# hamptus/mlx-swift-qwen3-tts

Measured on NVIDIA B200. Metric: audio-sec generated per sec (RTFx), higher is better.
Workload: dtype u4 g64 weights dequantised at load to f16 operands x f32 accumulate, f32 residual stream

## Files before the change

mlx-swift-qwen3-tts_b200/csrc/api.cu:

```cuda
#include <algorithm>
#include <atomic>
#include <deque>
#include <chrono>
#include <map>
#include <thread>

#include "audio_encoder.h"
#include "speaker_encoder.h"
#include "codec.h"
#include "codec_kernels.h"
#include "engine.h"
#include "gemm_tc.h"
#include "tc_ptx.cuh"

using namespace q3;

struct q3tts_handle : q3::Handle {};

namespace q3 {
void init_talker_kernels();
Handle::~Handle() {
  for (Handle* l : lanes) {
    cudaStreamSynchronize(l->stream);
    delete static_cast<q3tts_handle*>(l);
// ... 323 lines not shown

int64_t plan_decode(int mode, const int32_t* frames, int n, float* out, int64_t capacity, int up, std::vector<DecodeJob>& jobs) {
  if (n <= 0) return 0;
  const int64_t total = std::min<int64_t>((int64_t)n * up, capacity);
  if (mode == Q3TTS_DECODE_WHOLE) {
    jobs.push_back({frames, n, out, 0, total});
    return total;
  }
  const int chunk = mode == Q3TTS_DECODE_FILE ? 16 : (mode == Q3TTS_DECODE_BATCHAPI ? 24 : 18), left = 8;
  for (int pos = 0; pos < n; pos += chunk) {
    const int end = std::min(pos + chunk, n);
    const int ctx = pos == 0 ? 0 : std::min(left, pos);
    const int64_t o0 = (int64_t)pos * up;
    if (o0 >= total) break;
    jobs.push_back({frames + (size_t)(pos - ctx) * 16, end - pos + ctx, out + o0, (int64_t)ctx * up, std::min<int64_t>((int64_t)(end - pos) * up, total - o0)});
  }
  return total;
}

}

extern "C" {

int32_t q3tts_abi_version(void) { return Q3TTS_ABI_VERSION; }

void q3tts_default_options(q3tts_options* o) {
  if (!o) return;
  memset(o, 0, sizeof *o);
  o->struct_size = (int32_t)sizeof *o;
  o->device = 0;
  o->max_batch = 1;
  o->kv_capacity = 512;
  o->max_frames = 2400;
  o->use_cuda_graph = 1;
  o->load_codec = 1;
  o->load_talker = 1;
  o->codec_max_frames = 2400;
  o->codec_max_batch = 8;
}

void q3tts_default_request(q3tts_request* r) {
  if (!r) return;
  memset(r, 0, sizeof *r);
  r->struct_size = (int32_t)sizeof *r;
  r->speaker_id = -1;
  r->temperature = 0.9f;
  r->top_k = 0;
  r->top_p = 1.0f;
  r->repetition_penalty = 1.05f;
  r->max_tokens = 1200;
}

q3tts_status q3tts_create(const char* model_dir, const q3tts_options* opts, q3tts_handle** out) {
  if (!out) return Q3TTS_ERR_INVALID_ARG;
  *out = nullptr;
  q3tts_handle* h = nullptr;
  try {
    Q3_CHECK(model_dir != nullptr, Q3TTS_ERR_INVALID_ARG, "model_dir is NULL");
    q3tts_options o;
    q3tts_default_options(&o);
    if (opts) {
      const size_t n = std::min<size_t>(sizeof o, opts->struct_size > 0 ? (size_t)opts->struct_size : sizeof o);
      memcpy(&o, opts, n);
    }
    require_device(o.device);
    h = new q3tts_handle();
    h->opt.device = o.device;
    h->opt.max_batch = o.max_batch > 0 ? o.max_batch : 1;
    h->opt.kv_capacity = o.kv_capacity > 0 ? std::max(o.kv_capacity, 208) : 512;
    h->opt.max_frames = o.max_frames > 0 ? o.max_frames : 2400;
    h->opt.use_cuda_graph = o.use_cuda_graph;
    h->opt.load_codec = o.load_codec;
    h->opt.load_talker = o.load_talker;
    h->opt.codec_max_frames = o.codec_max_frames > 0 ? o.codec_max_frames : 2400;
    h->opt.codec_max_batch = o.codec_max_batch > 0 ? o.codec_max_batch : 8;
    Q3_CHECK(o.packed_gemm >= 0 && o.packed_gemm <= 2, Q3TTS_ERR_INVALID_ARG, "options.packed_gemm must be 0, 1 or 2");
    h->opt.packed_gemm = o.packed_gemm;
    h->opt.runtime_quantization = o.runtime_quantization != 0;
    h->opt.lanes = std::max(1, std::min(o.lanes, 8));
    if (o.cuda_stream) {
      h->stream = (cudaStream_t)o.cuda_stream;
    } else {
      Q3_CUDA(cudaStreamCreateWithFlags(&h->stream, cudaStreamNonBlocking));
      h->own_stream = true;
    }
    h->opt.stream = h->stream;
    Q3_CUDA(cudaEventCreate(&h->ev_start));
    Q3_CUDA(cudaEventCreate(&h->ev_stop));
    const std::string dir(model_dir);
    h->model_dir = dir;
    if (h->opt.load_talker) {
      Json root = parse_json_file(dir + "/config.json");
      h->cfg = parse_talker_config(root);
      h->talker.reset(new TalkerEngine(dir, h->cfg, h->opt, h->stream, &h->counter));
      h->has_talker = true;
      if (SpeakerEncoderDev::present(dir)) {
        try {
          h->speaker_encoder.reset(new SpeakerEncoderDev(dir, h->stream, &h->counter));
        } catch (const Error& e) {
          g_create_error = std::string("speaker encoder not loaded: ") + e.what();
          cudaGetLastError();
        }
      }
    }
    if (h->opt.load_codec) {
      h->codec.reset(new CodecDecoder(dir + "/speech_tokenizer", h->stream, &h->counter, h->opt.codec_max_frames));
      h->codec->set_use_graph(h->opt.use_cuda_graph != 0);
      if (AudioEncoder::present(dir + "/speech_tokenizer")) {
        try {
          h->audio_encoder.reset(new AudioEncoder(dir + "/speech_tokenizer", h->stream, &h->counter));
        } catch (const Error& e) {
          g_create_error = std::string("audio encoder not loaded: ") + e.what();
          cudaGetLastError();
        }
      }
    }
    Q3_CUDA(cudaStreamSynchronize(h->stream));
    *out = h;
    return Q3TTS_OK;
  } catch (const Error& e) {
    g_create_error = e.what();
    cudaGetLastError();
    delete h;
    return e.status;
  } catch (const std::exception& e) {
    g_create_error = e.what();
    delete h;
    return Q3TTS_ERR_CUDA;
  }
}

q3tts_status q3tts_clone(q3tts_handle* parent, q3tts_handle** out) {
  if (!out) return Q3TTS_ERR_INVALID_ARG;
  *out = nullptr;
  if (!parent) return Q3TTS_ERR_INVALID_ARG;
  q3tts_handle* h = nullptr;
  try {
    std::lock_guard<std::mutex> lk(parent->mu);
    Q3_CHECK(!parent->poisoned, Q3TTS_ERR_CUDA, "the parent handle is poisoned");
    Q3_CUDA(cudaSetDevice(parent->opt.device));
    h = new q3tts_handle();
    h->opt = parent->opt;
    h->opt.lanes = 1;
    h->model_dir = parent->model_dir;
    Q3_CUDA(cudaStreamCreateWithFlags(&h->stream, cudaStreamNonBlocking));
    h->own_stream = true;
    h->opt.stream = h->stream;
    Q3_CUDA(cudaEventCreate(&h->ev_start));
    Q3_CUDA(cudaEventCreate(&h->ev_stop));
    if (parent->talker) {
      h->cfg = parent->cfg;
      h->talker.reset(new TalkerEngine(h->model_dir, h->cfg, h->opt, h->stream, &h->counter, parent->talker->shared()));
      h->has_talker = true;
    }
    if (parent->codec) {
      h->codec.reset(new CodecDecoder(h->model_dir + "/speech_tokenizer", h->stream, &h->counter, h->opt.codec_max_frames));
      h->codec->set_use_graph(h->opt.use_cuda_graph != 0);
    }
    Q3_CUDA(cudaStreamSynchronize(h->stream));
    *out = h;
    return Q3TTS_OK;
  } catch (const Error& e) {
    g_create_error = e.what();
    cudaGetLastError();
    delete h;
    return e.status;
  } catch (const std::exception& e) {
    g_create_error = e.what();
    delete h;
    return Q3TTS_ERR_CUDA;
  }
}

void q3tts_destroy(q3tts_handle* h) {
  if (!h) return;
  cudaSetDevice(h->opt.device);
  cudaStreamSynchronize(h->stream);
  delete h;
}

const char* q3tts_last_error(const q3tts_handle* h) { return h ? h->last_error.c_str() : g_create_error.c_str(); }

q3tts_status q3tts_get_info(const q3tts_handle* hc, q3tts_info* out) {
  if (!hc || !out) return Q3TTS_ERR_INVALID_ARG;
  memset(out, 0, sizeof *out);
  const TalkerConfig& c = hc->cfg;
  if (hc->talker) {
    out->hidden_size = c.hidden_size; out->num_layers = c.num_hidden_layers; out->num_heads = c.num_attention_heads;
    out->num_kv_heads = c.num_key_value_heads; out->head_dim = c.head_dim; out->intermediate_size = c.intermediate_size;
    out->vocab_size = c.vocab_size; out->text_vocab_size = c.text_vocab_size; out->text_hidden_size = c.text_hidden_size;
    out->cp_hidden_size = c.cp.hidden_size; out->cp_num_layers = c.cp.num_hidden_layers; out->cp_vocab_size = c.cp.vocab_size;
    out->num_code_groups = c.cp.num_code_groups;
    out->quant_bits = hc->talker->quant_bits(); out->quant_group_size = hc->talker->quant_group();
    out->weight_dtype = hc->talker->weight_dtype();
    out->num_speakers = (int32_t)c.spk_id.size();
    out->model_type = c.tts_model_type == "voice_design" ? 1 : (c.tts_model_type == "custom_voice" ? 2 : 0);
    out->codec_eos_id = c.codec_eos_token_id; out->codec_pad_id = c.codec_pad_id;
    out->max_batch = hc->talker->max_batch(); out->kv_capacity = hc->talker->kv_capacity(); out->max_frames = hc->talker->max_frames();
    out->device_bytes += (int64_t)hc->talker->device_bytes();
  }
  if (hc->codec) {
    out->has_codec = 1;
    out->codec_num_quantizers = hc->codec->config().num_quantizers;
    out->codec_total_upsample = hc->codec->total_upsample();
    out->device_bytes += (int64_t)hc->codec->device_bytes();
  }
  if (hc->speaker_encoder) {
    out->has_speaker_encoder = 1;
    out->speaker_embedding_dim = hc->speaker_encoder->embedding_dim();
    out->device_bytes += (int64_t)hc->speaker_encoder->device_bytes();
  }
  if (hc->audio_encoder) {
    out->has_audio_encoder = 1;
    out->audio_encoder_hidden = hc->audio_encoder->config().hidden_size;
    out->device_bytes += (int64_t)hc->audio_encoder->device_bytes();
  }
  return Q3TTS_OK;
}

q3tts_status q3tts_speaker_name(const q3tts_handle* h, int32_t index, char* name_out, int32_t capacity, int32_t* id_out) {
  if (!h || index < 0 || index >= (int32_t)h->cfg.spk_id.size()) return Q3TTS_ERR_INVALID_ARG;
  std::vector<std::pair<std::string, int>> s = h->cfg.spk_id;
  std::sort(s.begin(), s.end());
  if (name_out && capacity > 0) {
    strncpy(name_out, s[index].first.c_str(), capacity - 1);
    name_out[capacity - 1] = 0;
  }
  if (id_out) *id_out = s[index].second;
  return Q3TTS_OK;
}

int32_t q3tts_speaker_id(const q3tts_handle* h, const char* name) {
  if (!h || !name) return -1;
  for (auto& kv : h->cfg.spk_id)
    if (kv.first == name) return kv.second;
  return -1;
}

q3tts_status q3tts_clear_cache(q3tts_handle* h) {
  if (h) {
    std::lock_guard<std::mutex> lk(h->lanes_mu);
    for (q3::Handle* l : h->lanes) q3tts_clear_cache(static_cast<q3tts_handle*>(l));
  }
  return guarded(h, [&] {
    Q3_CUDA(cudaStreamSynchronize(h->stream));
    if (h->talker) h->talker->drop_graphs();
  });
}

namespace {
__global__ void debug_mbar_trap_kernel() {
  __shared__ uint64_t bar;
  if (threadIdx.x == 0) {
    q3::tcptx::mbar_init(&bar, 1);
    asm volatile("fence.mbarrier_init.release.cluster;" ::: "memory");
  }
  __syncthreads();
  if (threadIdx.x == 0) q3::tcptx::mbar_wait(&bar, 0);
}
}

q3tts_status q3tts_debug_trap(q3tts_handle* h) {
  return guarded(h, [&] {
    debug_mbar_trap_kernel<<<1, 32, 0, h->stream>>>();
    Q3_CUDA(cudaGetLastError());
    Q3_CUDA(cudaStreamSynchronize(h->stream));
  });
}

q3tts_status q3tts_get_timing(const q3tts_handle* h, q3tts_timing* out) {
  if (!h || !out) return Q3TTS_ERR_INVALID_ARG;
  *out = h->timing;
  return Q3TTS_OK;
}

q3tts_status q3tts_generate_codes(q3tts_handle* h, const q3tts_request* req, int32_t* codes_out, int32_t capacity_frames,
                                  int32_t* frames_out) {
  return guarded(h, [&] {
    Q3_CHECK(req && frames_out, Q3TTS_ERR_INVALID_ARG, "NULL argument");
    Q3_CHECK(h->talker != nullptr, Q3TTS_ERR_MODEL_NOT_LOADED, "Model is not loaded");
    require_no_open_stream(h);
    *frames_out = 0;
    CallTimer tm(h);
    std::vector<int32_t> raw;
    int n_raw = 0;
    run_single(h, *req, raw, n_raw);
    *frames_out = filter_frames(*req, raw, n_raw, codes_out, capacity_frames);
    h->timing.d2h_bytes += (int64_t)n_raw * 64;
    h->timing.h2d_bytes += (int64_t)req->n_text_ids * 4;
    tm.finish();
  });
}

static bool use_lanes(q3tts_handle* h, const q3tts_request* reqs, int32_t n) {
  if (!h || !reqs || h->opt.lanes <= 1 || n <= h->opt.max_batch || h->poisoned) return false;
  for (int i = 0; i < n; ++i)
    if (reqs[i].code0_logits_out || reqs[i].cp_logits_out) return false;
  return true;
}

}
template <typename F>
static q3tts_status over_lanes(q3tts_handle* h, int32_t n, F&& run) {
  const int B = h->opt.max_batch;
  const int blocks = (n + B - 1) / B;
  const int L = std::min(h->opt.lanes, blocks);
// ... 843 lines not shown
```

mlx-swift-qwen3-tts_b200/csrc/engine.h:

```cpp
#pragma once
#include <map>
#include <memory>
#include <mutex>
#include <string>
#include <vector>

#include "frame_kernel.h"
#include "kernels.h"

namespace q3 {

class CodecDecoder;
class AudioEncoder;
class SpeakerEncoderDev;

struct EngineOptions {
  int device = 0;
  cudaStream_t stream = nullptr;
  int max_batch = 1, kv_capacity = 512, max_frames = 2400, use_cuda_graph = 1;
  int load_codec = 1, load_talker = 1, codec_max_frames = 2400, codec_max_batch = 8;
  int lanes = 1;
  int max_trailing = 1024;
  int packed_gemm = 0;
  int runtime_quantization = 0;
};

struct Admission {
  bool too_short = false;
  int prefill_len = 0;
};

struct TalkerShared {
  DeviceArena arena;
  TalkerWeights w;
  int weight_dtype = Q3TTS_BF16, eff_bits = 0, eff_group = 64;
  std::mutex mu;
};

class TalkerEngine {
 public:
  TalkerEngine(const std::string& model_dir, const TalkerConfig& cfg, const EngineOptions& opt, cudaStream_t stream,
               LaunchCounter* counter, std::shared_ptr<TalkerShared> shared = nullptr);
  ~TalkerEngine();

  Admission admit(int slot, const q3tts_request& req);
  struct AdmitItem { int slot; const q3tts_request* req; };
  void admit_batch(const std::vector<AdmitItem>& items, std::vector<Admission>& out);
  int max_prefill_rows() const { return max_rows_; }
  int step_slots(int hi) const {
    if (!handle_tc_) return hi;
    int b = hi <= 32 ? 32 : (hi <= 64 ? 64 : (hi + 127) / 128 * 128);
    return b < opt_.max_batch ? b : opt_.max_batch;
  }
  void run_frames(int n_slots, int n);
  void fetch_states(int n_slots, std::vector<SlotState>& out);
  void fetch_frames(int slot, int first, int count, int32_t* dst);
  void fetch_logits(int frames, float* code0_out, float* cp_out);
  int dump_slot() const { return dump_enabled_ ? dump_slot_ : -1; }
  void release(int slot);
  void drop_graphs();

  const TalkerConfig& config() const { return cfg_; }
  const TalkerWeights& weights() const { return w_; }
  int max_batch() const { return opt_.max_batch; }
  int kv_capacity() const { return opt_.kv_capacity; }
  int max_frames() const { return opt_.max_frames; }
  int weight_dtype() const { return shared_->weight_dtype; }
  int quant_bits() const { return shared_->eff_bits; }
  int quant_group() const { return shared_->eff_group; }
  size_t device_bytes() const { return arena_.total() + (owns_weights_ ? shared_->arena.total() : 0); }
  const std::shared_ptr<TalkerShared>& shared() const { return shared_; }
  size_t weight_bytes_per_frame() const { return w_.talker_step_bytes + 15 * w_.cp_pass_bytes; }
  int64_t graph_replays = 0, graph_nodes_replayed = 0, mega_launches = 0;
  bool megakernel_enabled() const { return mega_.ok; }
  double last_prefill_ms = 0;

  double profile_linears(int which, int m, int iters, int64_t& launches, int64_t& bytes_per_iter);
  int sample_probe(const float* logits, int vocab, float temperature, int top_k, float top_p, float rep_penalty,
                   const int32_t* token_set, int n_set, uint64_t seed, uint64_t counter);

 private:
  void forward_stack(const StackWeights& S, float* x, int m, const int* row_slot, const int* row_pos, const int* win_start,
                     const float* inv_freq, void* kbase, void* vbase, int kv_f16, size_t slot_stride, size_t layer_stride, int capacity,
                     bool one_row_per_slot, bool decode_step, bool x16_ready);
  void issue_frame(int n_slots);
  void build_tc_weights();
  void build_mega_plan();
  TcLinear make_tc(const Linear& L, bool interleave_halves, const float* fold = nullptr);
  bool use_tc(int) const { return handle_tc_; }
  bool use_tc_step(int) const { return handle_tc_; }
  bool use_mega(int n_slots) const { return mega_.ok && !handle_tc_ && opt_.max_batch <= mega_.max_slots && n_slots <= mega_.max_slots; }
  void linear_tc(const TcLinear& L, const void* x16, int m, float* out32, int ld32, void* out16, int ld16, const float* res, int act, int swiglu, bool row_count_invariant = false);
  LaunchCtx ctx() { return LaunchCtx{stream_, counter_, chain_on_ ? &chain_ : nullptr}; }

  TalkerConfig cfg_;
  EngineOptions opt_;
  cudaStream_t stream_;
  LaunchCounter* counter_;
  DeviceArena arena_;
  std::shared_ptr<TalkerShared> shared_;
  bool owns_weights_ = false;
  TalkerWeights& w_;

  int max_rows_ = 0, max_tp_rows_ = 0, set_words_ = 0;
  int tc_min_rows_ = 16, tc_min_rows_step_ = 3;
  bool step_tc_ = false;
  bool handle_tc_ = false;
  bool packed_gemm_ = false;
  void attach_packed(struct TcGemm& g, const TcLinear& L) const;
  static constexpr int kChainCounters = 1024;
  ChainState chain_;
  bool chain_on_ = false, chain_enabled_ = false;
  float* d_rs_ = nullptr;
  static constexpr float kX16Div = 16.0f;
  void *d_h16_ = nullptr, *d_attn16_ = nullptr, *d_act16_ = nullptr, *d_tpe16_ = nullptr, *d_tph16_ = nullptr;
  void *kcache_ = nullptr, *vcache_ = nullptr;
  int kv_f16_ = 0;
  float *cp_k_ = nullptr, *cp_v_ = nullptr;
  size_t kv_slot_stride_ = 0, kv_layer_stride_ = 0, cpkv_slot_stride_ = 0, cpkv_layer_stride_ = 0;
  static constexpr int kCpCapacity = 32;
  SlotState* d_state_ = nullptr;
  int *d_step_slot_ = nullptr, *d_step_pos_ = nullptr, *d_win_ = nullptr;
  int *d_cp_slot2_ = nullptr, *d_cp_pos2_ = nullptr, *d_iota_ = nullptr, *d_cp_pos_ = nullptr;
  int *d_pf_slot_ = nullptr, *d_pf_pos_ = nullptr, *d_pf_win_ = nullptr;
  float *d_x_ = nullptr, *d_qkv_ = nullptr, *d_attn_ = nullptr, *d_act_ = nullptr;
  float *d_hlast_ = nullptr, *d_logits0_ = nullptr, *d_cplogits_ = nullptr, *d_cpin_ = nullptr, *d_cpx_ = nullptr, *d_xstep_ = nullptr;
  int *d_cur_codes_ = nullptr, *d_frames_ = nullptr, *d_forced_ = nullptr;
  unsigned* d_sets_ = nullptr;
  float *d_trailing_ = nullptr, *d_tts_ = nullptr;
  float *d_tpe_ = nullptr, *d_tph_ = nullptr, *d_tp_ = nullptr, *d_spk_ = nullptr;
  int *d_ids_ = nullptr, *d_desc_ = nullptr;
  Embedding* d_cp_emb_ = nullptr;
  float *d_inv_freq_ = nullptr, *d_cp_inv_freq_ = nullptr;
  float *d_dump0_ = nullptr, *d_dumpcp_ = nullptr;
  int dump_cap_ = 0, dump_slot_ = 0;
  bool dump_enabled_ = false;
  float* d_probe_logits_ = nullptr;
  unsigned* d_probe_set_ = nullptr;
  int* d_probe_out_ = nullptr;
  int* h_stage_ = nullptr;
  size_t h_stage_ints_ = 0;
  SlotState* h_state_ = nullptr;
  cudaEvent_t ev_a_ = nullptr, ev_b_ = nullptr;

  struct Graph {
    cudaGraphExec_t exec = nullptr;
    int64_t nodes = 0;
  };
  std::map<long long, Graph> graphs_;
  MegaPlan mega_;
};

struct Handle {
  std::mutex mu;
  std::string model_dir;
  std::string last_error;
  bool poisoned = false;
  EngineOptions opt;
  cudaStream_t stream = nullptr;
  bool own_stream = false;
  LaunchCounter counter;
  TalkerConfig cfg;
  bool has_talker = false;
  std::unique_ptr<TalkerEngine> talker;
  std::unique_ptr<CodecDecoder> codec;
  std::unique_ptr<AudioEncoder> audio_encoder;
  std::unique_ptr<SpeakerEncoderDev> speaker_encoder;
  q3tts_timing timing{};
  cudaEvent_t ev_start = nullptr, ev_stop = nullptr;
  float* h_pcm = nullptr;
  size_t h_pcm_floats = 0;
  int32_t* h_codes = nullptr;
  size_t h_codes_ints = 0;
  int32_t* d_codes = nullptr;
  size_t d_codes_ints = 0;
  float* d_pcm = nullptr;
  size_t d_pcm_floats = 0;
  void* open_stream = nullptr;
  std::mutex lanes_mu;
  std::vector<Handle*> lanes;
  ~Handle();
};

}
```

mlx-swift-qwen3-tts_b200/csrc/gemm_skinny.cu:

```cuda
#include <cuda.h>

#include <algorithm>

#include "skinny_common.cuh"

namespace q3 {

namespace {

using namespace skinny;

template <int ACT, bool SWIGLU>
__global__ void __launch_bounds__(kThreads, 1)
tc_skinny_kernel(const __grid_constant__ CUtensorMap tmW, const __grid_constant__ CUtensorMap tmX, const SkParams p) {
  extern __shared__ uint8_t smem_raw[];
  uint8_t* smem = reinterpret_cast<uint8_t*>((reinterpret_cast<uintptr_t>(smem_raw) + 1023) & ~(uintptr_t)1023);
  const int x_bytes = p.m_pad * kBlockK * 2;
  uint8_t* sW = smem;
  uint8_t* sX = smem + (size_t)p.stages * kWBytes;
  float* red = reinterpret_cast<float*>(sX + (size_t)p.stages * x_bytes);
  uint64_t* full = reinterpret_cast<uint64_t*>(red + (size_t)kRowsW * p.m_pad);
  uint64_t* empty = full + p.stages;
  uint64_t* tmem_full = empty + p.stages;
  uint64_t* red_full = tmem_full + 1;
// ... 31 lines not shown
  __syncthreads();
  tc_fence_after();
  const uint32_t tmem_base = *tmem_slot;
  if (threadIdx.x == 0) SK_STAMP(2);
  if (p.split > 1) cluster_arrive_release();

  if (warp == 0) {
    {
      const bool lead = elect_one();
      const int pre = nkb < p.stages ? nkb : p.stages;
      if (lead) {
        for (int i = 0; i < pre; ++i) {
          mbar_expect_tx(&full[i], (uint32_t)(kWBytes + x_bytes));
          tma_load_2d(sW + (size_t)i * kWBytes, &tmW, &full[i], (kb0 + i) * kBlockK, n0);
        }
        for (int i = pre; i < nkb; ++i) tma_prefetch_2d(&tmW, (kb0 + i) * kBlockK, n0);
      }
      if (p.sig.in) {
        if (lead) sk_wait_dependency_tma(p);
        __syncwarp();
      } else {
        pdl_wait();
      }
      int s = 0;
      uint32_t ph = 0;
      for (int i = 0; i < nkb; ++i) {
        if (i >= pre) mbar_wait(&empty[s], ph ^ 1u);
        if (lead) {
          if (i >= pre) {
            mbar_expect_tx(&full[s], (uint32_t)(kWBytes + x_bytes));
            tma_load_2d(sW + (size_t)s * kWBytes, &tmW, &full[s], (kb0 + i) * kBlockK, n0);
          }
          tma_load_2d(sX + (size_t)s * x_bytes, &tmX, &full[s], (kb0 + i) * kBlockK, 0);
        }
        if (++s == p.stages) { s = 0; ph ^= 1u; }
      }
    }
    __syncwarp();
  } else if (warp == 1) {
    {
      const bool lead = elect_one();
      const uint32_t idesc = (1u << 4) | ((uint32_t)(p.m_pad >> 3) << 17) | ((uint32_t)(kRowsW >> 4) << 24);
      int s = 0;
      uint32_t ph = 0;
      for (int i = 0; i < nkb; ++i) {
        mbar_wait(&full[s], ph);
        tc_fence_after();
        if (lead && i == 0) SK_STAMP(3);
        const uint64_t ad = umma_desc(smem_u32(sW + (size_t)s * kWBytes));
        const uint64_t bd = umma_desc(smem_u32(sX + (size_t)s * x_bytes));
        if (lead) {
#pragma unroll
          for (int k = 0; k < kBlockK / 16; ++k)
            umma_f16(tmem_base, ad + (uint64_t)(2 * k), bd + (uint64_t)(2 * k), idesc, (i | k) != 0 ? 1u : 0u);
          umma_commit(&empty[s]);
        }
        if (++s == p.stages) { s = 0; ph ^= 1u; }
      }
      if (lead) umma_commit(tmem_full);
    }
    __syncwarp();
  } else {
    sk_wait_dependency_warp(p);
    if (p.rms_x) sk_row_factors(p, rowscale_s, rank);
    if (p.split > 1) cluster_wait_acquire();
    mbar_wait(tmem_full, 0);
    tc_fence_after();
    if (threadIdx.x == 64) SK_STAMP(4);
    sk_reduce_epilogue<ACT, SWIGLU>(p, reinterpret_cast<float*>(smem), red, red_full, ack, rowscale_s, tmem_base, rank, n0);
  }
  if (p.split > 1 && warp < 2) cluster_wait_acquire();
  tc_fence_before();
  __syncthreads();
  if (threadIdx.x == 0 && p.trace) {
    SK_STAMP(8);
    p.trace[((size_t)blockIdx.y * gridDim.x + blockIdx.x) * 16 + 9] = sk_globaltimer();
  }
  if (warp == 1) {
    tc_fence_after();
    asm volatile("tcgen05.dealloc.cta_group::1.sync.aligned.b32 %0, %1;" ::"r"(tmem_base), "r"(p.tmem_cols) : "memory");
  }
}

int env_int(const char* name, int dflt) {
  const char* e = getenv(name);
  return e ? atoi(e) : dflt;
}

struct SkPlan {
  int m_pad, split, stages, num_kb, tiles;
  size_t smem;
};

SkPlan plan(const TcGemm& g) {
  static const int max_split = std::max(1, std::min(16, env_int("Q3TTS_SK_MAX_SPLIT", 8)));
  static const int cta_target = env_int("Q3TTS_SK_CTAS", 200);
  static const int smem_kb = env_int("Q3TTS_SK_SMEM_KB", 108);
  SkPlan s{};
  const int M = g.Bt * g.T;
  s.m_pad = M <= 32 ? 32 : (M <= 64 ? 64 : 128);
  s.tiles = (g.N + kRowsW - 1) / kRowsW;
  s.num_kb = (g.cin + kBlockK - 1) / kBlockK;
  s.split = 1;
  while (s.split * 2 <= max_split && s.tiles * s.split * 2 <= cta_target && s.split * 2 <= s.num_kb && s.m_pad / (s.split * 2) >= 4) s.split *= 2;
  const int stage_bytes = kWBytes + s.m_pad * kBlockK * 2;
  const int red_bytes = kRowsW * s.m_pad * 4;
  const int nkb_max = (s.num_kb + s.split - 1) / s.split;
  s.stages = std::max(2, (smem_kb * 1024 - red_bytes) / stage_bytes);
  s.stages = std::max(1, std::min(s.stages, nkb_max));
  while (s.stages * stage_bytes < red_bytes) ++s.stages;
  s.smem = (size_t)s.stages * stage_bytes + red_bytes + 1024 + (2 * s.stages + 4) * 8 + 16 + 128 * 4;
  return s;
}

}

bool tc_skinny_enabled() {
  static const bool on = env_int("Q3TTS_SKINNY", 1) != 0;
  return on;
}

bool tc_skinny_supported(const TcGemm& g) {
  const bool on = tc_skinny_enabled();
  const long long M = (long long)g.Bt * g.T;
  return on && g.allow_skinny && !g.res16 && !g.outr16 && g.ntap == 1 && M >= 1 && M <= 128 && !g.snake_ea && !g.pcm && !(g.swiglu && g.act != TC_ACT_NONE) && tc_gemm_supported(g);
}

using SkKernel = void (*)(const CUtensorMap, const CUtensorMap, const SkParams);
static SkKernel pick_kernel(int act, int swiglu) {
  if (swiglu) return tc_skinny_kernel<TC_ACT_NONE, true>;
  if (act == TC_ACT_GELU) return tc_skinny_kernel<TC_ACT_GELU, false>;
  if (act == TC_ACT_SILU) return tc_skinny_kernel<TC_ACT_SILU, false>;
  return tc_skinny_kernel<TC_ACT_NONE, false>;
}

void init_tc_skinny() {
  tc_resolve_encode();
  for (SkKernel k : {pick_kernel(0, 1), pick_kernel(TC_ACT_GELU, 0), pick_kernel(TC_ACT_SILU, 0), pick_kernel(0, 0)})
    Q3_CUDA(cudaFuncSetAttribute(k, cudaFuncAttributeMaxDynamicSharedMemorySize, 220 * 1024));
  for (SkKernel k : {pick_kernel(0, 1), pick_kernel(TC_ACT_GELU, 0), pick_kernel(TC_ACT_SILU, 0), pick_kernel(0, 0)})
    Q3_CUDA(cudaFuncSetAttribute(k, cudaFuncAttributeNonPortableClusterSizeAllowed, 1));
  init_tc_skinny_q();
}

unsigned long long* g_sk_trace = nullptr;

void tc_skinny_set_trace(unsigned long long* dev_buf) { g_sk_trace = dev_buf; }
unsigned long long* tc_skinny_trace_buf() { return g_sk_trace; }
void tc_skinny_grid(const TcGemm& g, int* tiles, int* split, int* stages) {
  const SkPlan s = plan(g);
  *tiles = s.tiles; *split = s.split; *stages = s.stages;
}

void launch_tc_skinny(const LaunchCtx& c, const TcGemm& g) {
  if (tc_skinny_q_supported(g)) return launch_tc_skinny_q(c, g);
  Q3_CHECK(tc_skinny_supported(g), Q3TTS_ERR_INVALID_ARG, "tc_skinny: unsupported shape (rows %d, cin %d, N %d)", g.Bt * g.T, g.cin, g.N);
  tc_resolve_encode();
  const SkPlan s = plan(g);
  SkParams p{};
  p.M = g.Bt * g.T; p.N = g.N; p.K = g.cin;
  p.m_pad = s.m_pad; p.split = s.split; p.mc = s.m_pad / s.split; p.stages = s.stages; p.num_kb = s.num_kb;
  p.mc_shift = 0;
  while ((1 << p.mc_shift) < p.mc) ++p.mc_shift;
  p.split_shift = 0;
  while ((1 << p.split_shift) < p.split) ++p.split_shift;
  p.tmem_cols = std::max(32, s.m_pad);
  p.bias = g.bias; p.res = g.res; p.ld_res = g.ld_res; p.scale = g.scale; p.act = g.act; p.swiglu = g.swiglu;
  p.out32 = g.out32; p.ld32 = g.ld32; p.out16 = g.out16; p.ld16 = g.ld16;
  p.out16_scale = g.out16_scale;
  p.rms_x = g.rms_in ? g.a : nullptr;
  p.rms_a = 1.0f / (g.in_scale * g.in_scale * (float)g.cin); p.rms_eps = g.rms_eps; p.rms_mult = 1.0f / g.in_scale;
  Q3_CHECK(!g.row_scale, Q3TTS_ERR_INVALID_ARG, "tc_skinny: pass rms_in instead of precomputed row factors");
  p.trace = g_sk_trace;
  p.sig = c.chain_link((unsigned)(s.tiles * s.split));

  const uint64_t wdims[2] = {(uint64_t)g.cin, (uint64_t)g.N};
  const uint64_t wstr[1] = {(uint64_t)g.cin * 2};
  const uint32_t wbox[2] = {(uint32_t)kBlockK, (uint32_t)kRowsW};
  const CUtensorMap mw = tc_make_map(g.w, 2, wdims, wstr, wbox);
  const uint64_t xdims[2] = {(uint64_t)g.cin, (uint64_t)p.M};
  const uint64_t xstr[1] = {(uint64_t)g.cin * 2};
  const uint32_t xbox[2] = {(uint32_t)kBlockK, (uint32_t)s.m_pad};
  const CUtensorMap mx = tc_make_map(g.a, 2, xdims, xstr, xbox);

  Q3_CHECK(s.smem <= 220 * 1024, Q3TTS_ERR_CAPACITY, "tc_skinny: shared memory request %zu too large", s.smem);
  cudaLaunchConfig_t cfg{};
  cfg.gridDim = dim3((unsigned)s.tiles, (unsigned)s.split);
  cfg.blockDim = dim3(kThreads);
  cfg.dynamicSmemBytes = s.smem;
  cfg.stream = c.stream;
  cudaLaunchAttribute attr[2];
  int na = 0;
  if (s.split > 1) {
    attr[na].id = cudaLaunchAttributeClusterDimension;
    attr[na].val.clusterDim.x = 1; attr[na].val.clusterDim.y = (unsigned)s.split; attr[na].val.clusterDim.z = 1;
    ++na;
  }
  if (pdl_enabled()) {
    attr[na].id = cudaLaunchAttributeProgrammaticStreamSerialization;
    attr[na].val.programmaticStreamSerializationAllowed = 1;
    ++na;
  }
  cfg.attrs = attr;
  cfg.numAttrs = na;
  Q3_CUDA(cudaLaunchKernelEx(&cfg, pick_kernel(g.act, g.swiglu), mw, mx, p));
  c.tick_chained();
}

}
```

mlx-swift-qwen3-tts_b200/csrc/skinny_common.cuh:

```cuda
#pragma once
#include <cuda.h>

#include "gemm_tc.h"
#include "tc_ptx.cuh"

namespace q3 {
namespace skinny {

using namespace tcptx;

constexpr int kRowsW = 128;
constexpr int kBlockK = 64;
constexpr int kWBytes = kRowsW * kBlockK * 2;
constexpr int kThreads = 192;

struct SkParams {
  int M, N, K;
  int m_pad, mc, mc_shift, split, stages, num_kb, tmem_cols;
  const float* bias;
  const float* res;
  int ld_res;
  const float* scale;
  int act, swiglu;
  float* out32;
  int ld32;
  __half* out16;
  int ld16;
  float out16_scale;
  const __half* rms_x;
  float rms_a, rms_eps, rms_mult;
  unsigned long long* trace;
  ChainSig sig;
  const void* q_scales;
  const void* q_biases;
  const float* q_fold;
  int q_group, q_sdt;
  int q_pstages;
  int q_xstages, q_xown;
  int q_half_rows;
  int split_shift;
  int q_dbg;
};

__device__ __forceinline__ unsigned long long sk_globaltimer() {
  unsigned long long t;
  asm volatile("mov.u64 %0, %%globaltimer;" : "=l"(t));
  return t;
}
#define SK_STAMP_EPI(slot) do { if (!(p.q_dbg & 1)) SK_STAMP(slot); } while (0)
#define SK_STAMP(slot)                                                                                        \
  do {                                                                                                        \
    if (p.trace) p.trace[((size_t)blockIdx.y * gridDim.x + blockIdx.x) * 16 + (slot)] = (unsigned long long)clock64(); \
  } while (0)

__device__ __forceinline__ float sk_gelu_erf(float v) { return 0.5f * v * (1.0f + erff(v * 0.70710678118654752440f)); }
__device__ __forceinline__ float sk_silu(float v) { return v / (1.0f + expf(-v)); }
__device__ __forceinline__ float sk_silu_fast(float v) { return __fdividef(v, 1.0f + __expf(-v)); }

__device__ __forceinline__ float4 lds_f4(uint32_t saddr) {
  float4 v;
  asm volatile("ld.shared.v4.f32 {%0, %1, %2, %3}, [%4];" : "=f"(v.x), "=f"(v.y), "=f"(v.z), "=f"(v.w) : "r"(saddr));
  return v;
}

template <int NC>
__device__ __forceinline__ void sk_load_res(const SkParams& p, float (&r)[NC], int valid, int m0, int ob) {
  if (p.res) {
    const float* rp = p.res + (size_t)m0 * p.ld_res + ob;
#pragma unroll
    for (int e = 0; e < NC; ++e, rp += p.ld_res) r[e] = e < valid ? *rp : 0.f;
  }
}
template <int NC, int ACT, bool SWIGLU>
__device__ __forceinline__ void sk_finish(const SkParams& p, float (&acc)[NC], const float (&r)[NC], int valid, int m0, int ob, float bias,
                                          float scale, const float* rowscale) {
#pragma unroll
  for (int e = 0; e < NC; ++e) {
    float v = acc[e];
    if (rowscale) v *= rowscale[e];
    v += bias;
    if (ACT == TC_ACT_GELU) v = sk_gelu_erf(v);
    else if (ACT == TC_ACT_SILU) v = sk_silu(v);
    if (SWIGLU) {
      const float up = __shfl_xor_sync(0xffffffffu, v, 1);
      v = sk_silu_fast(v) * up;
    }
    if (p.res) v = r[e] + scale * v;
    acc[e] = v;
  }
  if (p.out32) {
    float* op = p.out32 + (size_t)m0 * p.ld32 + ob;
#pragma unroll
    for (int e = 0; e < NC; ++e, op += p.ld32)
      if (e < valid) *op = acc[e];
  }
  if (p.out16) {
    __half* hp = p.out16 + (size_t)m0 * p.ld16 + ob;
#pragma unroll
    for (int e = 0; e < NC; ++e, hp += p.ld16)
      if (e < valid) *hp = __float2half_rn(acc[e] * p.out16_scale);
  }
}

template <int ACT, bool SWIGLU>
__device__ __forceinline__ void sk_reduce_epilogue(const SkParams& p, float* stage_out, float* red, uint64_t* red_full, uint64_t* ack, const float* rowscale_s,
                                                   uint32_t tmem_base, uint32_t rank, int n0) {
  const int warp = threadIdx.x >> 5, lane = threadIdx.x & 31;
  const int q = warp & 3;
  const int row = q * 32 + lane;
  const int n = n0 + row;
  const bool n_ok = n < p.N;
  const uint32_t taddr = tmem_base + ((uint32_t)(q * 32) << 16);
  const float bias = (p.bias && n_ok) ? p.bias[n] : 0.f;
  const int so = SWIGLU ? (n >> 1) : n;
  const float scale = (p.scale && n_ok) ? p.scale[so] : 1.f;
  for (int c0 = 0; c0 < p.m_pad; c0 += 32) {
    uint32_t raw[32];
    tmem_ld32(taddr + (uint32_t)c0, raw);
#pragma unroll
    for (int j = 0; j < 32; j += 4) {
      const int col = c0 + j;
      const int dst = col >> p.mc_shift;
      const int off = col & (p.mc - 1);
      *reinterpret_cast<float4*>(stage_out + (size_t)dst * kRowsW * p.mc + ((size_t)(off >> 2) * kRowsW + row) * 4) =
          make_float4(__uint_as_float(raw[j]), __uint_as_float(raw[j + 1]), __uint_as_float(raw[j + 2]), __uint_as_float(raw[j + 3]));
    }
  }
  asm volatile("fence.proxy.async.shared::cta;" ::: "memory");
  asm volatile("bar.sync 1, 128;" ::: "memory");
  const uint32_t slice_bytes = (uint32_t)(kRowsW * p.mc * 4);
  if (threadIdx.x == 64 && p.split > 1) {
    mbar_expect_tx(red_full, slice_bytes * (uint32_t)(p.split - 1));
    for (int i = 1; i < p.split; ++i) {
      const uint32_t d = (rank + (uint32_t)i) & (uint32_t)(p.split - 1);
      bulk_copy_to_rank(map_to_rank(smem_u32(red + (size_t)rank * kRowsW * p.mc), d), smem_u32(stage_out + (size_t)d * kRowsW * p.mc), slice_bytes,
                        map_to_rank(smem_u32(red_full), d));
    }
  }
  if (threadIdx.x == 64) SK_STAMP(5);
  const int m_base = (int)rank * p.mc;
  const bool lane_out = n_ok && (!SWIGLU || (n & 1) == 0);
  float r16[16];
  {
    int valid0 = p.M - m_base;
    valid0 = valid0 < 16 ? valid0 : 16;
    valid0 = valid0 < p.mc ? valid0 : p.mc;
    sk_load_res<16>(p, r16, lane_out ? valid0 : 0, m_base, so);
  }
  if (p.split > 1) mbar_wait(red_full, 0);
  if (threadIdx.x == 96) SK_STAMP_EPI(10);
  if (threadIdx.x == 64) {
    SK_STAMP(6);
    for (int i = 1; i < p.split; ++i) mbar_arrive_remote_relaxed(map_to_rank(smem_u32(ack), (rank + (uint32_t)i) & (uint32_t)(p.split - 1)));
  }
  const uint32_t own_s = smem_u32(stage_out), red_s = smem_u32(red);
  for (int cb = 0; cb < p.mc; cb += 16) {
    const int nc = p.mc - cb < 16 ? p.mc - cb : 16;
    float a16[16];
#pragma unroll
    for (int j = 0; j < 16; ++j) a16[j] = 0.f;
    for (int s = 0; s < p.split; ++s) {
      const uint32_t base = (s == (int)rank ? own_s : red_s) + (uint32_t)s * slice_bytes + (uint32_t)row * 16u;
#pragma unroll
      for (int c = 0; c < 16; c += 4) {
        if (c < nc) {
          const float4 v = lds_f4(base + (uint32_t)((cb + c) >> 2) * (uint32_t)(kRowsW * 16));
          a16[c] += v.x; a16[c + 1] += v.y; a16[c + 2] += v.z; a16[c + 3] += v.w;
        }
      }
    }
    if (threadIdx.x == 96 && cb == 0) SK_STAMP_EPI(11);
    int valid = p.M - (m_base + cb);
    valid = valid < nc ? valid : nc;
    if (!lane_out) valid = 0;
    if (cb > 0) sk_load_res<16>(p, r16, valid, m_base + cb, so);
    sk_finish<16, ACT, SWIGLU>(p, a16, r16, valid, m_base + cb, so, bias, scale, p.rms_x ? rowscale_s + cb : nullptr);
    if (threadIdx.x == 96 && cb == 0) SK_STAMP_EPI(12);
  }
  if (threadIdx.x == 96) SK_STAMP_EPI(13);
  if (p.sig.out) {
    asm volatile("bar.sync 1, 128;" ::: "memory");
    if (threadIdx.x == 64) chain_signal(p.sig.out);
  }
  if (threadIdx.x == 64 && p.split > 1) {
    SK_STAMP(7);
    mbar_wait(ack, 0);
  }
}

__device__ __forceinline__ void sk_wait_dependency_warp(const SkParams& p) {
  if (p.sig.in) {
    if ((threadIdx.x & 31) == 0) chain_wait(p.sig.in, p.sig.in_target);
    __syncwarp();
  } else {
    pdl_wait();
  }
}
__device__ __forceinline__ void sk_wait_dependency_tma(const SkParams& p) {
  if (p.sig.in) {
    chain_wait(p.sig.in, p.sig.in_target);
    asm volatile("fence.proxy.async;" ::: "memory");
  } else {
    pdl_wait();
  }
}

__device__ __forceinline__ void sk_row_factors(const SkParams& p, float* rowscale_s, uint32_t rank) {
  const int warp = threadIdx.x >> 5, lane = threadIdx.x & 31;
  const int q = warp & 3;
  const int m_lo = (int)rank * p.mc, j = lane & 7;
  for (int r0 = 0; r0 < p.mc; r0 += 16) {
    const int r = r0 + q * 4 + (lane >> 3), m = m_lo + r;
    float ss = (r < p.mc && m < p.M) ? tc_row_sumsq_f16(p.rms_x + (size_t)m * p.K, p.K, j) : 0.f;
    ss = tc_group8_sum(ss);
    if (j == 0 && r < p.mc) rowscale_s[r] = p.rms_mult * rsqrtf(ss * p.rms_a + p.rms_eps);
  }
}

}
}
```

mlx-swift-qwen3-tts_b200/csrc/talker_engine.cu:

```cuda
#include <algorithm>
#include <cmath>

#include "engine.h"
#include "frame_kernel.h"
#include "gemm_tc.h"

namespace q3 {

void init_talker_kernels();
int mega_max_blocks_per_sm(int fmt, int slots, size_t smem);

TalkerEngine::TalkerEngine(const std::string& model_dir, const TalkerConfig& cfg, const EngineOptions& opt, cudaStream_t stream,
                           LaunchCounter* counter, std::shared_ptr<TalkerShared> shared)
    : cfg_(cfg), opt_(opt), stream_(stream), counter_(counter), shared_(shared ? shared : std::make_shared<TalkerShared>()),
      owns_weights_(!shared), w_(shared_->w) {
  init_talker_kernels();
  if (owns_weights_)
    load_talker_weights(model_dir, cfg_, shared_->arena, stream_, w_, shared_->weight_dtype, shared_->eff_bits, shared_->eff_group,
                        opt_.runtime_quantization != 0);
  const int B = opt_.max_batch, C = opt_.kv_capacity, F = opt_.max_frames;
  const int H = cfg_.hidden_size, Hcp = cfg_.cp.hidden_size;
  Q3_CHECK(B >= 1 && C >= 208 && F >= 1, Q3TTS_ERR_INVALID_ARG, "bad options: max_batch %d kv_capacity %d max_frames %d", B, C, F);
  const StackWeights &T = w_.talker, &P = w_.cp;
  max_rows_ = std::max(std::max(2 * B, C), std::min(B * 96, 8192));
  max_tp_rows_ = std::max(C + opt_.max_trailing + 8, std::min(B * 128, 16384));
  set_words_ = (std::max(cfg_.vocab_size, cfg_.cp.vocab_size) + 31) / 32;

  kv_layer_stride_ = (size_t)T.kv_heads * C * 128;
  kv_slot_stride_ = kv_layer_stride_ * T.layers;
  {
    int min_rows = 3;
    if (const char* e = getenv("Q3TTS_TC_MIN_ROWS")) min_rows = atoi(e);
    const char* e16 = getenv("Q3TTS_KV_F16");
    kv_f16_ = (min_rows > 0 && B >= min_rows && !(e16 && atoi(e16) == 0)) ? 1 : 0;
  }
  const size_t kv_elem = kv_f16_ ? 2 : 4;
  kcache_ = arena_.alloc(kv_slot_stride_ * B * kv_elem);
  vcache_ = arena_.alloc(kv_slot_stride_ * B * kv_elem);
  cpkv_layer_stride_ = (size_t)P.kv_heads * kCpCapacity * 128;
  cpkv_slot_stride_ = cpkv_layer_stride_ * P.layers;
  cp_k_ = arena_.alloc_n<float>(cpkv_slot_stride_ * B);
  cp_v_ = arena_.alloc_n<float>(cpkv_slot_stride_ * B);

  d_state_ = arena_.alloc_n<SlotState>(B);
  Q3_CUDA(cudaMemsetAsync(d_state_, 0, sizeof(SlotState) * B, stream_));
  d_step_slot_ = arena_.alloc_n<int>(B); d_step_pos_ = arena_.alloc_n<int>(B); d_win_ = arena_.alloc_n<int>(B);
  d_cp_slot2_ = arena_.alloc_n<int>(2 * B); d_cp_pos2_ = arena_.alloc_n<int>(2 * B);
  d_iota_ = arena_.alloc_n<int>(B); d_cp_pos_ = arena_.alloc_n<int>(16 * B);
  d_pf_slot_ = arena_.alloc_n<int>(max_rows_); d_pf_pos_ = arena_.alloc_n<int>(max_rows_); d_pf_win_ = arena_.alloc_n<int>(B);
  Q3_CUDA(cudaMemsetAsync(d_pf_win_, 0, sizeof(int) * B, stream_));
  Q3_CUDA(cudaMemsetAsync(d_win_, 0, sizeof(int) * B, stream_));

  const int wide_h = std::max(H, Hcp);
  const int qkv_w = std::max((T.heads + 2 * T.kv_heads) * 128, (P.heads + 2 * P.kv_heads) * 128);
  const int attn_w = std::max(T.heads, P.heads) * 128;
  const int act_w = std::max(T.inter, P.inter);
  d_x_ = arena_.alloc_n<float>((size_t)max_rows_ * wide_h);
  d_qkv_ = arena_.alloc_n<float>((size_t)max_rows_ * qkv_w);
  d_attn_ = arena_.alloc_n<float>((size_t)max_rows_ * attn_w);
  d_act_ = arena_.alloc_n<float>((size_t)max_rows_ * act_w);
  d_hlast_ = arena_.alloc_n<float>((size_t)B * H);
  d_logits0_ = arena_.alloc_n<float>((size_t)B * cfg_.vocab_size);
  d_cplogits_ = arena_.alloc_n<float>((size_t)B * cfg_.cp.vocab_size);
  d_cpin_ = arena_.alloc_n<float>((size_t)2 * B * H);
  d_cpx_ = arena_.alloc_n<float>((size_t)2 * B * Hcp);
  d_xstep_ = arena_.alloc_n<float>((size_t)B * H);
  d_cur_codes_ = arena_.alloc_n<int>((size_t)B * 16);
  Q3_CUDA(cudaMemsetAsync(d_cur_codes_, 0, sizeof(int) * B * 16, stream_));
  d_frames_ = arena_.alloc_n<int>((size_t)B * F * 16);
  d_forced_ = arena_.alloc_n<int>((size_t)B * F * 16);
  d_sets_ = arena_.alloc_n<unsigned>((size_t)B * 16 * set_words_);
  d_trailing_ = arena_.alloc_n<float>((size_t)B * opt_.max_trailing * H);
  d_tts_ = arena_.alloc_n<float>((size_t)3 * H);
  d_tpe_ = arena_.alloc_n<float>((size_t)max_tp_rows_ * cfg_.text_hidden_size);
  d_tph_ = arena_.alloc_n<float>((size_t)max_tp_rows_ * cfg_.text_hidden_size);
  d_tp_ = arena_.alloc_n<float>((size_t)max_tp_rows_ * H);
  d_spk_ = arena_.alloc_n<float>((size_t)B * H);
  d_ids_ = arena_.alloc_n<int>(max_tp_rows_);
  d_desc_ = arena_.alloc_n<int>((size_t)3 * max_rows_);
  if (const char* e = getenv("Q3TTS_TC_MIN_ROWS")) tc_min_rows_ = tc_min_rows_step_ = atoi(e);
  if (tc_min_rows_step_ > 0 && B >= tc_min_rows_step_) {
    init_tc_gemm();
    {
      std::lock_guard<std::mutex> lk(shared_->mu);
      if (!w_.has_tc) build_tc_weights();
    }
    d_h16_ = arena_.alloc((size_t)max_rows_ * std::max(wide_h, cfg_.text_hidden_size) * 2);
    d_attn16_ = arena_.alloc((size_t)max_rows_ * attn_w * 2);
    d_act16_ = arena_.alloc((size_t)max_rows_ * act_w * 2);
    d_rs_ = arena_.alloc_n<float>((size_t)max_rows_);
    d_tpe16_ = arena_.alloc((size_t)max_tp_rows_ * cfg_.text_hidden_size * 2);
    d_tph16_ = arena_.alloc((size_t)max_tp_rows_ * cfg_.text_hidden_size * 2);
  }
  handle_tc_ = w_.has_tc && tc_min_rows_step_ > 0 && B >= tc_min_rows_step_;
  {
    const char* e = getenv("Q3TTS_SKINNY_Q");
    packed_gemm_ = opt_.packed_gemm == 1 || (opt_.packed_gemm == 0 && e && atoi(e) != 0);
  }
  Q3_CHECK(!kv_f16_ || handle_tc_ || !w_.has_tc, Q3TTS_ERR_BAD_CONFIG, "internal: fp16 KV rings on a handle without the tensor-core step");
  chain_.base = arena_.alloc_n<unsigned>(kChainCounters);
  chain_.capacity = kChainCounters;
  Q3_CUDA(cudaMemsetAsync(chain_.base, 0, sizeof(unsigned) * kChainCounters, stream_));
  chain_enabled_ = false;
  if (const char* e = getenv("Q3TTS_CHAIN")) chain_enabled_ = atoi(e) != 0;
  if (!pdl_enabled()) chain_enabled_ = false;
  d_probe_logits_ = arena_.alloc_n<float>(4096);
  d_probe_set_ = arena_.alloc_n<unsigned>(128);
  d_probe_out_ = arena_.alloc_n<int>(1);

  std::vector<int> slot2(2 * B), pos2(2 * B), iota(B), cpos(16 * B);
  for (int s = 0; s < B; ++s) {
    slot2[2 * s] = slot2[2 * s + 1] = s;
    pos2[2 * s] = 0; pos2[2 * s + 1] = 1;
    iota[s] = s;
    for (int g = 0; g < 16; ++g) cpos[g * B + s] = g + 1;
  }
  Q3_CUDA(cudaMemcpy(d_cp_slot2_, slot2.data(), slot2.size() * 4, cudaMemcpyHostToDevice));
  Q3_CUDA(cudaMemcpy(d_cp_pos2_, pos2.data(), pos2.size() * 4, cudaMemcpyHostToDevice));
  Q3_CUDA(cudaMemcpy(d_iota_, iota.data(), iota.size() * 4, cudaMemcpyHostToDevice));
  Q3_CUDA(cudaMemcpy(d_cp_pos_, cpos.data(), cpos.size() * 4, cudaMemcpyHostToDevice));

  std::vector<float> f(64), fc(64);
  for (int i = 0; i < 64; ++i) {
    f[i] = 1.0f / powf(cfg_.rope_theta, (float)(2 * i) / 128.0f);
    fc[i] = 1.0f / powf(cfg_.cp.rope_theta, (float)(2 * i) / 128.0f);
  }
  d_inv_freq_ = arena_.alloc_n<float>(64); d_cp_inv_freq_ = arena_.alloc_n<float>(64);
  Q3_CUDA(cudaMemcpy(d_inv_freq_, f.data(), 256, cudaMemcpyHostToDevice));
  Q3_CUDA(cudaMemcpy(d_cp_inv_freq_, fc.data(), 256, cudaMemcpyHostToDevice));

  d_cp_emb_ = arena_.alloc_n<Embedding>(15);
  Q3_CUDA(cudaMemcpy(d_cp_emb_, w_.cp_codec_embedding.data(), sizeof(Embedding) * 15, cudaMemcpyHostToDevice));

  h_stage_ints_ = (size_t)max_tp_rows_ + 3 * (size_t)C + 64;
  Q3_CUDA(cudaMallocHost(&h_stage_, h_stage_ints_ * sizeof(int)));
  Q3_CUDA(cudaMallocHost(&h_state_, sizeof(SlotState) * B));
  Q3_CUDA(cudaEventCreate(&ev_a_));
  Q3_CUDA(cudaEventCreate(&ev_b_));

  h_stage_[0] = cfg_.tts_bos_token_id; h_stage_[1] = cfg_.tts_eos_token_id; h_stage_[2] = cfg_.tts_pad_token_id;
  for (int i = 0; i < 3; ++i)
    Q3_CHECK(h_stage_[i] >= 0 && h_stage_[i] < cfg_.text_vocab_size, Q3TTS_ERR_BAD_CONFIG, "tts special token id %d outside text vocab", h_stage_[i]);
  Q3_CUDA(cudaMemcpyAsync(d_ids_, h_stage_, 12, cudaMemcpyHostToDevice, stream_));
  LaunchCtx c{stream_, nullptr};
  launch_gather_rows(c, w_.text_embedding, d_ids_, 3, d_tpe_, cfg_.text_hidden_size, false);
  launch_linear(c, w_.fc1, d_tpe_, cfg_.text_hidden_size, 3, d_tph_, cfg_.text_hidden_size, nullptr, 0.f, EPI_SILU);
  launch_linear(c, w_.fc2, d_tph_, cfg_.text_hidden_size, 3, d_tts_, H, nullptr, 0.f, EPI_STORE);
  Q3_CUDA(cudaStreamSynchronize(stream_));
  build_mega_plan();
}

void TalkerEngine::build_mega_plan() {
  mega_ = MegaPlan{};
  if (const char* e = getenv("Q3TTS_MEGAKERNEL"))
    if (atoi(e) == 0) return;
  if (!opt_.use_cuda_graph) return;
  const StackWeights &T = w_.talker, &P = w_.cp;
  std::vector<const Linear*> order;
  std::vector<int> swiglu;
  struct Norms { const float *norm_w, *q_norm, *k_norm; };
  struct PhaseInfo { int in_kind, pass, epi, out_sel, flags, layer, unit, tkind; };
  std::vector<Norms> norms;
  std::vector<PhaseInfo> phase;
  enum { IN_GX = 0, IN_GX_LAST, IN_CP0, IN_CPG, IN_TALKER, IN_ATTN, IN_ACT };
  enum { E_STORE = 0, E_ADD_RAW = 1, E_SWIGLU = 2 };
  auto push = [&](const Linear& L, bool sw, PhaseInfo ph, const float* nw = nullptr, const float* qn = nullptr, const float* kn = nullptr) {
    order.push_back(&L); swiglu.push_back(sw ? 1 : 0); norms.push_back({nw, qn, kn}); phase.push_back(ph);
  };
  for (int u = 0; u < 16; ++u) {
    const bool talker = (u == 15);
    const StackWeights& S = talker ? T : P;
    const int base = (talker ? MF_TALKER : 0) | (u == 0 ? MF_ROWS2 : 0);
    const int first_kind = talker ? IN_TALKER : (u == 0 ? IN_CP0 : IN_CPG);
    bool first = true;
    auto flags_of = [&](int extra) { const int f = base | extra | (first ? MF_UNIT_START : 0); first = false; return f; };
    const bool mtp = !talker && w_.has_mtp;
    if (mtp) push(w_.small_to_mtp, false, {first_kind, u, E_STORE, 0, flags_of(0), 0, u, 0});
    for (int l = 0; l < S.layers; ++l) {
      const LayerWeights& lw = S.layer[l];
      const int qkv_in = (l == 0 && !mtp) ? first_kind : IN_GX;
      push(lw.qkv, false, {qkv_in, u, E_STORE, 1, flags_of(MF_ATTN | MF_KEEP_RAW | ((talker && l == 0) ? MF_FINALIZE : 0)), l, u, 1}, lw.in_norm, lw.q_norm, lw.k_norm);
      push(lw.o, false, {IN_ATTN, u, E_ADD_RAW, 0, flags_of(0), l, u, 2});
      push(lw.gate_up, true, {IN_GX, u, E_SWIGLU, 2, flags_of(MF_KEEP_RAW), l, u, 3}, lw.post_norm);
      push(lw.down, false, {IN_ACT, u, E_ADD_RAW, 0, flags_of(0), l, u, 4});
    }
    if (talker) push(w_.codec_head, false, {IN_GX, u, E_STORE, 3, flags_of(MF_HEAD | MF_KEEP_RAW), 0, u, 5}, T.final_norm);
    else push(w_.lm_head[u], false, {IN_GX_LAST, u == 0 ? 2 : 1, E_STORE, 3, flags_of(MF_HEAD), 0, u, 5}, P.final_norm);
  }
  const Linear& L0 = *order[0];
  int fmt = -1;
  if (L0.bits == 4) fmt = 0; else if (L0.bits == 8) fmt = 1;
  else if (L0.bits == 0) fmt = L0.sdt == Q3TTS_BF16 ? 2 : (L0.sdt == Q3TTS_F16 ? 3 : 4);
  if (fmt < 0) return;
  const int vpl = fmt == 0 ? 32 : (fmt == 1 ? 16 : (fmt == 4 ? 4 : 8));
  const int kc = 32 * vpl;
  std::vector<MegaLinear> lin;
  int kmax = 0, need_slot = 0;
  for (size_t i = 0; i < order.size(); ++i) {
    const Linear& L = *order[i];
    if (L.bits != L0.bits || (L.bits == 0 && L.sdt != L0.sdt)) return;
    if (L.bits && (L.group % vpl != 0 || L.in % L.group != 0)) return;
    if (L.in % vpl != 0 || L.in % 4 != 0) return;
    MegaLinear m{};
    m.w = L.bits ? (const void*)L.qw : L.w; m.scales = L.scales; m.biases = L.biases; m.bias = L.bias;
    m.nsub = swiglu[i] ? 2 : 1;
    m.out_eff = L.out / m.nsub;
    m.in = L.in;
    m.row_bytes = L.bits ? L.in * L.bits / 8 : L.in * (int)dtype_size(L.sdt);
    m.srow_bytes = L.bits ? (L.in / L.group) * (int)dtype_size(L.sdt) : 0;
    m.sdt = L.sdt; m.group = L.bits ? L.group : 1;
    if (m.group & (m.group - 1)) return;
    m.group_shift = 0;
    while ((1 << m.group_shift) < m.group) ++m.group_shift;
    int u = 1;
    while (u <= 16 && ((u * m.row_bytes) % 16 != 0 || (u * m.srow_bytes) % 16 != 0)) u <<= 1;
    if (u > 16 || m.out_eff % u != 0) return;
    m.unit = u;
    m.norm_w = norms[i].norm_w; m.q_norm = norms[i].q_norm; m.k_norm = norms[i].k_norm;
    m.in_kind = phase[i].in_kind; m.pass = phase[i].pass; m.epi = phase[i].epi; m.out_sel = phase[i].out_sel; m.flags = phase[i].flags;
    m.layer = phase[i].layer; m.uidx = phase[i].unit; m.tkind = phase[i].tkind;
    need_slot = std::max(need_slot, u * m.nsub * (m.row_bytes + 2 * m.srow_bytes));
    kmax = std::max(kmax, L.in);
    lin.push_back(m);
  }
  const int G_tk = T.heads / T.kv_heads, G_cp = P.heads / P.kv_heads;
  auto g_ok = [](int g) { return g == 1 || g == 2 || g == 4; };
  if (!g_ok(G_tk) || !g_ok(G_cp) || T.head_dim != 128 || P.head_dim != 128) return;
  if (T.heads % T.kv_heads || P.heads % P.kv_heads) return;
  if (cfg_.vocab_size > 4096 || cfg_.cp.vocab_size > 4096) return;
  if (T.hidden % 4 || P.hidden % 4 || T.inter % 4 || P.inter % 4) return;
  int slot_bytes = 32 * 1024;
  while (slot_bytes < need_slot) slot_bytes += 8 * 1024;
  const int nchunk = (kmax + kc - 1) / kc;
  const int hmax = std::max(T.hidden, P.hidden);
  auto up = [](int v, int a) { return (v + a - 1) / a * a; };
  const bool mma = (fmt == 0 || fmt == 1);
  int gmin = 1 << 30, gmax = 0, max_tiles = 0;
  for (const MegaLinear& m : lin) {
    gmin = std::min(gmin, m.group); gmax = std::max(gmax, m.group);
    const int rch = (slot_bytes / (m.nsub * (m.row_bytes + 2 * m.srow_bytes))) / m.unit * m.unit;
    max_tiles = std::max(max_tiles, ((rch + 15) / 16) * m.nsub);
  }
  if (mma && (gmin < 32 || gmax > 128 || kmax % 32 != 0)) return;
  const int budget = 226 * 1024;
  int NS = 0, MT = 0, n_ring = 0, xs_bytes = 0, xsum_bytes = 0, xraw_bytes = 0, red_bytes = 0, hl_bytes = 0, rope_bytes = 0, part_bytes = 0;
  const int scratch = (4096 + 64 + 4096) * 4;
  for (int cand : {kMegaMaxSlots, 1}) {
    if (cand > 1 && (!mma || opt_.max_batch < 2)) continue;
    NS = cand; MT = 2 * NS;
    const bool tc = mma && cand > 1;
    xs_bytes = up(std::max(tc ? 8 * (kmax * 2 + 64) : MT * nchunk * kc * 4, scratch), 128);
    xsum_bytes = up(tc ? MT * (kmax / gmin) * 4 : MT * nchunk * 32 * 4, 128);
    xraw_bytes = up(MT * hmax * 4, 128);
    red_bytes = up(MT * 16 * 4, 128);
    hl_bytes = up(NS * hmax * 4, 128);
    rope_bytes = up(NS * 128 * 2 * 4, 128);
    part_bytes = tc ? up(std::max(32, max_tiles) * 128 * 4, 128) : 0;
    const int fixed = xs_bytes + xsum_bytes + xraw_bytes + red_bytes + 256 + 512 + hl_bytes + rope_bytes + part_bytes + 128;
    n_ring = std::min(8, (budget - fixed) / slot_bytes);
    if (n_ring >= 3 || (cand == 1 && n_ring >= 2)) break;
    NS = 0;
  }
  if (NS == 0) return;
  mega_.max_slots = NS;
  MegaParams& p = mega_.p;
  p.slot_bytes = slot_bytes; p.n_ring = n_ring;
  p.off_xs = n_ring * slot_bytes;
  p.off_xsum = p.off_xs + xs_bytes;
  p.off_xraw = p.off_xsum + xsum_bytes;
  p.off_red = p.off_xraw + xraw_bytes;
  p.off_bar = p.off_red + red_bytes;
  p.off_dsc = p.off_bar + 256;
  static_assert(2 * sizeof(MegaLinear) <= 512, "descriptor slots");
  p.off_hl = p.off_dsc + 512;
  p.raw_ld = hmax;
  p.off_rope = p.off_hl + hl_bytes;
  p.off_part = p.off_rope + rope_bytes;
  p.xh_stride = kmax + 32;
  mega_.smem = (size_t)p.off_part + part_bytes + 128;
  mega_.fmt = fmt; mega_.G_cp = G_cp; mega_.G_tk = G_tk;
  int dev = 0, sms = 0, coop = 0;
  Q3_CUDA(cudaGetDevice(&dev));
  Q3_CUDA(cudaDeviceGetAttribute(&sms, cudaDevAttrMultiProcessorCount, dev));
  Q3_CUDA(cudaDeviceGetAttribute(&coop, cudaDevAttrCooperativeLaunch, dev));
  if (!coop || sms < 1) return;
  init_mega_kernels();
  if (mega_max_blocks_per_sm(fmt, mega_.max_slots, mega_.smem) < 1) return;
  int min_units = 1 << 30;
  for (const MegaLinear& m : lin) min_units = std::min(min_units, m.out_eff / m.unit);
  mega_.grid = std::min(sms, min_units);
  if (mega_.grid < 1 || opt_.kv_capacity > 4 * 128) return;
  for (MegaLinear& m : lin) {
    const int U = m.out_eff / m.unit;
    m.ubase = U / mega_.grid; m.urem = U % mega_.grid;
    m.rch = (slot_bytes / (m.nsub * (m.row_bytes + 2 * m.srow_bytes))) / m.unit * m.unit;
  }
  MegaLinear* d_lin = arena_.alloc_n<MegaLinear>(lin.size());
  Q3_CUDA(cudaMemcpy(d_lin, lin.data(), sizeof(MegaLinear) * lin.size(), cudaMemcpyHostToDevice));
  auto stack_of = [&](const StackWeights& S, const float* inv_freq, float* k, float* v, size_t slot_stride, size_t layer_stride, int cap, int nsplit) {
    MegaStack s{};
    s.hidden = S.hidden; s.layers = S.layers; s.heads = S.heads; s.kv_heads = S.kv_heads; s.inter = S.inter; s.eps = S.eps;
    s.final_norm = S.final_norm; s.inv_freq = inv_freq; s.k = k; s.v = v;
    s.slot_stride = slot_stride; s.layer_stride = layer_stride; s.capacity = cap; s.nsplit = nsplit;
    return s;
  };
  const int nsplit_tk = 4;
  p.lin = d_lin; p.n_lin = (int)lin.size();
  p.cp = stack_of(P, d_cp_inv_freq_, cp_k_, cp_v_, cpkv_slot_stride_, cpkv_layer_stride_, kCpCapacity, 1);
  if (kv_f16_) return;
  p.tk = stack_of(T, d_inv_freq_, (float*)kcache_, (float*)vcache_, kv_slot_stride_, kv_layer_stride_, opt_.kv_capacity, nsplit_tk);
  p.has_mtp = w_.has_mtp ? 1 : 0; p.H = cfg_.hidden_size; p.Hcp = cfg_.cp.hidden_size; p.V = cfg_.vocab_size; p.Vc = cfg_.cp.vocab_size;
  p.codec = w_.codec_embedding; p.cp_emb = d_cp_emb_;
  p.st = d_state_; p.cur_codes = d_cur_codes_; p.frames = d_frames_; p.forced = d_forced_; p.max_frames = opt_.max_frames;
  p.sets = d_sets_; p.set_words = set_words_;
  p.trailing = d_trailing_; p.max_trailing = opt_.max_trailing; p.tts_pad = d_tts_ + (size_t)2 * cfg_.hidden_size;
  p.hlast = d_hlast_; p.logits0 = d_logits0_; p.cplogits = d_cplogits_;
  p.part_stride = up(std::max(T.heads, P.heads) * 130, 4);
  p.ld_x = up(hmax, 4);
  p.ld_qkv = up(std::max((T.heads + 2 * T.kv_heads) * 128, (P.heads + 2 * P.kv_heads) * 128), 4);
  p.ld_act = up(std::max(T.inter, P.inter), 4);
  p.ld_logit = up(std::max(cfg_.vocab_size, cfg_.cp.vocab_size), 4);
  const size_t n_x = (size_t)MT * p.ld_x, n_qkv = (size_t)MT * p.ld_qkv, n_part = (size_t)MT * nsplit_tk * p.part_stride;
  const size_t n_act = (size_t)MT * p.ld_act, n_logit = (size_t)NS * p.ld_logit, n_msg = (size_t)2 * 16 * kMegaMaxSlots * 4;
  p.ex_bytes = (n_x + n_qkv + n_part + n_act + n_logit + n_msg) * sizeof(unsigned long long);
  unsigned long long* ex = arena_.alloc_n<unsigned long long>(n_x + n_qkv + n_part + n_act + n_logit + n_msg);
  p.ex_base = ex;
  p.ex_x = ex; ex += n_x;
  p.ex_qkv = ex; ex += n_qkv;
  p.ex_part = ex; ex += n_part;
  p.ex_act = ex; ex += n_act;
  p.ex_logit = ex; ex += n_logit;
  p.ex_msg = ex;
  p.window = 192;
  p.eos_id = cfg_.codec_eos_token_id; p.pad_id = cfg_.codec_pad_id;
  if (getenv("Q3TTS_MEGA_TRACE")) {
    p.trace_stride = 8 * 1024 * 8;
    p.trace = arena_.alloc_n<long long>((size_t)2 * p.trace_stride);
  }
  mega_.ok = true;
}

TalkerEngine::~TalkerEngine() {
  drop_graphs();
  if (h_stage_) cudaFreeHost(h_stage_);
  if (h_state_) cudaFreeHost(h_state_);
  if (ev_a_) cudaEventDestroy(ev_a_);
  if (ev_b_) cudaEventDestroy(ev_b_);
  if (d_dump0_) cudaFree(d_dump0_);
  if (d_dumpcp_) cudaFree(d_dumpcp_);
}

void TalkerEngine::drop_graphs() {
  for (auto& g : graphs_)
    if (g.second.exec) cudaGraphExecDestroy(g.second.exec);
  graphs_.clear();
}

TcLinear TalkerEngine::make_tc(const Linear& L, bool interleave_halves, const float* fold) {
  const LaunchCtx c{stream_, nullptr};
  TcLinear t;
  t.out = L.out; t.in = L.in; t.bias = L.bias;
  if (L.bits) { t.qw = L.qw; t.qscales = L.scales; t.qbiases = L.biases; t.qbits = L.bits; t.qgroup = L.group; t.qsdt = L.sdt; t.fold = fold; t.halves = interleave_halves; }
  __half* dst = (__half*)shared_->arena.alloc((size_t)L.out * L.in * 2);
  if (L.bits && fold) {
    float* tmp = nullptr;
    Q3_CUDA(cudaMalloc(&tmp, (size_t)L.out * L.in * 4));
    launch_dequantize(c, L.qw, L.scales, L.biases, L.sdt, L.out, L.in, L.group, L.bits, Q3TTS_F32, tmp);
    launch_weight_to_f16(c, tmp, Q3TTS_F32, L.out, L.in, interleave_halves, dst, fold);
    Q3_CUDA(cudaStreamSynchronize(stream_));
    cudaFree(tmp);
  } else if (L.bits) {
    if (!interleave_halves) {
      launch_dequantize(c, L.qw, L.scales, L.biases, L.sdt, L.out, L.in, L.group, L.bits, Q3TTS_F16, dst);
    } else {
      __half* tmp = nullptr;
      Q3_CUDA(cudaMalloc(&tmp, (size_t)L.out * L.in * 2));
      launch_dequantize(c, L.qw, L.scales, L.biases, L.sdt, L.out, L.in, L.group, L.bits, Q3TTS_F16, tmp);
      launch_weight_to_f16(c, tmp, Q3TTS_F16, L.out, L.in, true, dst);
      Q3_CUDA(cudaStreamSynchronize(stream_));
      cudaFree(tmp);
    }
  } else {
    launch_weight_to_f16(c, L.w, L.sdt, L.out, L.in, interleave_halves, dst, fold);
  }
  t.w = dst;
  return t;
}

void TalkerEngine::build_tc_weights() {
  auto ok = [](const Linear& L) { return L.in % 8 == 0 && L.out % 32 == 0; };
  bool all = ok(w_.fc1) && ok(w_.fc2) && ok(w_.codec_head) && (!w_.has_mtp || ok(w_.small_to_mtp));
  for (StackWeights* S : {&w_.talker, &w_.cp})
    for (auto& l : S->layer) all = all && ok(l.qkv) && ok(l.o) && ok(l.gate_up) && ok(l.down) && (l.gate_up.out / 2) % 16 == 0;
  for (auto& h : w_.lm_head) all = all && ok(h);
  if (!all) return;
  for (StackWeights* S : {&w_.talker, &w_.cp}) {
    S->tc.resize(S->layers);
    for (int l = 0; l < S->layers; ++l) {
      S->tc[l].qkv = make_tc(S->layer[l].qkv, false, S->layer[l].in_norm);
      S->tc[l].o = make_tc(S->layer[l].o, false);
      S->tc[l].gate_up_il = make_tc(S->layer[l].gate_up, true, S->layer[l].post_norm);
      S->tc[l].down = make_tc(S->layer[l].down, false);
    }
  }
  w_.fc1_tc = make_tc(w_.fc1, false);
  w_.fc2_tc = make_tc(w_.fc2, false);
  w_.codec_head_tc = make_tc(w_.codec_head, false);
  for (auto& h : w_.lm_head) w_.lm_head_tc.push_back(make_tc(h, false, w_.cp.final_norm));
  if (w_.has_mtp) w_.small_to_mtp_tc = make_tc(w_.small_to_mtp, false);
  Q3_CUDA(cudaStreamSynchronize(stream_));
  w_.has_tc = true;
}

void TalkerEngine::attach_packed(TcGemm& g, const TcLinear& L) const {
  if (!L.qbits || !packed_gemm_) return;
  g.q_w = L.qw; g.q_scales = L.qscales; g.q_biases = L.qbiases; g.q_fold = L.fold;
  g.q_bits = L.qbits; g.q_group = L.qgroup; g.q_sdt = L.qsdt; g.q_halves = L.halves ? 1 : 0;
}

void TalkerEngine::linear_tc(const TcLinear& L, const void* x16, int m, float* out32, int ld32, void* out16, int ld16, const float* res,
                             int act, int swiglu, bool row_count_invariant) {
  TcGemm g;
  if (row_count_invariant) { g.allow_skinny = 0; g.k_rotate = 0; }
  g.a = (const __half*)x16; g.w = (const __half*)L.w; g.Bt = 1; g.T = m; g.cin = L.in; g.N = L.out; g.ntap = 1; g.dil = 1;
  g.bias = L.bias; g.res = res; g.ld_res = ld32; g.act = act; g.swiglu = swiglu;
  g.out32 = out32; g.ld32 = ld32; g.out16 = (__half*)out16; g.ld16 = ld16;
  if (!row_count_invariant) attach_packed(g, L);
  launch_tc_gemm(ctx(), g);
}

void TalkerEngine::forward_stack(const StackWeights& S, float* x, int m, const int* row_slot, const int* row_pos,
                                 const int* win_start, const float* inv_freq, void* kbase, void* vbase, int kv_f16, size_t slot_stride,
                                 size_t layer_stride, int capacity, bool one_row_per_slot, bool decode_step, bool x16_ready) {
  const size_t kv_elem = kv_f16 ? 2 : 4;
  const LaunchCtx c = ctx();
  const int qkv_ld = (S.heads + 2 * S.kv_heads) * 128, attn_ld = S.heads * 128;
  if ((decode_step ? step_tc_ : use_tc(m)) && !S.tc.empty()) {
    const bool fused = decode_step && m <= 128 && tc_skinny_enabled();
    const bool pass0_pairs = decode_step && !one_row_per_slot && win_start == nullptr && row_pos == d_cp_pos2_ && (m % 2) == 0;
    const float inv16 = 1.0f / kX16Div;
    auto consumer = [&](const TcLinear& L, float* out32, int ld32, void* out16, int ld16, int swiglu) {
      TcGemm g;
      g.a = (const __half*)d_h16_; g.w = (const __half*)L.w; g.Bt = 1; g.T = m; g.cin = L.in; g.N = L.out;
      g.bias = L.bias; g.swiglu = swiglu; g.out32 = out32; g.ld32 = ld32; g.out16 = (__half*)out16; g.ld16 = ld16;
      g.rms_eps = S.eps; g.in_scale = inv16; g.allow_skinny = fused; g.k_rotate = fused;
      if (fused) {
        g.rms_in = 1;
        attach_packed(g, L);
      } else {
        launch_row_scale(c, (const __half*)d_h16_, m, S.hidden, inv16, S.eps, d_rs_);
        g.row_scale = d_rs_;
      }
      launch_tc_gemm(c, g);
    };
    auto producer = [&](const TcLinear& L, const void* a16) {
      TcGemm g;
      g.a = (const __half*)a16; g.w = (const __half*)L.w; g.Bt = 1; g.T = m; g.cin = L.in; g.N = L.out;
      g.bias = L.bias; g.res = x; g.ld_res = S.hidden; g.out32 = x; g.ld32 = S.hidden; g.allow_skinny = fused; g.k_rotate = fused;
      if (fused) {
        g.out16 = (__half*)d_h16_; g.ld16 = S.hidden; g.out16_scale = inv16;
        attach_packed(g, L);
        launch_tc_gemm(c, g);
      } else {
        launch_tc_gemm(c, g);
        launch_scale_to_f16(c, x, (size_t)m * S.hidden, inv16, (__half*)d_h16_);
      }
    };
    if (!x16_ready) launch_scale_to_f16(c, x, (size_t)m * S.hidden, inv16, (__half*)d_h16_);
    for (int l = 0; l < S.layers; ++l) {
      const LayerWeights& L = S.layer[l];
      const LayerTc& Tc = S.tc[l];
      KVLayout kv;
      kv.k = static_cast<char*>(kbase) + l * layer_stride * kv_elem; kv.v = static_cast<char*>(vbase) + l * layer_stride * kv_elem;
      kv.slot_stride = slot_stride; kv.capacity = capacity; kv.f16 = kv_f16;
      consumer(Tc.qkv, d_qkv_, qkv_ld, nullptr, 0, 0);
      static const int dbg_skip = getenv("Q3TTS_DEBUG_SKIP") ? atoi(getenv("Q3TTS_DEBUG_SKIP")) : 0;
      if (one_row_per_slot && (dbg_skip & 1)) {
      } else if (one_row_per_slot) {
        launch_rope_attention_f16(c, d_qkv_, qkv_ld, m, S.heads, S.kv_heads, L.q_norm, L.k_norm, S.eps, inv_freq, row_slot, row_pos, win_start, kv,
                                  (__half*)d_attn16_, attn_ld);
      } else if (pass0_pairs) {
        launch_cp_pass0_attention_f16(c, d_qkv_, qkv_ld, m / 2, S.heads, S.kv_heads, L.q_norm, L.k_norm, S.eps, inv_freq, kv, (__half*)d_attn16_, attn_ld);
      } else {
        launch_qk_norm_rope_append(c, d_qkv_, qkv_ld, m, S.heads, S.kv_heads, S.head_dim, L.q_norm, L.k_norm, S.eps, inv_freq, row_slot,
                                   row_pos, kv);
        launch_attention_f16(c, d_qkv_, qkv_ld, m, S.heads, S.kv_heads, S.head_dim, row_slot, row_pos, win_start, kv, (__half*)d_attn16_, attn_ld);
      }
      if (!(dbg_skip & 2)) producer(Tc.o, d_attn16_);
      if (!(dbg_skip & 4)) consumer(Tc.gate_up_il, nullptr, 0, d_act16_, S.inter, 1);
      if (!(dbg_skip & 8)) producer(Tc.down, d_act16_);
    }
    return;
  }
  for (int l = 0; l < S.layers; ++l) {
    const LayerWeights& L = S.layer[l];
    KVLayout kv;
    kv.k = static_cast<char*>(kbase) + l * layer_stride * kv_elem; kv.v = static_cast<char*>(vbase) + l * layer_stride * kv_elem;
    kv.slot_stride = slot_stride; kv.capacity = capacity; kv.f16 = kv_f16;
// ... 67 lines not shown
    const int tp_first = (int)ids.size();
    ids.push_back(r.text_ids[3]);
    const int tp_trailing = (int)ids.size();
    for (int i = 0; i < n_trailing; ++i) ids.push_back(r.text_ids[4 + i]);
    int spk_ref = 0;
    if (spk_by_vec) {
      spk_host.insert(spk_host.end(), r.speaker_embedding, r.speaker_embedding + H);
      spk_ref = (int)(spk_host.size() / H);
    }
    const int row0 = (int)meta_slot.size();
    auto row = [&](int tp, int codec, int spk) {
      desc.push_back(tp); desc.push_back(codec); desc.push_back(spk);
      meta_slot.push_back(slot); meta_pos.push_back((int)meta_slot.size() - 1 - row0);
    };
    for (int i = 0; i < n_front_text; ++i) row(tp_front + i, -1, 0);
    for (int i = 0; i < n_ref_audio; ++i) {
      const int code = r.ref_codes[i];
      Q3_CHECK(code >= 0 && code < cfg_.vocab_size, Q3TTS_ERR_INVALID_ARG, "reference code %d outside codec vocabulary", code);
      row(-1, code, 0);
    }
    for (int i = 0; i < 3; ++i) row(tp_role + i, -1, 0);
    int codec_ids[6], codec_spk[6] = {0, 0, 0, 0, 0, 0};
    int k = 0;
    codec_ids[k++] = cfg_.codec_nothink_id; codec_ids[k++] = cfg_.codec_think_bos_id; codec_ids[k++] = cfg_.codec_think_eos_id;
    if (spk_by_id) codec_ids[k++] = r.speaker_id;
    else if (spk_by_vec) { codec_ids[k] = -1; codec_spk[k] = spk_ref; ++k; }
    codec_ids[k++] = cfg_.codec_pad_id; codec_ids[k++] = cfg_.codec_bos_id;
    for (int i = 0; i < n_codec - 1; ++i) row(i < n_codec - 2 ? TP_PAD : TP_BOS, codec_ids[i], codec_spk[i]);
    row(tp_first, codec_ids[n_codec - 1], 0);
    out[it].prefill_len = P;
    plans.push_back({slot, row0, P, tp_trailing, n_trailing, &r});
  }
  if (plans.empty()) return;
  const int n_tp = (int)ids.size(), R = (int)meta_slot.size();
  Q3_CHECK((int)(spk_host.size() / H) <= opt_.max_batch, Q3TTS_ERR_CAPACITY, "too many speaker embeddings in one admission batch");

  const LaunchCtx c = ctx();
  Q3_CUDA(cudaEventRecord(ev_a_, stream_));
  Q3_CUDA(cudaMemcpyAsync(d_ids_, ids.data(), sizeof(int) * n_tp, cudaMemcpyHostToDevice, stream_));
  Q3_CUDA(cudaMemcpyAsync(d_desc_, desc.data(), sizeof(int) * 3 * R, cudaMemcpyHostToDevice, stream_));
  Q3_CUDA(cudaMemcpyAsync(d_pf_slot_, meta_slot.data(), sizeof(int) * R, cudaMemcpyHostToDevice, stream_));
  Q3_CUDA(cudaMemcpyAsync(d_pf_pos_, meta_pos.data(), sizeof(int) * R, cudaMemcpyHostToDevice, stream_));
  if (!spk_host.empty()) Q3_CUDA(cudaMemcpyAsync(d_spk_, spk_host.data(), sizeof(float) * spk_host.size(), cudaMemcpyHostToDevice, stream_));
  if (use_tc(n_tp)) {
    launch_gather_rows_f16(c, w_.text_embedding, d_ids_, n_tp, (__half*)d_tpe16_, TH);
    linear_tc(w_.fc1_tc, d_tpe16_, n_tp, nullptr, 0, d_tph16_, TH, nullptr, TC_ACT_SILU, 0, true);
    linear_tc(w_.fc2_tc, d_tph16_, n_tp, d_tp_, H, nullptr, 0, nullptr, TC_ACT_NONE, 0, true);
  } else {
    launch_gather_rows(c, w_.text_embedding, d_ids_, n_tp, d_tpe_, TH, false);
    launch_linear(c, w_.fc1, d_tpe_, TH, n_tp, d_tph_, TH, nullptr, 0.f, EPI_SILU);
    launch_linear(c, w_.fc2, d_tph_, TH, n_tp, d_tp_, H, nullptr, 0.f, EPI_STORE);
  }
  launch_assemble_rows(c, d_tp_, H, w_.codec_embedding, d_spk_, d_desc_, R, d_x_);
  for (const Plan& p : plans) {
    float* tr = d_trailing_ + (size_t)p.slot * opt_.max_trailing * H;
    if (p.n_trailing > 0)
      Q3_CUDA(cudaMemcpyAsync(tr, d_tp_ + (size_t)p.tp_trailing * H, sizeof(float) * p.n_trailing * H, cudaMemcpyDeviceToDevice, stream_));
    Q3_CUDA(cudaMemcpyAsync(tr + (size_t)p.n_trailing * H, d_tp_ + (size_t)TP_EOS * H, sizeof(float) * H, cudaMemcpyDeviceToDevice, stream_));
  }
  forward_stack(w_.talker, d_x_, R, d_pf_slot_, d_pf_pos_, d_pf_win_, d_inv_freq_, kcache_, vcache_, kv_f16_, kv_slot_stride_, kv_layer_stride_, C, false, false, false);
  for (const Plan& p : plans) {
    launch_rmsnorm(c, d_x_ + (size_t)(p.row0 + p.P - 1) * H, H, 1, H, w_.talker.final_norm, w_.talker.eps, d_hlast_ + (size_t)p.slot * H, H);
    launch_linear(c, w_.codec_head, d_hlast_ + (size_t)p.slot * H, H, 1, d_logits0_ + (size_t)p.slot * cfg_.vocab_size, cfg_.vocab_size, nullptr, 0.f, EPI_STORE);
  }
  for (const Plan& p : plans) {
    const q3tts_request& r = *p.r;
    const int slot = p.slot;
    const bool forced = r.forced_codes != nullptr && r.n_forced_frames > 0;
    if (forced) {
      Q3_CHECK(r.n_forced_frames <= F, Q3TTS_ERR_CAPACITY, "n_forced_frames %d > max_frames %d", r.n_forced_frames, F);
      Q3_CUDA(cudaMemcpyAsync(d_forced_ + (size_t)slot * F * 16, r.forced_codes, sizeof(int) * 16 * r.n_forced_frames, cudaMemcpyHostToDevice, stream_));
    }
    int logits_cap = 0;
    if ((r.code0_logits_out != nullptr || r.cp_logits_out != nullptr) && r.logits_capacity_frames > 0) {
      Q3_CHECK(slot == 0 || !use_mega(opt_.max_batch), Q3TTS_ERR_INVALID_ARG, "logit dumps on a handle of <= 2 slots are only available for slot 0");
      Q3_CHECK(slot < 4096, Q3TTS_ERR_INVALID_ARG, "logit dumps are limited to slots < 4096");
      logits_cap = std::min(r.logits_capacity_frames, F);
      if (logits_cap > dump_cap_) {
        Q3_CUDA(cudaStreamSynchronize(stream_));
        if (d_dump0_) cudaFree(d_dump0_);
        if (d_dumpcp_) cudaFree(d_dumpcp_);
        Q3_CUDA(cudaMalloc(&d_dump0_, sizeof(float) * (size_t)logits_cap * cfg_.vocab_size));
        Q3_CUDA(cudaMalloc(&d_dumpcp_, sizeof(float) * (size_t)logits_cap * 15 * cfg_.cp.vocab_size));
        dump_cap_ = logits_cap;
        drop_graphs();
      }
      Q3_CUDA(cudaMemsetAsync(d_dump0_, 0, sizeof(float) * (size_t)logits_cap * cfg_.vocab_size, stream_));
      Q3_CUDA(cudaMemsetAsync(d_dumpcp_, 0, sizeof(float) * (size_t)logits_cap * 15 * cfg_.cp.vocab_size, stream_));
    }
    if (logits_cap > 0) { dump_slot_ = slot; dump_enabled_ = true; }
    else if (slot == dump_slot_) dump_enabled_ = false;
    SlotState s{};
    s.active = 1;
    s.pos = p.P;
    s.total_text = p.n_trailing + 1;
    s.max_tokens = forced ? r.n_forced_frames : std::min(std::max(r.max_tokens, 0), F);
    s.n_forced = forced ? r.n_forced_frames : 0;
    s.stream_variant = r.stream_variant ? 1 : 0;
    s.top_k = r.top_k;
    s.logits_cap = logits_cap;
    s.temperature = r.temperature;
    s.top_p = (r.top_p > 0.f) ? r.top_p : 1.0f;
    s.rep_penalty = (r.repetition_penalty > 0.f) ? r.repetition_penalty : 1.0f;
    s.seed = r.seed;
    if (s.max_tokens <= 0) s.finished = 1;
    h_state_[slot] = s;
    Q3_CUDA(cudaMemsetAsync(d_sets_ + (size_t)slot * 16 * set_words_, 0, sizeof(unsigned) * 16 * set_words_, stream_));
  }
  Q3_CUDA(cudaStreamSynchronize(stream_));
  for (const Plan& p : plans)
    Q3_CUDA(cudaMemcpyAsync(d_state_ + p.slot, h_state_ + p.slot, sizeof(SlotState), cudaMemcpyHostToDevice, stream_));
  Q3_CUDA(cudaEventRecord(ev_b_, stream_));
  Q3_CUDA(cudaStreamSynchronize(stream_));
  float ms = 0.f;
  cudaEventElapsedTime(&ms, ev_a_, ev_b_);
  last_prefill_ms += ms;
}

void TalkerEngine::release(int slot) {
  Q3_CUDA(cudaMemsetAsync(d_state_ + slot, 0, sizeof(SlotState), stream_));
}

void TalkerEngine::issue_frame(int n_slots) {
  step_tc_ = use_tc_step(n_slots);
  struct ChainScope {
    bool& on;
    explicit ChainScope(bool& f, bool v) : on(f) { on = v; }
    ~ChainScope() { on = false; }
  } chain_scope(chain_on_, step_tc_ && chain_enabled_ && opt_.use_cuda_graph != 0);
  if (chain_on_) {
    chain_.next = 0;
    chain_.prev = nullptr;
    Q3_CUDA(cudaMemsetAsync(chain_.base, 0, sizeof(unsigned) * kChainCounters, stream_));
  }
  const LaunchCtx c = ctx();
  const int H = cfg_.hidden_size, Hcp = cfg_.cp.hidden_size, V = cfg_.vocab_size, Vc = cfg_.cp.vocab_size;
  const int B = opt_.max_batch, F = opt_.max_frames;
  SamplerParams p{};
  p.vocab = V; p.group = 0; p.codec_vocab = V; p.eos_id = cfg_.codec_eos_token_id; p.pad_id = cfg_.codec_pad_id;
  p.groups = 16; p.set_words = set_words_;
  float* dump0 = dump_enabled_ ? d_dump0_ : nullptr;
  float* dumpcp = dump_enabled_ ? d_dumpcp_ : nullptr;
  const bool x16_direct = step_tc_ && !w_.has_mtp;
  auto next_input = [&](int mode) {
    NextInput ni;
    ni.mode = mode; ni.H = H; ni.h_last = d_hlast_; ni.codec = w_.codec_embedding; ni.cp_emb = d_cp_emb_; ni.y32 = d_cpin_;
    if (step_tc_) { ni.y16 = (__half*)d_h16_; ni.y16_scale = w_.has_mtp ? 1.0f : 1.0f / kX16Div; }
    return ni;
  };
  launch_sample(c, d_logits0_, V, n_slots, d_state_, p, d_sets_, d_cur_codes_, d_forced_, F, dump0, V, 0, dump_slot_, next_input(1));
  for (int g = 0; g < 15; ++g) {
    const int m = g == 0 ? 2 * n_slots : n_slots;
    float* x = d_cpin_;
    if (w_.has_mtp) {
      if (step_tc_) {
        linear_tc(w_.small_to_mtp_tc, d_h16_, m, d_cpx_, Hcp, nullptr, 0, nullptr, TC_ACT_NONE, 0);
      } else {
        launch_linear(c, w_.small_to_mtp, d_cpin_, H, m, d_cpx_, Hcp, nullptr, 0.f, EPI_STORE);
      }
      x = d_cpx_;
    }
    forward_stack(w_.cp, x, m, g == 0 ? d_cp_slot2_ : d_iota_, g == 0 ? d_cp_pos2_ : d_cp_pos_ + (size_t)g * B, nullptr,
                  d_cp_inv_freq_, cp_k_, cp_v_, 0, cpkv_slot_stride_, cpkv_layer_stride_, kCpCapacity, g != 0, true, x16_direct);
    if (step_tc_ && g != 0 && n_slots <= 128 && tc_skinny_enabled()) {
      TcGemm hg;
      hg.a = (const __half*)d_h16_; hg.w = (const __half*)w_.lm_head_tc[g].w; hg.Bt = 1; hg.T = n_slots; hg.cin = Hcp; hg.N = Vc;
      hg.bias = w_.lm_head_tc[g].bias; hg.out32 = d_cplogits_; hg.ld32 = Vc;
      hg.rms_in = 1; hg.rms_eps = w_.cp.eps; hg.in_scale = 1.0f / kX16Div;
      attach_packed(hg, w_.lm_head_tc[g]);
      launch_tc_gemm(c, hg);
    } else if (step_tc_) {
      launch_rmsnorm_f16(c, g == 0 ? x + Hcp : x, g == 0 ? 2 * Hcp : Hcp, n_slots, Hcp, nullptr, w_.cp.eps, (__half*)d_h16_, Hcp);
      linear_tc(w_.lm_head_tc[g], d_h16_, n_slots, d_cplogits_, Vc, nullptr, 0, nullptr, TC_ACT_NONE, 0);
    } else if (g == 0) {
      launch_linear(c, w_.lm_head[0], x + Hcp, 2 * Hcp, n_slots, d_cplogits_, Vc, w_.cp.final_norm, w_.cp.eps, EPI_STORE);
    } else {
      launch_linear(c, w_.lm_head[g], x, Hcp, n_slots, d_cplogits_, Vc, w_.cp.final_norm, w_.cp.eps, EPI_STORE);
    }
    SamplerParams pg = p;
    pg.vocab = Vc; pg.group = g + 1;
    launch_sample(c, d_cplogits_, Vc, n_slots, d_state_, pg, d_sets_, d_cur_codes_, d_forced_, F, dumpcp, 15 * Vc, g * Vc, dump_slot_,
                  g < 14 ? next_input(2) : NextInput());
  }
  launch_frame_finalize(c, n_slots, d_state_, d_cur_codes_, d_frames_, F, d_sets_, set_words_, d_trailing_, opt_.max_trailing,
                        d_tts_ + (size_t)2 * H, w_.codec_embedding, d_cp_emb_, H, d_xstep_, step_tc_ ? (__half*)d_h16_ : nullptr, 1.0f / kX16Div);
  launch_step_rows(c, n_slots, d_state_, d_step_slot_, d_step_pos_, d_win_);
  forward_stack(w_.talker, d_xstep_, n_slots, d_step_slot_, d_step_pos_, d_win_, d_inv_freq_, kcache_, vcache_, kv_f16_, kv_slot_stride_,
                kv_layer_stride_, opt_.kv_capacity, true, true, step_tc_);
  launch_rmsnorm(c, d_xstep_, H, n_slots, H, w_.talker.final_norm, w_.talker.eps, d_hlast_, H);
  if (step_tc_) {
    launch_f32_to_f16(c, d_hlast_, (size_t)n_slots * H, (__half*)d_h16_);
    linear_tc(w_.codec_head_tc, d_h16_, n_slots, d_logits0_, V, nullptr, 0, nullptr, TC_ACT_NONE, 0);
  } else {
    launch_linear(c, w_.codec_head, d_hlast_, H, n_slots, d_logits0_, V, nullptr, 0.f, EPI_STORE);
  }
  launch_step_advance(c, n_slots, d_state_, 192);
}

void TalkerEngine::run_frames(int n_slots, int n) {
  if (n <= 0 || n_slots <= 0) return;
  if (!opt_.use_cuda_graph) {
    for (int i = 0; i < n; ++i) issue_frame(n_slots);
    return;
  }
  if (use_mega(n_slots)) {
    if (mega_.p.trace) Q3_CUDA(cudaMemsetAsync(mega_.p.trace, 0, sizeof(long long) * 2 * mega_.p.trace_stride, stream_));
    launch_frame_megakernel(ctx(), mega_, n_slots, n, dump_enabled_ ? d_dump0_ : nullptr, dump_enabled_ ? d_dumpcp_ : nullptr);
    ++mega_launches;
    if (mega_.p.trace) {
      std::vector<long long> t((size_t)2 * mega_.p.trace_stride);
      Q3_CUDA(cudaMemcpyAsync(t.data(), mega_.p.trace, sizeof(long long) * t.size(), cudaMemcpyDeviceToHost, stream_));
      Q3_CUDA(cudaStreamSynchronize(stream_));
      if (FILE* f = fopen(getenv("Q3TTS_MEGA_TRACE"), "wb")) { fwrite(t.data(), sizeof(long long), t.size(), f); fclose(f); }
    }
    return;
  }
  const long long key = (long long)n_slots * 8192 + (dump_enabled_ ? 1 + dump_slot_ : 0);
  auto it = graphs_.find(key);
  if (it == graphs_.end()) {
    cudaGraph_t g = nullptr;
    if (counter_) { counter_->capturing = true; counter_->captured = 0; }
    Q3_CUDA(cudaStreamBeginCapture(stream_, cudaStreamCaptureModeThreadLocal));
    try {
      issue_frame(n_slots);
    } catch (...) {
      cudaStreamEndCapture(stream_, &g);
      if (g) cudaGraphDestroy(g);
      if (counter_) counter_->capturing = false;
      throw;
    }
    cudaError_t e = cudaStreamEndCapture(stream_, &g);
    if (counter_) counter_->capturing = false;
    if (e != cudaSuccess) fail(Q3TTS_ERR_CUDA, "graph capture failed: %s", cudaGetErrorString(e));
    Graph gr;
    gr.nodes = counter_ ? counter_->captured : 0;
    e = cudaGraphInstantiate(&gr.exec, g, 0);
    cudaGraphDestroy(g);
    if (e != cudaSuccess) fail(Q3TTS_ERR_CUDA, "graph instantiate failed: %s", cudaGetErrorString(e));
    it = graphs_.emplace(key, gr).first;
  }
  for (int i = 0; i < n; ++i) {
    Q3_CUDA(cudaGraphLaunch(it->second.exec, stream_));
    if (counter_) counter_->n += it->second.nodes;
    ++graph_replays;
  }
}

void TalkerEngine::fetch_states(int n_slots, std::vector<SlotState>& out) {
  Q3_CUDA(cudaMemcpyAsync(h_state_, d_state_, sizeof(SlotState) * n_slots, cudaMemcpyDeviceToHost, stream_));
  Q3_CUDA(cudaStreamSynchronize(stream_));
  out.assign(h_state_, h_state_ + n_slots);
}

void TalkerEngine::fetch_frames(int slot, int first, int count, int32_t* dst) {
  if (count <= 0) return;
  Q3_CUDA(cudaMemcpyAsync(dst, d_frames_ + ((size_t)slot * opt_.max_frames + first) * 16, sizeof(int) * 16 * count,
                          cudaMemcpyDeviceToHost, stream_));
  Q3_CUDA(cudaStreamSynchronize(stream_));
}

void TalkerEngine::fetch_logits(int frames, float* code0_out, float* cp_out) {
  frames = std::min(frames, dump_cap_);
  if (frames <= 0) return;
  if (code0_out) Q3_CUDA(cudaMemcpyAsync(code0_out, d_dump0_, sizeof(float) * (size_t)frames * cfg_.vocab_size, cudaMemcpyDeviceToHost, stream_));
  if (cp_out) Q3_CUDA(cudaMemcpyAsync(cp_out, d_dumpcp_, sizeof(float) * (size_t)frames * 15 * cfg_.cp.vocab_size, cudaMemcpyDeviceToHost, stream_));
  Q3_CUDA(cudaStreamSynchronize(stream_));
}

double TalkerEngine::profile_linears(int which, int m, int iters, int64_t& launches, int64_t& bytes_per_iter) {
  const StackWeights& S = which == 0 ? w_.talker : w_.cp;
  Q3_CHECK(m >= 1 && m <= max_rows_, Q3TTS_ERR_INVALID_ARG, "m %d out of range (1..%d)", m, max_rows_);
  const LaunchCtx c{stream_, nullptr};
  const int qkv_ld = (S.heads + 2 * S.kv_heads) * 128, attn_ld = S.heads * 128;
  Q3_CUDA(cudaMemsetAsync(d_x_, 0, sizeof(float) * (size_t)m * S.hidden, stream_));
  Q3_CUDA(cudaMemsetAsync(d_attn_, 0, sizeof(float) * (size_t)m * attn_ld, stream_));
  if (d_h16_) {
    Q3_CUDA(cudaMemsetAsync(d_h16_, 0, (size_t)m * S.hidden * 2, stream_));
    Q3_CUDA(cudaMemsetAsync(d_attn16_, 0, (size_t)m * attn_ld * 2, stream_));
    Q3_CUDA(cudaMemsetAsync(d_act16_, 0, (size_t)m * S.inter * 2, stream_));
  }
  launches = 0;
  bytes_per_iter = 0;
  const bool tc = handle_tc_ && m >= tc_min_rows_step_ && !S.tc.empty();
  auto pass = [&](bool count) {
    for (int l = 0; l < S.layers; ++l) {
      const LayerWeights& L = S.layer[l];
      if (tc) {
        const LayerTc& T = S.tc[l];
        linear_tc(T.qkv, d_h16_, m, d_qkv_, qkv_ld, nullptr, 0, nullptr, TC_ACT_NONE, 0);
        linear_tc(T.o, d_attn16_, m, d_x_, S.hidden, nullptr, 0, nullptr, TC_ACT_NONE, 0);
        linear_tc(T.gate_up_il, d_h16_, m, nullptr, 0, d_act16_, S.inter, nullptr, TC_ACT_NONE, 1);
        linear_tc(T.down, d_act16_, m, d_x_, S.hidden, nullptr, 0, nullptr, TC_ACT_NONE, 0);
        if (count) { launches += 4; bytes_per_iter += (int64_t)(L.qkv.weight_bytes() + L.o.weight_bytes() + L.gate_up.weight_bytes() + L.down.weight_bytes()); }
        continue;
      }
      launch_linear(c, L.qkv, d_x_, S.hidden, m, d_qkv_, qkv_ld, L.in_norm, S.eps, EPI_STORE);
      launch_linear(c, L.o, d_attn_, attn_ld, m, d_x_, S.hidden, nullptr, 0.f, EPI_ADD);
      launch_linear(c, L.gate_up, d_x_, S.hidden, m, d_act_, S.inter, L.post_norm, S.eps, EPI_SWIGLU);
      launch_linear(c, L.down, d_act_, S.inter, m, d_x_, S.hidden, nullptr, 0.f, EPI_ADD);
      if (count) { launches += 4; bytes_per_iter += (int64_t)(L.qkv.weight_bytes() + L.o.weight_bytes() + L.gate_up.weight_bytes() + L.down.weight_bytes()); }
    }
    if (tc) {
      const TcLinear& head = which == 0 ? w_.codec_head_tc : w_.lm_head_tc[0];
      linear_tc(head, d_h16_, m, which == 0 ? d_logits0_ : d_cplogits_, head.out, nullptr, 0, nullptr, TC_ACT_NONE, 0);
      if (count) { launches += 1; bytes_per_iter += (int64_t)(which == 0 ? w_.codec_head : w_.lm_head[0]).weight_bytes(); }
      return;
    }
    const Linear& head = which == 0 ? w_.codec_head : w_.lm_head[0];
    launch_linear(c, head, d_x_, S.hidden, m, which == 0 ? d_logits0_ : d_cplogits_, head.out, S.final_norm, S.eps, EPI_STORE);
    if (count) { launches += 1; bytes_per_iter += (int64_t)head.weight_bytes(); }
  };
  pass(true);
  struct ChainScope {
    bool& on;
    explicit ChainScope(bool& f, bool v) : on(f) { on = v; }
    ~ChainScope() { on = false; }
  } chain_scope(chain_on_, tc && chain_enabled_);
  cudaGraph_t graph = nullptr;
  cudaGraphExec_t exec = nullptr;
  Q3_CUDA(cudaStreamBeginCapture(stream_, cudaStreamCaptureModeThreadLocal));
  if (chain_on_) {
    chain_.next = 0;
    chain_.prev = nullptr;
    Q3_CUDA(cudaMemsetAsync(chain_.base, 0, sizeof(unsigned) * kChainCounters, stream_));
  }
  pass(false);
  Q3_CUDA(cudaStreamEndCapture(stream_, &graph));
  Q3_CUDA(cudaGraphInstantiate(&exec, graph, 0));
  Q3_CUDA(cudaGraphLaunch(exec, stream_));
  Q3_CUDA(cudaEventRecord(ev_a_, stream_));
  for (int i = 0; i < iters; ++i) Q3_CUDA(cudaGraphLaunch(exec, stream_));
  Q3_CUDA(cudaEventRecord(ev_b_, stream_));
  Q3_CUDA(cudaStreamSynchronize(stream_));
  float ms = 0.f;
  cudaEventElapsedTime(&ms, ev_a_, ev_b_);
  cudaGraphExecDestroy(exec);
  cudaGraphDestroy(graph);
  launches *= iters;
  return ms;
}

int TalkerEngine::sample_probe(const float* logits, int vocab, float temperature, int top_k, float top_p, float rep_penalty,
                               const int32_t* token_set, int n_set, uint64_t seed, uint64_t counter) {
  Q3_CHECK(vocab > 0 && vocab <= 4096, Q3TTS_ERR_INVALID_ARG, "vocab %d out of range", vocab);
  std::vector<unsigned> bm(128, 0u);
  for (int i = 0; i < n_set; ++i)
    if (token_set[i] >= 0 && token_set[i] < vocab) bm[token_set[i] >> 5] |= 1u << (token_set[i] & 31);
  Q3_CUDA(cudaMemcpyAsync(d_probe_logits_, logits, sizeof(float) * vocab, cudaMemcpyHostToDevice, stream_));
  Q3_CUDA(cudaMemcpyAsync(d_probe_set_, bm.data(), sizeof(unsigned) * 128, cudaMemcpyHostToDevice, stream_));
  launch_sample_probe(ctx(), d_probe_logits_, vocab, cfg_.vocab_size, temperature, top_k, top_p > 0.f ? top_p : 1.f,
                      rep_penalty > 0.f ? rep_penalty : 1.f, n_set > 0 ? d_probe_set_ : nullptr, seed, counter, d_probe_out_);
  int id = -1;
  Q3_CUDA(cudaMemcpyAsync(&id, d_probe_out_, sizeof(int), cudaMemcpyDeviceToHost, stream_));
  Q3_CUDA(cudaStreamSynchronize(stream_));
  return id;
}

}
```

mlx-swift-qwen3-tts_b200/csrc/talker_kernels.cu:

```cuda
#include <cuda_bf16.h>
#include <cuda_fp16.h>

#include "kernels.h"
#include "device_utils.cuh"
#include "sampler.cuh"

namespace q3 {

__global__ void dequantize_kernel(const uint32_t* __restrict__ qw, const void* __restrict__ scales,
                                  const void* __restrict__ biases, int sdt, int out, int in, int group, int bits,
                                  int out_dt, void* __restrict__ dst) {
  const int per = 32 / bits;
  const size_t words = (size_t)out * (in / per);
  const uint32_t mask = (1u << bits) - 1u;
  for (size_t wi = (size_t)blockIdx.x * blockDim.x + threadIdx.x; wi < words; wi += (size_t)gridDim.x * blockDim.x) {
    const size_t row = wi / (in / per);
    const int col0 = (int)(wi % (in / per)) * per;
    const uint32_t w = qw[wi];
    const size_t gi = row * (in / group) + col0 / group;
    const float s = load_as_f32(scales, gi, sdt), b = load_as_f32(biases, gi, sdt);
    for (int j = 0; j < per; ++j) {
      const float q = (float)((w >> (j * bits)) & mask);
      const float v = __fadd_rn(__fmul_rn(s, q), b);
      const size_t o = row * in + col0 + j;
      if (out_dt == Q3TTS_F32) reinterpret_cast<float*>(dst)[o] = v;
      else if (out_dt == Q3TTS_F16) reinterpret_cast<__half*>(dst)[o] = __float2half_rn(v);
      else reinterpret_cast<__nv_bfloat16*>(dst)[o] = __float2bfloat16_rn(v);
    }
  }
}

void launch_dequantize(const LaunchCtx& c, const uint32_t* qw, const void* scales, const void* biases, int sdt, int out,
                       int in, int group, int bits, int out_dt, void* dst) {
  const size_t words = (size_t)out * in * bits / 32;
  int blocks = (int)std::min<size_t>((words + 255) / 256, 148 * 16);
  if (blocks < 1) blocks = 1;
  dequantize_kernel<<<blocks, 256, 0, c.stream>>>(qw, scales, biases, sdt, out, in, group, bits, out_dt, dst);
  c.tick();
}

__global__ void mlx_quantize_kernel(const void* __restrict__ w, int wdt, size_t groups, int in, int bits, uint32_t* __restrict__ qw8,
                                    void* __restrict__ scales, void* __restrict__ biases, void* __restrict__ fake) {
  const size_t g = (size_t)blockIdx.x * blockDim.x + threadIdx.x;
  if (g >= groups) return;
  const int gpr = in / 64;
  const size_t row = g / gpr;
  const size_t e0 = row * (size_t)in + (size_t)(g - row * gpr) * 64;
  float v[64];
  float mx = -INFINITY, mn = INFINITY;
#pragma unroll 8
  for (int j = 0; j < 64; ++j) {
    v[j] = load_as_f32(w, e0 + j, wdt);
    mx = fmaxf(mx, v[j]);
    mn = fminf(mn, v[j]);
  }
  const float n_bins = (float)((1 << bits) - 1);
  const bool side = fabsf(mn) > fabsf(mx);
  float s = fmaxf(__fdiv_rn(__fsub_rn(mx, mn), n_bins), 1e-7f);
  s = side ? s : -s;
  const float edge = side ? mn : mx;
  const float q0 = rintf(__fdiv_rn(edge, s));
  if (q0 != 0.f) s = __fdiv_rn(edge, q0);
  float b = q0 == 0.f ? 0.f : edge;
  if (wdt == Q3TTS_BF16) { s = __bfloat162float(__float2bfloat16_rn(s)); b = __bfloat162float(__float2bfloat16_rn(b)); }
  else if (wdt == Q3TTS_F16) { s = __half2float(__float2half_rn(s)); b = __half2float(__float2half_rn(b)); }
  const float s_safe = s == 0.f ? 1e-7f : s;
  if (wdt == Q3TTS_F32) { reinterpret_cast<float*>(scales)[g] = s; reinterpret_cast<float*>(biases)[g] = b; }
  else if (wdt == Q3TTS_F16) { reinterpret_cast<__half*>(scales)[g] = __float2half_rn(s); reinterpret_cast<__half*>(biases)[g] = __float2half_rn(b); }
  else { reinterpret_cast<__nv_bfloat16*>(scales)[g] = __float2bfloat16_rn(s); reinterpret_cast<__nv_bfloat16*>(biases)[g] = __float2bfloat16_rn(b); }
#pragma unroll 4
  for (int j = 0; j < 64; j += 4) {
    uint32_t word = 0;
#pragma unroll
    for (int u = 0; u < 4; ++u) {
      const float q = fminf(fmaxf(rintf(__fdiv_rn(__fsub_rn(v[j + u], b), s_safe)), 0.f), n_bins);
      word |= (uint32_t)q << (8 * u);
      if (fake) {
        const float d = __fadd_rn(__fmul_rn(s, q), b);
        const size_t o = e0 + j + u;
        if (wdt == Q3TTS_F32) reinterpret_cast<float*>(fake)[o] = d;
        else if (wdt == Q3TTS_F16) reinterpret_cast<__half*>(fake)[o] = __float2half_rn(d);
        else reinterpret_cast<__nv_bfloat16*>(fake)[o] = __float2bfloat16_rn(d);
      }
    }
    if (qw8) qw8[(e0 + j) >> 2] = word;
  }
}

void launch_mlx_quantize(const LaunchCtx& c, const void* w, int wdt, int out, int in, int bits, uint32_t* qw8, void* scales, void* biases,
                         void* fake) {
  Q3_CHECK(in % 64 == 0 && (bits == 4 || bits == 6 || bits == 8), Q3TTS_ERR_INVALID_ARG, "mlx_quantize: in %d / bits %d unsupported", in, bits);
  const size_t groups = (size_t)out * (in / 64);
  mlx_quantize_kernel<<<(unsigned)((groups + 127) / 128), 128, 0, c.stream>>>(w, wdt, groups, in, bits, qw8, scales, biases, fake);
  c.tick();
}

struct LinearKArgs {
  const void* w;
  const void* scales;
  const void* biases;
  const float* bias;
  const float* x;
  float* y;
  const float* norm_w;
  float eps;
  int out, in, group, sdt, m, ldx, ldy, epi;
};

template <int FMT, int MT>
__global__ void __launch_bounds__(256, (MT <= 2 ? 3 : 1)) linear_kernel(const LinearKArgs a) {
  constexpr int VPL = FmtTraits<FMT>::VPL;
  constexpr int KC = 32 * VPL;
  constexpr bool QUANT = (FMT == W_Q4 || FMT == W_Q8);
  constexpr int LPG = VPL / 4;
  extern __shared__ __align__(16) unsigned char smem_raw[];
  const int nchunk = (a.in + KC - 1) / KC;
  const int xstride = nchunk * (KC / 4);
  float4* xs = reinterpret_cast<float4*>(smem_raw);
  float* xsum = reinterpret_cast<float*>(smem_raw + (size_t)MT * xstride * sizeof(float4));
  __shared__ float red[MT][8];

  const int tid = threadIdx.x, lane = tid & 31, warp = tid >> 5;
  const int m0 = blockIdx.y * MT;
  const int in4 = a.in >> 2;
  const int out_eff = (a.epi == EPI_SWIGLU) ? (a.out >> 1) : a.out;
  const int nsub = (a.epi == EPI_SWIGLU) ? 2 : 1;
  const size_t row_bytes = QUANT ? (size_t)a.in * (FMT == W_Q4 ? 4 : 8) / 8 : (size_t)a.in * (FMT == W_F32 ? 4 : 2);
  const int ngroups = QUANT ? a.in / a.group : 0;
  const int r_first = blockIdx.x * 8 + warp;

  if (r_first < out_eff) {
    for (int s = 0; s < nsub; ++s) {
      const int row = r_first + s * out_eff;
      const unsigned char* wr = reinterpret_cast<const unsigned char*>(a.w) + (size_t)row * row_bytes;
      for (size_t off = (size_t)lane * 128; off < row_bytes; off += 32 * 128) prefetch_l2(wr + off);
      if constexpr (QUANT) {
        if (lane == 0) prefetch_l2(reinterpret_cast<const unsigned char*>(a.scales) + (size_t)row * ngroups * (a.sdt == Q3TTS_F32 ? 4 : 2));
        if (lane == 1) prefetch_l2(reinterpret_cast<const unsigned char*>(a.biases) + (size_t)row * ngroups * (a.sdt == Q3TTS_F32 ? 4 : 2));
      }
    }
  }

  const int iters = (in4 + 255) / 256;
#pragma unroll
  for (int mi = 0; mi < MT; ++mi) {
    const bool valid = (m0 + mi) < a.m;
    const float4* xr = reinterpret_cast<const float4*>(a.x + (size_t)(valid ? m0 + mi : 0) * a.ldx);
    float ss = 0.f;
    for (int it = 0; it < iters; ++it) {
      const int f = tid + it * 256;
      float4 v = make_float4(0.f, 0.f, 0.f, 0.f);
      if (valid && f < in4) v = xr[f];
      ss += v.x * v.x + v.y * v.y + v.z * v.z + v.w * v.w;
      if (a.norm_w != nullptr && f < in4) {
        const float4 nw = reinterpret_cast<const float4*>(a.norm_w)[f];
        v.x *= nw.x; v.y *= nw.y; v.z *= nw.z; v.w *= nw.w;
      }
// ... 22 lines not shown
      float s = 0.f;
#pragma unroll
      for (int w = 0; w < 8; ++w) s += red[mi][w];
      inv_rms[mi] = rsqrtf(s / (float)a.in + a.eps);
    }
  }

  for (int r = r_first; r < out_eff; r += gridDim.x * 8) {
    float yold[MT];
#pragma unroll
    for (int mi = 0; mi < MT; ++mi) yold[mi] = (a.epi == EPI_ADD && lane == 0 && m0 + mi < a.m) ? a.y[(size_t)(m0 + mi) * a.ldy + r] : 0.f;
    float res[2][MT];
#pragma unroll
    for (int s = 0; s < 2; ++s) {
#pragma unroll
      for (int mi = 0; mi < MT; ++mi) res[s][mi] = 0.f;
    }
#pragma unroll
    for (int s = 0; s < 2; ++s) {
      if (s >= nsub) break;
      const int row = r + s * out_eff;
      const uint4* wr = reinterpret_cast<const uint4*>(reinterpret_cast<const unsigned char*>(a.w) + (size_t)row * row_bytes);
      float acc[MT];
#pragma unroll
      for (int mi = 0; mi < MT; ++mi) acc[mi] = 0.f;
      for (int c0 = 0; c0 < nchunk; c0 += 4) {
        uint4 wv[4];
        float scv[4], biv[4];
#pragma unroll
        for (int u = 0; u < 4; ++u) {
          if ((c0 + u) * KC + lane * VPL < a.in) {
            wv[u] = ldg_stream(wr + (size_t)(c0 + u) * 32 + lane);
            if constexpr (QUANT) {
              const size_t gi = (size_t)row * ngroups + ((c0 + u) * KC + lane * VPL) / a.group;
              scv[u] = load_as_f32(a.scales, gi, a.sdt);
              biv[u] = load_as_f32(a.biases, gi, a.sdt);
            }
          }
        }
#pragma unroll
        for (int u = 0; u < 4; ++u) {
          if ((c0 + u) * KC + lane * VPL < a.in) {
            const int ch = c0 + u;
            float wf[VPL];
            lane_expand<FMT>(wv[u], wf);
#pragma unroll
            for (int mi = 0; mi < MT; ++mi) {
              const float d = lane_dot<FMT>(wf, xs + (size_t)mi * xstride + ch * (KC / 4) + lane);
              if constexpr (QUANT) acc[mi] += scv[u] * d + biv[u] * xsum[mi * (nchunk * 32) + ch * 32 + lane];
              else acc[mi] += d;
            }
          }
        }
      }
#pragma unroll
      for (int mi = 0; mi < MT; ++mi) res[s][mi] = warp_sum(acc[mi]) * inv_rms[mi];
    }
    if (lane == 0) {
#pragma unroll
      for (int mi = 0; mi < MT; ++mi) {
        if (m0 + mi >= a.m) break;
        float v = res[0][mi];
        float* yp = a.y + (size_t)(m0 + mi) * a.ldy + r;
        if (a.epi == EPI_SWIGLU) {
          float g = v, u = res[1][mi];
          if (a.bias) { g += a.bias[r]; u += a.bias[r + out_eff]; }
          *yp = silu_f(g) * u;
        } else {
          if (a.bias) v += a.bias[r];
          if (a.epi == EPI_SILU) v = silu_f(v);
          if (a.epi == EPI_ADD) v += yold[mi];
          *yp = v;
        }
      }
    }
  }
}

template <int FMT, int MT>
static void launch_linear_t(const LaunchCtx& c, const LinearKArgs& a, int num_sms) {
  constexpr int VPL = FmtTraits<FMT>::VPL;
  constexpr bool QUANT = (FMT == W_Q4 || FMT == W_Q8);
  constexpr int KC = 32 * VPL;
  const int nchunk = (a.in + KC - 1) / KC;
  size_t smem = (size_t)MT * nchunk * KC * sizeof(float) + (QUANT ? (size_t)MT * nchunk * 32 * sizeof(float) : 0);
  const int out_eff = (a.epi == EPI_SWIGLU) ? a.out / 2 : a.out;
  int bx = (out_eff + 7) / 8;
  const int cap = num_sms * 8;
  if (bx > cap) bx = cap;
  dim3 grid(bx, (a.m + MT - 1) / MT);
  linear_kernel<FMT, MT><<<grid, 256, smem, c.stream>>>(a);
  c.tick();
}

template <int FMT>
static void launch_linear_f(const LaunchCtx& c, LinearKArgs a) {
  int mt = 8;
  while (mt > 1 && (mt > a.m * 2 - 1 || (size_t)mt * a.in * 5 > 96 * 1024)) mt >>= 1;
  if (a.m == 1) mt = 1;
  switch (mt) {
    case 8: launch_linear_t<FMT, 8>(c, a, 148); break;
    case 4: launch_linear_t<FMT, 4>(c, a, 148); break;
    case 2: launch_linear_t<FMT, 2>(c, a, 148); break;
    default: launch_linear_t<FMT, 1>(c, a, 148); break;
  }
}

void launch_linear(const LaunchCtx& c, const Linear& L, const float* x, int ldx, int m, float* y, int ldy,
                   const float* norm_w, float eps, int epilogue) {
  if (m <= 0) return;
  LinearKArgs a;
  a.w = L.bits ? (const void*)L.qw : L.w;
  a.scales = L.scales; a.biases = L.biases; a.bias = L.bias;
  a.x = x; a.y = y; a.norm_w = norm_w; a.eps = eps;
  a.out = L.out; a.in = L.in; a.group = L.group; a.sdt = L.sdt; a.m = m; a.ldx = ldx; a.ldy = ldy; a.epi = epilogue;
  Q3_CHECK((ldx % 4) == 0, Q3TTS_ERR_INVALID_ARG, "linear: activation stride %d not 16-byte aligned", ldx);
  if (L.bits == 4) {
    Q3_CHECK(L.in % 32 == 0 && L.group % 32 == 0, Q3TTS_ERR_BAD_CONFIG, "4-bit linear needs in %% 32 == 0 and group %% 32 == 0 (in=%d, group=%d)", L.in, L.group);
    launch_linear_f<W_Q4>(c, a);
  } else if (L.bits == 8) {
    Q3_CHECK(L.in % 16 == 0 && L.group % 16 == 0, Q3TTS_ERR_BAD_CONFIG, "8-bit linear needs in %% 16 == 0 (in=%d)", L.in);
    launch_linear_f<W_Q8>(c, a);
  } else if (L.bits == 0) {
    if (L.sdt == Q3TTS_BF16) { Q3_CHECK(L.in % 8 == 0, Q3TTS_ERR_BAD_CONFIG, "bf16 linear needs in %% 8 == 0 (in=%d)", L.in); launch_linear_f<W_BF16>(c, a); }
    else if (L.sdt == Q3TTS_F16) { Q3_CHECK(L.in % 8 == 0, Q3TTS_ERR_BAD_CONFIG, "f16 linear needs in %% 8 == 0 (in=%d)", L.in); launch_linear_f<W_F16>(c, a); }
    else { Q3_CHECK(L.in % 4 == 0, Q3TTS_ERR_BAD_CONFIG, "f32 linear needs in %% 4 == 0 (in=%d)", L.in); launch_linear_f<W_F32>(c, a); }
  } else {
    fail(Q3TTS_ERR_BAD_CONFIG, "unsupported quantisation bits %d (4 and 8 are in scope; 6-bit runtime quantisation is not)", L.bits);
  }
}

__global__ void __launch_bounds__(256) rmsnorm_kernel(const float* __restrict__ x, int ldx, int dim, const float* __restrict__ w,
                                                      float eps, float* __restrict__ y, int ldy) {
  __shared__ float red[8];
  const float* xr = x + (size_t)blockIdx.x * ldx;
  float ss = 0.f;
  for (int i = threadIdx.x; i < dim; i += 256) { const float v = xr[i]; ss += v * v; }
  ss = warp_sum(ss);
  if ((threadIdx.x & 31) == 0) red[threadIdx.x >> 5] = ss;
  __syncthreads();
  float tot = 0.f;
#pragma unroll
  for (int i = 0; i < 8; ++i) tot += red[i];
  const float inv = rsqrtf(tot / (float)dim + eps);
  float* yr = y + (size_t)blockIdx.x * ldy;
  for (int i = threadIdx.x; i < dim; i += 256) yr[i] = xr[i] * inv * w[i];
}
void launch_rmsnorm(const LaunchCtx& c, const float* x, int ldx, int m, int dim, const float* w, float eps, float* y, int ldy) {
  if (m <= 0) return;
  rmsnorm_kernel<<<m, 256, 0, c.stream>>>(x, ldx, dim, w, eps, y, ldy);
  c.tick();
}

__device__ __forceinline__ float4 kv_ld4(const float* p) { return *reinterpret_cast<const float4*>(p); }
__device__ __forceinline__ float4 kv_ld4(const __half* p) {
  const uint2 u = *reinterpret_cast<const uint2*>(p);
  const float2 a = __half22float2(*reinterpret_cast<const __half2*>(&u.x)), b = __half22float2(*reinterpret_cast<const __half2*>(&u.y));
  return make_float4(a.x, a.y, b.x, b.y);
}
__device__ __forceinline__ float kv_ld(const float* p) { return *p; }
__device__ __forceinline__ float kv_ld(const __half* p) { return __half2float(*p); }
__device__ __forceinline__ void kv_st(float* p, float v) { *p = v; }
__device__ __forceinline__ void kv_st(__half* p, float v) { *p = __float2half_rn(v); }
template <typename KvT>
__global__ void __launch_bounds__(128) qk_norm_rope_append_kernel(float* __restrict__ qkv, int ld, int m, int heads, int kv_heads,
                                                                  const float* __restrict__ q_norm, const float* __restrict__ k_norm,
                                                                  float eps, const float* __restrict__ inv_freq,
                                                                  const int* __restrict__ row_slot, const int* __restrict__ row_pos,
                                                                  KVLayout kv) {
  const int total_heads = heads + 2 * kv_heads;
  const int gw = blockIdx.x * 4 + (threadIdx.x >> 5);
  if (gw >= m * total_heads) return;
  const int row = gw / total_heads, head = gw - row * total_heads;
  const int lane = threadIdx.x & 31;
  float* p = qkv + (size_t)row * ld + (size_t)head * 128;
  const int slot = row_slot[row], pos = row_pos[row];
  const int ring = pos % kv.capacity;
  if (head >= heads + kv_heads) {
    KvT* dst = static_cast<KvT*>(kv.v) + (size_t)slot * kv.slot_stride + ((size_t)(head - heads - kv_heads) * kv.capacity + ring) * 128;
    const float4 v4 = reinterpret_cast<const float4*>(p)[lane];
    kv_st(dst + 4 * lane, v4.x); kv_st(dst + 4 * lane + 1, v4.y); kv_st(dst + 4 * lane + 2, v4.z); kv_st(dst + 4 * lane + 3, v4.w);
    return;
  }
  const float a0 = p[lane], a1 = p[lane + 32], b0 = p[lane + 64], b1 = p[lane + 96];
  const float ss = warp_sum(a0 * a0 + a1 * a1 + b0 * b0 + b1 * b1);
  const float inv = rsqrtf(ss * (1.0f / 128.0f) + eps);
  const float* nw = head < heads ? q_norm : k_norm;
  const float x0 = a0 * inv * nw[lane], x1 = a1 * inv * nw[lane + 32];
  const float y0 = b0 * inv * nw[lane + 64], y1 = b1 * inv * nw[lane + 96];
  const float fp = (float)pos;
  float s0, c0, s1, c1;
  sincosf(fp * inv_freq[lane], &s0, &c0);
  sincosf(fp * inv_freq[lane + 32], &s1, &c1);
  const float o0 = x0 * c0 - y0 * s0, o1 = x1 * c1 - y1 * s1;
  const float o2 = y0 * c0 + x0 * s0, o3 = y1 * c1 + x1 * s1;
  if (head >= heads) {
    KvT* dst = static_cast<KvT*>(kv.k) + (size_t)slot * kv.slot_stride + ((size_t)(head - heads) * kv.capacity + ring) * 128;
    kv_st(dst + lane, o0); kv_st(dst + lane + 32, o1); kv_st(dst + lane + 64, o2); kv_st(dst + lane + 96, o3);
  } else {
    p[lane] = o0; p[lane + 32] = o1; p[lane + 64] = o2; p[lane + 96] = o3;
  }
}
void launch_qk_norm_rope_append(const LaunchCtx& c, float* qkv, int ld, int m, int heads, int kv_heads, int head_dim,
                                const float* q_norm, const float* k_norm, float eps, const float* inv_freq,
                                const int* row_slot, const int* row_pos, const KVLayout& kv) {
  Q3_CHECK(head_dim == 128, Q3TTS_ERR_BAD_CONFIG, "talker kernels are specialised for head_dim 128 (got %d)", head_dim);
  const int warps = m * (heads + 2 * kv_heads);
  if (warps <= 0) return;
  if (kv.f16)
    qk_norm_rope_append_kernel<__half><<<(warps + 3) / 4, 128, 0, c.stream>>>(qkv, ld, m, heads, kv_heads, q_norm, k_norm, eps, inv_freq, row_slot, row_pos, kv);
  else
    qk_norm_rope_append_kernel<float><<<(warps + 3) / 4, 128, 0, c.stream>>>(qkv, ld, m, heads, kv_heads, q_norm, k_norm, eps, inv_freq, row_slot, row_pos, kv);
  c.tick();
}

__device__ __forceinline__ void store_act(float* p, float v) { *p = v; }
__device__ __forceinline__ void store_act(__half* p, float v) { *p = __float2half_rn(v); }

template <int G, typename OutT, typename KvT>
__global__ void __launch_bounds__(128) attention_kernel(const float* __restrict__ qkv, int ld, int heads, int kv_heads,
                                                        const int* __restrict__ row_slot, const int* __restrict__ row_pos,
                                                        const int* __restrict__ win_start, KVLayout kv, OutT* __restrict__ out,
                                                        int ldo, float scale) {
  extern __shared__ __align__(16) float sm[];
  float* q = sm;
  float* sc = sm + G * 128;
  __shared__ float red_max[G], red_sum[G];
  const int row = blockIdx.x, kvh = blockIdx.y, tid = threadIdx.x, lane = tid & 31, warp = tid >> 5;
  const int slot = row_slot[row], pos = row_pos[row];
  const int w0 = win_start ? win_start[slot] : 0;
  const int S = pos - w0 + 1;
  const int cap = kv.capacity;
  const int r0 = w0 % cap;
  const KvT* kb = static_cast<const KvT*>(kv.k) + (size_t)slot * kv.slot_stride + (size_t)kvh * cap * 128;
  const KvT* vb = static_cast<const KvT*>(kv.v) + (size_t)slot * kv.slot_stride + (size_t)kvh * cap * 128;
#pragma unroll
  for (int g = 0; g < G; ++g) q[g * 128 + tid] = qkv[(size_t)row * ld + (size_t)(kvh * G + g) * 128 + tid];
  __syncthreads();
  for (int j = tid; j < S; j += 128) {
    const int rj = r0 + j;
    const KvT* kr = kb + (size_t)(rj >= cap ? rj - cap : rj) * 128;
    float acc[G];
#pragma unroll
    for (int g = 0; g < G; ++g) acc[g] = 0.f;
#pragma unroll 8
    for (int d = 0; d < 32; ++d) {
      const float4 kk = kv_ld4(kr + 4 * d);
#pragma unroll
      for (int g = 0; g < G; ++g) {
        const float4 qq = reinterpret_cast<const float4*>(q + g * 128)[d];
        acc[g] += kk.x * qq.x + kk.y * qq.y + kk.z * qq.z + kk.w * qq.w;
      }
    }
#pragma unroll
    for (int g = 0; g < G; ++g) sc[g * S + j] = acc[g] * scale;
  }
  __syncthreads();
  for (int g = warp; g < G; g += 4) {
    float mx = -INFINITY;
    for (int j = lane; j < S; j += 32) mx = fmaxf(mx, sc[g * S + j]);
    mx = warp_max(mx);
    float sum = 0.f;
    for (int j = lane; j < S; j += 32) { const float e = expf(sc[g * S + j] - mx); sc[g * S + j] = e; sum += e; }
    sum = warp_sum(sum);
    if (lane == 0) { red_max[g] = mx; red_sum[g] = sum; }
  }
  __syncthreads();
  float o[G];
#pragma unroll
  for (int g = 0; g < G; ++g) o[g] = 0.f;
  for (int j = 0; j < S; ++j) {
    const int rj = r0 + j;
    const float vv = kv_ld(vb + (size_t)(rj >= cap ? rj - cap : rj) * 128 + tid);
#pragma unroll
    for (int g = 0; g < G; ++g) o[g] = fmaf(sc[g * S + j], vv, o[g]);
  }
#pragma unroll
  for (int g = 0; g < G; ++g) store_act(out + (size_t)row * ldo + (size_t)(kvh * G + g) * 128 + tid, o[g] / red_sum[g]);
}
template <int G, typename OutT, typename KvT>
__global__ void __launch_bounds__(128, 4) rope_attention_kernel(const float* __restrict__ qkv, int ld, int heads, int kv_heads,
                                                             const float* __restrict__ q_norm, const float* __restrict__ k_norm, float eps,
                                                             const float* __restrict__ inv_freq, const int* __restrict__ row_slot,
                                                             const int* __restrict__ row_pos, const int* __restrict__ win_start, KVLayout kv,
                                                             OutT* __restrict__ out, int ldo, float scale, const ChainSig sig) {
  __shared__ __align__(16) float q[G * 128];
  __shared__ __align__(16) float part_o[4][G][128];
  __shared__ float part_m[4][G], part_l[4][G];
  pdl_launch_dependents();
  if (sig.in) {
    if (threadIdx.x == 0) chain_wait(sig.in, sig.in_target);
    __syncthreads();
  } else {
    pdl_wait();
  }
  const int row = blockIdx.x, kvh = blockIdx.y, tid = threadIdx.x, lane = tid & 31, warp = tid >> 5;
  const int slot = row_slot[row], pos = row_pos[row];
  const int w0 = win_start ? win_start[slot] : 0;
  const int S = pos - w0 + 1;
  const int cap = kv.capacity;
  const int r0 = w0 % cap;
  const int ring = (r0 + S - 1 >= cap) ? r0 + S - 1 - cap : r0 + S - 1;
  KvT* kb = static_cast<KvT*>(kv.k) + (size_t)slot * kv.slot_stride + (size_t)kvh * cap * 128;
  KvT* vb = static_cast<KvT*>(kv.v) + (size_t)slot * kv.slot_stride + (size_t)kvh * cap * 128;
  const float* rowp = qkv + (size_t)row * ld;
  for (int hh = warp; hh <= G; hh += 4) {
    const float* src = rowp + (size_t)(hh < G ? (kvh * G + hh) : (heads + kvh)) * 128;
    const float a0 = src[lane], a1 = src[lane + 32], b0 = src[lane + 64], b1 = src[lane + 96];
    const float ss = warp_sum(a0 * a0 + a1 * a1 + b0 * b0 + b1 * b1);
    const float inv = rsqrtf(ss * (1.0f / 128.0f) + eps);
    const float* nw = hh < G ? q_norm : k_norm;
    const float x0 = a0 * inv * nw[lane], x1 = a1 * inv * nw[lane + 32], y0 = b0 * inv * nw[lane + 64], y1 = b1 * inv * nw[lane + 96];
    float s0, c0, s1, c1;
    sincosf((float)pos * inv_freq[lane], &s0, &c0);
    sincosf((float)pos * inv_freq[lane + 32], &s1, &c1);
    const float o0 = x0 * c0 - y0 * s0, o1 = x1 * c1 - y1 * s1, o2 = y0 * c0 + x0 * s0, o3 = y1 * c1 + x1 * s1;
    if (hh < G) {
      float* dst = q + hh * 128;
      dst[lane] = o0; dst[lane + 32] = o1; dst[lane + 64] = o2; dst[lane + 96] = o3;
    } else {
      KvT* dst = kb + (size_t)ring * 128;
      kv_st(dst + lane, o0); kv_st(dst + lane + 32, o1); kv_st(dst + lane + 64, o2); kv_st(dst + lane + 96, o3);
    }
  }
  kv_st(vb + (size_t)ring * 128 + tid, rowp[(size_t)(heads + kv_heads + kvh) * 128 + tid]);
  __syncthreads();
  const int seg = lane & 7, grp = warp * 4 + (lane >> 3);
  float qf[G][16];
#pragma unroll
  for (int g = 0; g < G; ++g)
#pragma unroll
    for (int i = 0; i < 4; ++i) {
      const float4 t = *reinterpret_cast<const float4*>(q + g * 128 + i * 32 + seg * 4);
      qf[g][4 * i] = t.x * scale; qf[g][4 * i + 1] = t.y * scale; qf[g][4 * i + 2] = t.z * scale; qf[g][4 * i + 3] = t.w * scale;
    }
  float mx[G], l[G], o[G][16];
#pragma unroll
  for (int g = 0; g < G; ++g) {
    mx[g] = -INFINITY; l[g] = 0.f;
#pragma unroll
    for (int d = 0; d < 16; ++d) o[g][d] = 0.f;
  }
  for (int jb = 0; jb < S; jb += 32) {
    const int j0 = jb + grp;
    float4 kk[2][4], vv[2][4];
#pragma unroll
    for (int u = 0; u < 2; ++u) {
      const int j = j0 + 16 * u;
      const int rj = r0 + (j < S ? j : 0);
      const size_t base = (size_t)(rj >= cap ? rj - cap : rj) * 128 + seg * 4;
#pragma unroll
      for (int i = 0; i < 4; ++i) {
        kk[u][i] = kv_ld4(kb + base + i * 32);
        vv[u][i] = kv_ld4(vb + base + i * 32);
      }
    }
#pragma unroll
    for (int u = 0; u < 2; ++u) {
      const bool valid = j0 + 16 * u < S;
#pragma unroll
      for (int g = 0; g < G; ++g) {
        float sdot = 0.f;
#pragma unroll
        for (int i = 0; i < 4; ++i)
          sdot += kk[u][i].x * qf[g][4 * i] + kk[u][i].y * qf[g][4 * i + 1] + kk[u][i].z * qf[g][4 * i + 2] + kk[u][i].w * qf[g][4 * i + 3];
        sdot += __shfl_xor_sync(0xffffffffu, sdot, 1);
        sdot += __shfl_xor_sync(0xffffffffu, sdot, 2);
        sdot += __shfl_xor_sync(0xffffffffu, sdot, 4);
        if (!valid) sdot = -INFINITY;
        const float mn = fmaxf(mx[g], sdot);
        const bool none = mn == -INFINITY;
        const float corr = none ? 1.f : expf(mx[g] - mn), pr = none ? 0.f : expf(sdot - mn);
        mx[g] = mn;
        l[g] = l[g] * corr + pr;
#pragma unroll
        for (int i = 0; i < 4; ++i) {
          o[g][4 * i] = o[g][4 * i] * corr + pr * vv[u][i].x;
          o[g][4 * i + 1] = o[g][4 * i + 1] * corr + pr * vv[u][i].y;
          o[g][4 * i + 2] = o[g][4 * i + 2] * corr + pr * vv[u][i].z;
          o[g][4 * i + 3] = o[g][4 * i + 3] * corr + pr * vv[u][i].w;
        }
      }
    }
  }
#pragma unroll
  for (int g = 0; g < G; ++g) {
    float m_all = fmaxf(mx[g], __shfl_xor_sync(0xffffffffu, mx[g], 8));
    m_all = fmaxf(m_all, __shfl_xor_sync(0xffffffffu, m_all, 16));
    const float f = (mx[g] == -INFINITY) ? 0.f : expf(mx[g] - m_all);
    float lw = l[g] * f;
    lw += __shfl_xor_sync(0xffffffffu, lw, 8);
    lw += __shfl_xor_sync(0xffffffffu, lw, 16);
#pragma unroll
    for (int d = 0; d < 16; ++d) {
      float t = o[g][d] * f;
      t += __shfl_xor_sync(0xffffffffu, t, 8);
      t += __shfl_xor_sync(0xffffffffu, t, 16);
      o[g][d] = t;
    }
    if (lane < 8) {
#pragma unroll
      for (int i = 0; i < 4; ++i)
        *reinterpret_cast<float4*>(&part_o[warp][g][i * 32 + seg * 4]) = make_float4(o[g][4 * i], o[g][4 * i + 1], o[g][4 * i + 2], o[g][4 * i + 3]);
      if (lane == 0) { part_m[warp][g] = m_all; part_l[warp][g] = lw; }
    }
  }
  __syncthreads();
#pragma unroll
  for (int g = 0; g < G; ++g) {
    float m_all = fmaxf(fmaxf(part_m[0][g], part_m[1][g]), fmaxf(part_m[2][g], part_m[3][g]));
    float num = 0.f, den = 0.f;
#pragma unroll
    for (int w = 0; w < 4; ++w) {
      const float f = (part_m[w][g] == -INFINITY) ? 0.f : expf(part_m[w][g] - m_all);
      num += part_o[w][g][tid] * f;
      den += part_l[w][g] * f;
    }
    store_act(out + (size_t)row * ldo + (size_t)(kvh * G + g) * 128 + tid, num / den);
  }
  if (sig.out) {
    __syncthreads();
    if (threadIdx.x == 0) chain_signal(sig.out);
  }
}
template <int G>
__global__ void __launch_bounds__(128) cp_pass0_attention_kernel(const float* __restrict__ qkv, int ld, int heads, int kv_heads,
                                                                 const float* __restrict__ q_norm, const float* __restrict__ k_norm, float eps,
                                                                 const float* __restrict__ inv_freq, KVLayout kv, __half* __restrict__ out,
                                                                 int ldo, float scale, const ChainSig sig) {
  __shared__ __align__(16) float q1[G * 128];
  __shared__ __align__(16) float kk[2][128];
  __shared__ __align__(16) float vv[2][128];
  __shared__ float w0[G], w1[G];
  pdl_launch_dependents();
  if (sig.in) {
    if (threadIdx.x == 0) chain_wait(sig.in, sig.in_target);
    __syncthreads();
  } else {
    pdl_wait();
  }
  const int slot = blockIdx.x, kvh = blockIdx.y, tid = threadIdx.x, lane = tid & 31, warp = tid >> 5;
  float* kb = static_cast<float*>(kv.k) + (size_t)slot * kv.slot_stride + (size_t)kvh * kv.capacity * 128;
  float* vb = static_cast<float*>(kv.v) + (size_t)slot * kv.slot_stride + (size_t)kvh * kv.capacity * 128;
  for (int item = warp; item < G + 2; item += 4) {
    const int pos = item < G ? 1 : item - G;
    const float* rowp = qkv + (size_t)(2 * slot + pos) * ld;
    const float* src = rowp + (size_t)(item < G ? (kvh * G + item) : (heads + kvh)) * 128;
    const float a0 = src[lane], a1 = src[lane + 32], b0 = src[lane + 64], b1 = src[lane + 96];
    const float ss = warp_sum(a0 * a0 + a1 * a1 + b0 * b0 + b1 * b1);
    const float inv = rsqrtf(ss * (1.0f / 128.0f) + eps);
    const float* nw = item < G ? q_norm : k_norm;
    const float x0 = a0 * inv * nw[lane], x1 = a1 * inv * nw[lane + 32], y0 = b0 * inv * nw[lane + 64], y1 = b1 * inv * nw[lane + 96];
    float s0 = 0.f, c0 = 1.f, s1 = 0.f, c1 = 1.f;
    if (pos == 1) {
      sincosf(inv_freq[lane], &s0, &c0);
      sincosf(inv_freq[lane + 32], &s1, &c1);
    }
    const float o0 = x0 * c0 - y0 * s0, o1 = x1 * c1 - y1 * s1, o2 = y0 * c0 + x0 * s0, o3 = y1 * c1 + x1 * s1;
    float* dst = item < G ? q1 + item * 128 : kk[pos];
    dst[lane] = o0; dst[lane + 32] = o1; dst[lane + 64] = o2; dst[lane + 96] = o3;
    if (item >= G) {
      float* kd = kb + (size_t)pos * 128;
      kd[lane] = o0; kd[lane + 32] = o1; kd[lane + 64] = o2; kd[lane + 96] = o3;
    }
  }
#pragma unroll
  for (int pos = 0; pos < 2; ++pos) {
    const float v = qkv[(size_t)(2 * slot + pos) * ld + (size_t)(heads + kv_heads + kvh) * 128 + tid];
    vv[pos][tid] = v;
    vb[(size_t)pos * 128 + tid] = v;
  }
  __syncthreads();
  for (int g = warp; g < G; g += 4) {
    float d0 = 0.f, d1 = 0.f;
#pragma unroll
    for (int i = 0; i < 4; ++i) {
      const float qv = q1[g * 128 + lane + 32 * i];
      d0 = fmaf(qv, kk[0][lane + 32 * i], d0);
      d1 = fmaf(qv, kk[1][lane + 32 * i], d1);
    }
    d0 = warp_sum(d0) * scale;
    d1 = warp_sum(d1) * scale;
    const float mx = fmaxf(d0, d1);
    const float e0 = expf(d0 - mx), e1 = expf(d1 - mx);
    if (lane == 0) { w0[g] = e0 / (e0 + e1); w1[g] = e1 / (e0 + e1); }
  }
  __syncthreads();
#pragma unroll
  for (int g = 0; g < G; ++g) {
    out[(size_t)(2 * slot) * ldo + (size_t)(kvh * G + g) * 128 + tid] = __float2half_rn(vv[0][tid]);
    out[(size_t)(2 * slot + 1) * ldo + (size_t)(kvh * G + g) * 128 + tid] = __float2half_rn(w0[g] * vv[0][tid] + w1[g] * vv[1][tid]);
  }
  if (sig.out) {
    __syncthreads();
    if (threadIdx.x == 0) chain_signal(sig.out);
  }
}
void launch_cp_pass0_attention_f16(const LaunchCtx& c, const float* qkv, int ld, int n_slots, int heads, int kv_heads, const float* q_norm,
                                   const float* k_norm, float eps, const float* inv_freq, const KVLayout& kv, __half* out, int ldo) {
  if (n_slots <= 0) return;
  const int G = heads / kv_heads;
  const float scale = 1.0f / sqrtf(128.0f);
  dim3 grid(n_slots, kv_heads);
  const bool pdl = pdl_enabled();
  Q3_CHECK(G == 1 || G == 2 || G == 4, Q3TTS_ERR_BAD_CONFIG, "unsupported GQA group size %d", G);
  const ChainSig sig = pdl ? c.chain_link((unsigned)(n_slots * kv_heads)) : ChainSig();
  if (G == 1) launch_kernel_pdl(cp_pass0_attention_kernel<1>, grid, dim3(128), 0, c.stream, pdl, qkv, ld, heads, kv_heads, q_norm, k_norm, eps, inv_freq, kv, out, ldo, scale, sig);
  else if (G == 2) launch_kernel_pdl(cp_pass0_attention_kernel<2>, grid, dim3(128), 0, c.stream, pdl, qkv, ld, heads, kv_heads, q_norm, k_norm, eps, inv_freq, kv, out, ldo, scale, sig);
  else launch_kernel_pdl(cp_pass0_attention_kernel<4>, grid, dim3(128), 0, c.stream, pdl, qkv, ld, heads, kv_heads, q_norm, k_norm, eps, inv_freq, kv, out, ldo, scale, sig);
  if (sig.out) c.tick_chained(); else c.tick();
}

template <typename OutT>
static void launch_rope_attention_t(const LaunchCtx& c, const float* qkv, int ld, int m, int heads, int kv_heads, const float* q_norm,
                                    const float* k_norm, float eps, const float* inv_freq, const int* row_slot, const int* row_pos,
                                    const int* win_start, const KVLayout& kv, OutT* out, int ldo) {
  if (m <= 0) return;
  const int G = heads / kv_heads;
  const float scale = 1.0f / sqrtf(128.0f);
  const size_t smem = 0;
  dim3 grid(m, kv_heads);
  const bool pdl = pdl_enabled();
  Q3_CHECK(G == 1 || G == 2 || G == 4, Q3TTS_ERR_BAD_CONFIG, "unsupported GQA group size %d", G);
  const ChainSig sig = pdl ? c.chain_link((unsigned)(m * kv_heads)) : ChainSig();
#define RA_LAUNCH(GV)                                                                                                                              \
  {                                                                                                                                                \
    if (kv.f16) launch_kernel_pdl(rope_attention_kernel<GV, OutT, __half>, grid, dim3(128), smem, c.stream, pdl, qkv, ld, heads, kv_heads, q_norm, k_norm, eps, \
                                  inv_freq, row_slot, row_pos, win_start, kv, out, ldo, scale, sig);                                               \
    else launch_kernel_pdl(rope_attention_kernel<GV, OutT, float>, grid, dim3(128), smem, c.stream, pdl, qkv, ld, heads, kv_heads, q_norm, k_norm, eps,         \
                           inv_freq, row_slot, row_pos, win_start, kv, out, ldo, scale, sig);                                                      \
  }
  if (G == 1) RA_LAUNCH(1)
  else if (G == 2) RA_LAUNCH(2)
  else RA_LAUNCH(4)
#undef RA_LAUNCH
  if (sig.out) c.tick_chained(); else c.tick();
}
void launch_rope_attention(const LaunchCtx& c, const float* qkv, int ld, int m, int heads, int kv_heads, const float* q_norm,
                           const float* k_norm, float eps, const float* inv_freq, const int* row_slot, const int* row_pos,
                           const int* win_start, const KVLayout& kv, float* out, int ldo) {
  launch_rope_attention_t<float>(c, qkv, ld, m, heads, kv_heads, q_norm, k_norm, eps, inv_freq, row_slot, row_pos, win_start, kv, out, ldo);
}
void launch_rope_attention_f16(const LaunchCtx& c, const float* qkv, int ld, int m, int heads, int kv_heads, const float* q_norm,
                               const float* k_norm, float eps, const float* inv_freq, const int* row_slot, const int* row_pos,
                               const int* win_start, const KVLayout& kv, __half* out, int ldo) {
  launch_rope_attention_t<__half>(c, qkv, ld, m, heads, kv_heads, q_norm, k_norm, eps, inv_freq, row_slot, row_pos, win_start, kv, out, ldo);
}

template <typename OutT>
static void launch_attention_t(const LaunchCtx& c, const float* qkv, int ld, int m, int heads, int kv_heads, int head_dim,
                               const int* row_slot, const int* row_pos, const int* win_start, const KVLayout& kv, OutT* out, int ldo) {
  Q3_CHECK(head_dim == 128, Q3TTS_ERR_BAD_CONFIG, "talker kernels are specialised for head_dim 128 (got %d)", head_dim);
  if (m <= 0) return;
  const int G = heads / kv_heads;
  const float scale = 1.0f / sqrtf((float)head_dim);
  const size_t smem = (size_t)G * (128 + kv.capacity) * sizeof(float);
  dim3 grid(m, kv_heads);
#define Q3_ATT(GV)                                                                                                     \
  {                                                                                                                    \
    if (kv.f16) attention_kernel<GV, OutT, __half><<<grid, 128, smem, c.stream>>>(qkv, ld, heads, kv_heads, row_slot, row_pos, win_start, kv, out, ldo, scale); \
    else attention_kernel<GV, OutT, float><<<grid, 128, smem, c.stream>>>(qkv, ld, heads, kv_heads, row_slot, row_pos, win_start, kv, out, ldo, scale); \
  }
  Q3_CHECK(smem <= 160 * 1024, Q3TTS_ERR_CAPACITY, "kv_capacity %d too large for the attention kernel", kv.capacity);
  if (G == 1) Q3_ATT(1) else if (G == 2) Q3_ATT(2) else if (G == 4) Q3_ATT(4)
  else fail(Q3TTS_ERR_BAD_CONFIG, "unsupported GQA group size %d", G);
#undef Q3_ATT
  c.tick();
}
void launch_attention(const LaunchCtx& c, const float* qkv, int ld, int m, int heads, int kv_heads, int head_dim,
                      const int* row_slot, const int* row_pos, const int* win_start, const KVLayout& kv, float* out, int ldo) {
  launch_attention_t<float>(c, qkv, ld, m, heads, kv_heads, head_dim, row_slot, row_pos, win_start, kv, out, ldo);
}
// ... 266 lines not shown
```

Measured before the change: 1115.

## Fuse code-predictor pass into one persistent cooperative cluster kernel

Adds a persistent cooperative kernel with 8-CTA clusters that runs a whole code-predictor pass (all layer GEMMs via TMA and tcgen05 UMMA, plus fused rope attention) in one launch. Cross-stage ordering uses global readiness counters with a timeout and error reporting. The attention body is moved into a shared device function so the existing kernel and the new kernel use the same code. The aim is to cut per-layer launch and synchronisation overhead in the small-batch decode path, at the cost of spin-wait complexity, a possible deadlock guarded only by the timeout, and a dependence on cooperative cluster launches being accepted inside stream capture.

Result: slower. 576.9, median of 6 (-48.3%).

```diff
diff --git a/mlx-swift-qwen3-tts_b200/csrc/api.cu b/mlx-swift-qwen3-tts_b200/csrc/api.cu
--- a/mlx-swift-qwen3-tts_b200/csrc/api.cu
+++ b/mlx-swift-qwen3-tts_b200/csrc/api.cu
@@ -499,6 +499,8 @@
       h->cfg = parent->cfg;
       h->talker.reset(new TalkerEngine(h->model_dir, h->cfg, h->opt, h->stream, &h->counter, parent->talker->shared()));
       h->has_talker = true;
+      Q3_CUDA(cudaStreamSynchronize(parent->stream));
+      parent->talker->drop_graphs();
     }
     if (parent->codec) {
       h->codec.reset(new CodecDecoder(h->model_dir + "/speech_tokenizer", h->stream, &h->counter, h->opt.codec_max_frames));
diff --git a/mlx-swift-qwen3-tts_b200/csrc/cp_pass.cu b/mlx-swift-qwen3-tts_b200/csrc/cp_pass.cu
--- /dev/null
+++ b/mlx-swift-qwen3-tts_b200/csrc/cp_pass.cu
@@ -0,0 +1,338 @@
+#include <cuda.h>
+
+#include <algorithm>
+
+#include "cp_pass.h"
+#include "rope_attention.cuh"
+
+namespace q3 {
+
+namespace {
+
+using namespace skinny;
+
+constexpr int kCluster = 8;
+constexpr int kStages = 3;
+constexpr int kCtrlBytes = 1024;
+constexpr int kG = 2;
+
+__device__ __forceinline__ unsigned ld_acquire(const unsigned* p) {
+  unsigned v;
+  asm volatile("ld.acquire.gpu.global.u32 %0, [%1];" : "=r"(v) : "l"(p) : "memory");
+  return v;
+}
+__device__ __forceinline__ unsigned ld_volatile(const unsigned* p) { return *(const volatile unsigned*)p; }
+
+__device__ bool cp_wait(const CpPassParams& p, int phase, int item, unsigned target) {
+  const unsigned* c = p.cnt + phase * kCpItems + item;
+  if (ld_acquire(c) >= target) return true;
+  const unsigned long long t0 = sk_globaltimer();
+  while (true) {
+    for (int i = 0; i < 64; ++i)
+      if (ld_acquire(c) >= target) return true;
+    if (ld_volatile(p.err) != 0) return false;
+    if (sk_globaltimer() - t0 > p.timeout_ns) {
+      atomicCAS(p.err, 0u, 1u + (((unsigned)p.pass << 16) | ((unsigned)phase << 8) | (unsigned)item));
+      return false;
+    }
+  }
+}
+
+__device__ __forceinline__ int gemm_phase(int k, int layers) { return k == 4 * layers ? 5 * layers : 5 * (k >> 2) + 1 + ((k & 3) == 0 ? -1 : (k & 3)); }
+
+__device__ bool gemm_deps(const CpPassParams& p, int k, int kb0, int kb1) {
+  const int layers = p.layers, l = k >> 2, kind = k == 4 * layers ? 4 : (k & 3);
+  bool ok = true;
+  if (kind == 0 || kind == 2 || kind == 4) {
+    if (kind == 0 && l == 0) return true;
+    const int prev = kind == 2 ? 4 * l + 1 : (kind == 0 ? 4 * (l - 1) + 3 : 4 * (layers - 1) + 3);
+    const int tiles = (p.sk[prev].N + kRowsW - 1) / kRowsW;
+    for (int t = 0; t < tiles; ++t) ok = ok && cp_wait(p, gemm_phase(prev, layers), t, (unsigned)p.sk[prev].split);
+  } else if (kind == 1) {
+    const int g0 = kb0 * kBlockK / (kG * 128), g1 = (kb1 * kBlockK - 1) / (kG * 128);
+    for (int g = g0; g <= g1; ++g) ok = ok && cp_wait(p, 5 * l + 1, g, (unsigned)p.M);
+  } else {
+    const int gu = 4 * l + 2;
+    for (int t = kb0; t < kb1; ++t) ok = ok && cp_wait(p, gemm_phase(gu, layers), t, (unsigned)p.sk[gu].split);
+  }
+  return ok;
+}
+
+__device__ __forceinline__ void cp_stamp(const CpPassParams& p, int slot) {
+  if (p.trace) p.trace[((size_t)p.pass * gridDim.x + blockIdx.x) * 32 + slot] = sk_globaltimer();
+}
+
+struct CpSmem {
+  uint8_t* sW;
+  uint8_t* sX;
+  float* red;
+  uint64_t *full, *empty, *tmem_full, *red_full, *ack;
+  uint32_t* tmem_slot;
+  float* rowscale;
+};
+
+__global__ void __launch_bounds__(kThreads, 2) cp_pass_kernel(const __grid_constant__ CpPassParams p) {
+  extern __shared__ uint8_t smem_raw[];
+  __shared__ RopeAttnSmem<kG> att;
+  uint8_t* smem = reinterpret_cast<uint8_t*>((reinterpret_cast<uintptr_t>(smem_raw) + 1023) & ~(uintptr_t)1023);
+  const int m_pad = p.sk[0].m_pad;
+  const int x_bytes = m_pad * kBlockK * 2;
+  CpSmem s;
+  s.full = reinterpret_cast<uint64_t*>(smem);
+  s.empty = s.full + kStages;
+  s.tmem_full = s.empty + kStages;
+  s.red_full = s.tmem_full + 1;
+  s.ack = s.red_full + 1;
+  s.tmem_slot = reinterpret_cast<uint32_t*>(s.ack + 4);
+  s.rowscale = reinterpret_cast<float*>(smem + 512);
+  s.sW = smem + kCtrlBytes;
+  s.sX = s.sW + (size_t)kStages * kWBytes;
+  s.red = reinterpret_cast<float*>(s.sX + (size_t)kStages * x_bytes);
+
+  const int warp = threadIdx.x >> 5;
+  const uint32_t crank = cluster_ctarank();
+  const int cid = blockIdx.x / kCluster, ncl = gridDim.x / kCluster;
+  const int tmem_cols = std::max(32, m_pad);
+  const int layers = p.layers;
+
+  if (threadIdx.x == 0) {
+    cp_stamp(p, 0);
+    for (int i = 0; i < kStages; ++i) { mbar_init(&s.full[i], 1); mbar_init(&s.empty[i], 1); }
+    mbar_init(s.tmem_full, 1);
+    mbar_init(s.red_full, 1);
+    for (int i = 0; i < 4; ++i) mbar_init(&s.ack[i], i == 0 ? 1 : (1 << i) - 1);
+    asm volatile("fence.mbarrier_init.release.cluster;" ::: "memory");
+    asm volatile("fence.proxy.async.shared::cta;" ::: "memory");
+  }
+  if (warp == 1) {
+    asm volatile("tcgen05.alloc.cta_group::1.sync.aligned.shared::cta.b32 [%0], %1;" ::"r"(smem_u32(s.tmem_slot)), "r"(tmem_cols) : "memory");
+    asm volatile("tcgen05.relinquish_alloc_permit.cta_group::1.sync.aligned;" ::: "memory");
+  }
+  tc_fence_before();
+  cluster_arrive_release();
+  cluster_wait_acquire();
+  tc_fence_after();
+  const uint32_t tmem_base = *s.tmem_slot;
+
+  uint32_t kc = 0;
+  uint32_t jobs = 0, red_uses = 0;
+  uint32_t ack_par = 0;
+
+  for (int l = 0; l <= layers; ++l) {
+    for (int part = 0; part < 5; ++part) {
+      if (l == layers && part > 0) break;
+      const bool attention = l < layers && part == 1;
+      const int phase = l == layers ? 5 * layers : 5 * l + part;
+      if (attention) {
+        if (warp >= 2) {
+          const int tid = threadIdx.x - 64;
+          const int items = p.M * p.kv_heads;
+          for (int it = blockIdx.x; it < items; it += gridDim.x) {
+            const int row = it / p.kv_heads, kvh = it - row * p.kv_heads;
+            const int qt = kvh * kG, kt = p.heads + kvh, vt = p.heads + p.kv_heads + kvh;
+            const int qkv_phase = 5 * l;
+            if (tid == 0) {
+              const unsigned need = (unsigned)p.sk[4 * l].split;
+              bool ok = true;
+              for (int h = 0; h < kG; ++h) ok = ok && cp_wait(p, qkv_phase, qt + h, need);
+              ok = ok && cp_wait(p, qkv_phase, kt, need) && cp_wait(p, qkv_phase, vt, need);
+            }
+            ra_bar(1);
+            rope_attention_item<kG, __half, float>(att, 1, tid, row, kvh, p.qkv, p.ld_qkv, p.heads, p.kv_heads, p.q_norm[l], p.k_norm[l], p.eps,
+                                                   p.inv_freq, p.row_slot, p.row_pos, nullptr, p.kv[l], p.attn16, p.ld_attn, p.scale);
+            ra_bar(1);
+            if (tid == 0) chain_signal(p.cnt + phase * kCpItems + kvh);
+          }
+          if (threadIdx.x == 64) cp_stamp(p, 1 + phase);
+        }
+        continue;
+      }
+      const int k = l == layers ? 4 * layers : 4 * l + (part == 0 ? 0 : part - 1);
+      const SkParams& sp0 = p.sk[k];
+      const int S = sp0.split, tpc = kCluster / S;
+      const int tiles = (sp0.N + kRowsW - 1) / kRowsW;
+      const int J = (tiles + tpc - 1) / tpc;
+      const uint32_t sub = crank / (uint32_t)S, lr = crank & (uint32_t)(S - 1), rb = sub * (uint32_t)S;
+      int sidx = 0;
+      while ((1 << sidx) < S) ++sidx;
+      const int kb0 = (int)((lr * (uint32_t)sp0.num_kb) >> sp0.split_shift);
+      const int kb1 = (int)(((lr + 1u) * (uint32_t)sp0.num_kb) >> sp0.split_shift);
+      const int nkb = kb1 - kb0;
+      for (int j = cid; j < J; j += ncl) {
+        const int tile = j * tpc + (int)sub;
+        const int n0 = tile * kRowsW;
+        if (tile < tiles) {
+          if (warp == 0) {
+            const bool lead = elect_one();
+            const int pre = nkb < kStages ? nkb : kStages;
+            if (lead) {
+              for (int i = 0; i < pre; ++i) {
+                const uint32_t q = kc + (uint32_t)i, st = q % kStages;
+                mbar_wait(&s.empty[st], ((q / kStages) & 1u) ^ 1u);
+                mbar_expect_tx(&s.full[st], (uint32_t)(kWBytes + x_bytes));
+                tma_load_2d(s.sW + (size_t)st * kWBytes, &p.wmap[k], &s.full[st], (kb0 + i) * kBlockK, n0);
+              }
+              for (int i = pre; i < nkb; ++i) tma_prefetch_2d(&p.wmap[k], (kb0 + i) * kBlockK, n0);
+              if (k + 1 < 4 * layers + 1 && j == cid) {
+                const SkParams& np = p.sk[k + 1];
+                const int ntpc = kCluster / np.split;
+                const uint32_t nsub = crank / (uint32_t)np.split, nlr = crank & (uint32_t)(np.split - 1);
+                const int ntile = cid * ntpc + (int)nsub;
+                const int nb0 = (int)((nlr * (uint32_t)np.num_kb) >> np.split_shift), nb1 = (int)(((nlr + 1u) * (uint32_t)np.num_kb) >> np.split_shift);
+                if (ntile * kRowsW < np.N)
+                  for (int i = nb0; i < nb1; ++i) tma_prefetch_2d(&p.wmap[k + 1], i * kBlockK, ntile * kRowsW);
+              }
+              gemm_deps(p, k, kb0, kb1);
+              asm volatile("fence.proxy.async;" ::: "memory");
+            }
+            __syncwarp();
+            for (int i = 0; i < nkb; ++i) {
+              const uint32_t q = kc + (uint32_t)i, st = q % kStages;
+              if (i >= pre) mbar_wait(&s.empty[st], ((q / kStages) & 1u) ^ 1u);
+              if (lead) {
+                if (i >= pre) {
+                  mbar_expect_tx(&s.full[st], (uint32_t)(kWBytes + x_bytes));
+                  tma_load_2d(s.sW + (size_t)st * kWBytes, &p.wmap[k], &s.full[st], (kb0 + i) * kBlockK, n0);
+                }
+                tma_load_2d(s.sX + (size_t)st * x_bytes, &p.xmap[k], &s.full[st], (kb0 + i) * kBlockK, 0);
+              }
+            }
+            __syncwarp();
+          } else if (warp == 1) {
+            const bool lead = elect_one();
+            const uint32_t idesc = (1u << 4) | ((uint32_t)(m_pad >> 3) << 17) | ((uint32_t)(kRowsW >> 4) << 24);
+            for (int i = 0; i < nkb; ++i) {
+              const uint32_t q = kc + (uint32_t)i, st = q % kStages;
+              mbar_wait(&s.full[st], (q / kStages) & 1u);
+              tc_fence_after();
+              const uint64_t ad = umma_desc(smem_u32(s.sW + (size_t)st * kWBytes));
+              const uint64_t bd = umma_desc(smem_u32(s.sX + (size_t)st * x_bytes));
+              if (lead) {
+#pragma unroll
+                for (int kk = 0; kk < kBlockK / 16; ++kk)
+                  umma_f16(tmem_base, ad + (uint64_t)(2 * kk), bd + (uint64_t)(2 * kk), idesc, (i | kk) != 0 ? 1u : 0u);
+                umma_commit(&s.empty[st]);
+              }
+            }
+            if (lead) umma_commit(s.tmem_full);
+            __syncwarp();
+          } else {
+            if ((threadIdx.x & 31) == 0) gemm_deps(p, k, kb0, kb1);
+            __syncwarp();
+            if (sp0.rms_x) sk_row_factors(sp0, s.rowscale, lr);
+            mbar_wait(s.tmem_full, jobs & 1u);
+            tc_fence_after();
+            if (sp0.swiglu)
+              sk_reduce_epilogue<TC_ACT_NONE, true>(sp0, reinterpret_cast<float*>(s.sW), s.red, s.red_full, &s.ack[sidx], s.rowscale, tmem_base, lr, n0, rb, red_uses & 1u,
+                                (ack_par >> sidx) & 1u);
+            else
+              sk_reduce_epilogue<TC_ACT_NONE, false>(sp0, reinterpret_cast<float*>(s.sW), s.red, s.red_full, &s.ack[sidx], s.rowscale, tmem_base, lr, n0, rb, red_uses & 1u,
+                                 (ack_par >> sidx) & 1u);
+            ra_bar(1);
+            if (threadIdx.x == 64) chain_signal(p.cnt + gemm_phase(k, layers) * kCpItems + tile);
+          }
+          kc += (uint32_t)nkb;
+          ++jobs;
+          if (S > 1) { ++red_uses; ack_par ^= 1u << sidx; }
+        }
+        tc_fence_before();
+        cluster_arrive_release();
+        cluster_wait_acquire();
+        tc_fence_after();
+      }
+      if (threadIdx.x == 64) cp_stamp(p, 1 + phase);
+    }
+  }
+  __syncthreads();
+  if (warp == 1) {
+    tc_fence_after();
+    asm volatile("tcgen05.dealloc.cta_group::1.sync.aligned.b32 %0, %1;" ::"r"(tmem_base), "r"(tmem_cols) : "memory");
+  }
+  __shared__ unsigned last;
+  if (threadIdx.x == 0) {
+    __threadfence();
+    last = atomicAdd(p.done, 1u) == gridDim.x - 1;
+  }
+  __syncthreads();
+  if (last) {
+    __threadfence();
+    for (int i = threadIdx.x; i < kCpPhaseSlots * kCpItems; i += blockDim.x) p.cnt[i] = 0;
+    if (threadIdx.x == 0) *p.done = 0;
+  }
+}
+
+__global__ void cp_probe_kernel(int* out) {
+  cluster_arrive_release();
+  cluster_wait_acquire();
+  if (threadIdx.x == 0 && blockIdx.x == 0) *out = 1;
+}
+
+cudaLaunchConfig_t cp_config(dim3 grid, size_t smem, cudaStream_t stream, cudaLaunchAttribute* attr) {
+  cudaLaunchConfig_t cfg{};
+  cfg.gridDim = grid;
+  cfg.blockDim = dim3(kThreads);
+  cfg.dynamicSmemBytes = smem;
+  cfg.stream = stream;
+  attr[0].id = cudaLaunchAttributeClusterDimension;
+  attr[0].val.clusterDim.x = kCluster; attr[0].val.clusterDim.y = 1; attr[0].val.clusterDim.z = 1;
+  attr[1].id = cudaLaunchAttributeCooperative;
+  attr[1].val.cooperative = 1;
+  cfg.attrs = attr;
+  cfg.numAttrs = 2;
+  return cfg;
+}
+
+}
+
+size_t cp_pass_smem(int m_pad) {
+  return 1024 + kCtrlBytes + (size_t)kStages * (kWBytes + m_pad * kBlockK * 2) + (size_t)kRowsW * m_pad * 4;
+}
+
+int cp_pass_init(int m_pad, std::string& why) {
+  const size_t smem = cp_pass_smem(m_pad);
+  cudaError_t e = cudaFuncSetAttribute(cp_pass_kernel, cudaFuncAttributeMaxDynamicSharedMemorySize, (int)smem);
+  if (e != cudaSuccess) { why = std::string("shared memory attribute: ") + cudaGetErrorString(e); cudaGetLastError(); return 0; }
+  cudaLaunchAttribute attr[2];
+  cudaLaunchConfig_t cfg = cp_config(dim3(kCluster), smem, nullptr, attr);
+  int clusters = 0;
+  e = cudaOccupancyMaxActiveClusters(&clusters, cp_pass_kernel, &cfg);
+  if (e != cudaSuccess || clusters < 1) {
+    why = std::string("no resident 8-CTA cluster: ") + (e != cudaSuccess ? cudaGetErrorString(e) : "occupancy 0");
+    cudaGetLastError();
+    return 0;
+  }
+  cudaStream_t st = nullptr;
+  int* d = nullptr;
+  int h = 0;
+  cudaGraph_t g = nullptr;
+  cudaGraphExec_t ge = nullptr;
+  bool ok = cudaStreamCreateWithFlags(&st, cudaStreamNonBlocking) == cudaSuccess && cudaMalloc(&d, sizeof(int)) == cudaSuccess &&
+            cudaMemsetAsync(d, 0, sizeof(int), st) == cudaSuccess && cudaStreamSynchronize(st) == cudaSuccess;
+  if (ok) ok = cudaStreamBeginCapture(st, cudaStreamCaptureModeThreadLocal) == cudaSuccess;
+  if (ok) {
+    cudaLaunchAttribute pa[2];
+    cudaLaunchConfig_t pc = cp_config(dim3(kCluster * 2), 0, st, pa);
+    pc.blockDim = dim3(32);
+    const cudaError_t le = cudaLaunchKernelEx(&pc, cp_probe_kernel, d);
+    const cudaError_t ce = cudaStreamEndCapture(st, &g);
+    ok = le == cudaSuccess && ce == cudaSuccess && g != nullptr;
+    if (ok) ok = cudaGraphInstantiate(&ge, g, 0) == cudaSuccess && cudaGraphLaunch(ge, st) == cudaSuccess && cudaStreamSynchronize(st) == cudaSuccess &&
+                 cudaMemcpy(&h, d, sizeof(int), cudaMemcpyDeviceToHost) == cudaSuccess && h == 1;
+  }
+  if (!ok) why = std::string("cooperative cluster launch inside stream capture not accepted: ") + cudaGetErrorString(cudaGetLastError());
+  cudaGetLastError();
+  if (ge) cudaGraphExecDestroy(ge);
+  if (g) cudaGraphDestroy(g);
+  if (d) cudaFree(d);
+  if (st) cudaStreamDestroy(st);
+  return ok ? clusters : 0;
+}
+
+void launch_cp_pass(const LaunchCtx& c, const CpPassParams& p, int clusters) {
+  cudaLaunchAttribute attr[2];
+  cudaLaunchConfig_t cfg = cp_config(dim3(kCluster * clusters), cp_pass_smem(p.sk[0].m_pad), c.stream, attr);
+  Q3_CUDA(cudaLaunchKernelEx(&cfg, cp_pass_kernel, p));
+  c.tick();
+}
+
+}
diff --git a/mlx-swift-qwen3-tts_b200/csrc/cp_pass.h b/mlx-swift-qwen3-tts_b200/csrc/cp_pass.h
--- /dev/null
+++ b/mlx-swift-qwen3-tts_b200/csrc/cp_pass.h
@@ -0,0 +1,44 @@
+#pragma once
+#include <cuda.h>
+
+#include <string>
+
+#include "kernels.h"
+#include "skinny_common.cuh"
+
+namespace q3 {
+
+constexpr int kCpMaxLayers = 5;
+constexpr int kCpGemms = 4 * kCpMaxLayers + 1;
+constexpr int kCpItems = 64;
+constexpr int kCpPhaseSlots = 5 * kCpMaxLayers + 1;
+
+struct CpPassParams {
+  CUtensorMap wmap[kCpGemms];
+  CUtensorMap xmap[kCpGemms];
+  skinny::SkParams sk[kCpGemms];
+  const float* qkv;
+  int ld_qkv, heads, kv_heads;
+  const float* q_norm[kCpMaxLayers];
+  const float* k_norm[kCpMaxLayers];
+  KVLayout kv[kCpMaxLayers];
+  float eps, scale;
+  const float* inv_freq;
+  const int* row_slot;
+  const int* row_pos;
+  __half* attn16;
+  int ld_attn;
+  int layers, M, pass;
+  unsigned* cnt;
+  unsigned* done;
+  unsigned* err;
+  unsigned long long timeout_ns;
+  unsigned long long* trace;
+};
+
+skinny::SkParams tc_skinny_params(const TcGemm& g, CUtensorMap* mw, CUtensorMap* mx);
+size_t cp_pass_smem(int m_pad);
+int cp_pass_init(int m_pad, std::string& why);
+void launch_cp_pass(const LaunchCtx& c, const CpPassParams& p, int clusters);
+
+}
diff --git a/mlx-swift-qwen3-tts_b200/csrc/engine.h b/mlx-swift-qwen3-tts_b200/csrc/engine.h
--- a/mlx-swift-qwen3-tts_b200/csrc/engine.h
+++ b/mlx-swift-qwen3-tts_b200/csrc/engine.h
@@ -111,6 +111,14 @@
   static constexpr int kChainCounters = 1024;
   ChainState chain_;
   bool chain_on_ = false, chain_enabled_ = false;
+  bool cp_persist_env_ = true;
+  int cp_clusters_[2] = {0, 0};
+  std::string cp_why_;
+  unsigned* d_cp_cnt_ = nullptr;
+  unsigned* h_cp_err_ = nullptr;
+  unsigned long long* d_cp_trace_ = nullptr;
+  bool use_cp_persist(int n_slots) const;
+  void issue_cp_pass(int g, int n_slots, float* x);
   float* d_rs_ = nullptr;
   static constexpr float kX16Div = 16.0f;
   void *d_h16_ = nullptr, *d_attn16_ = nullptr, *d_act16_ = nullptr, *d_tpe16_ = nullptr, *d_tph16_ = nullptr;
diff --git a/mlx-swift-qwen3-tts_b200/csrc/gemm_skinny.cu b/mlx-swift-qwen3-tts_b200/csrc/gemm_skinny.cu
--- a/mlx-swift-qwen3-tts_b200/csrc/gemm_skinny.cu
+++ b/mlx-swift-qwen3-tts_b200/csrc/gemm_skinny.cu
@@ -207,8 +207,7 @@
   *tiles = s.tiles; *split = s.split; *stages = s.stages;
 }
 
-void launch_tc_skinny(const LaunchCtx& c, const TcGemm& g) {
-  if (tc_skinny_q_supported(g)) return launch_tc_skinny_q(c, g);
+SkParams tc_skinny_params(const TcGemm& g, CUtensorMap* mw, CUtensorMap* mx) {
   Q3_CHECK(tc_skinny_supported(g), Q3TTS_ERR_INVALID_ARG, "tc_skinny: unsupported shape (rows %d, cin %d, N %d)", g.Bt * g.T, g.cin, g.N);
   tc_resolve_encode();
   const SkPlan s = plan(g);
@@ -226,17 +225,25 @@
   p.rms_x = g.rms_in ? g.a : nullptr;
   p.rms_a = 1.0f / (g.in_scale * g.in_scale * (float)g.cin); p.rms_eps = g.rms_eps; p.rms_mult = 1.0f / g.in_scale;
   Q3_CHECK(!g.row_scale, Q3TTS_ERR_INVALID_ARG, "tc_skinny: pass rms_in instead of precomputed row factors");
-  p.trace = g_sk_trace;
-  p.sig = c.chain_link((unsigned)(s.tiles * s.split));
 
   const uint64_t wdims[2] = {(uint64_t)g.cin, (uint64_t)g.N};
   const uint64_t wstr[1] = {(uint64_t)g.cin * 2};
   const uint32_t wbox[2] = {(uint32_t)kBlockK, (uint32_t)kRowsW};
-  const CUtensorMap mw = tc_make_map(g.w, 2, wdims, wstr, wbox);
+  *mw = tc_make_map(g.w, 2, wdims, wstr, wbox);
   const uint64_t xdims[2] = {(uint64_t)g.cin, (uint64_t)p.M};
   const uint64_t xstr[1] = {(uint64_t)g.cin * 2};
   const uint32_t xbox[2] = {(uint32_t)kBlockK, (uint32_t)s.m_pad};
-  const CUtensorMap mx = tc_make_map(g.a, 2, xdims, xstr, xbox);
+  *mx = tc_make_map(g.a, 2, xdims, xstr, xbox);
+  return p;
+}
+
+void launch_tc_skinny(const LaunchCtx& c, const TcGemm& g) {
+  if (tc_skinny_q_supported(g)) return launch_tc_skinny_q(c, g);
+  CUtensorMap mw, mx;
+  SkParams p = tc_skinny_params(g, &mw, &mx);
+  const SkPlan s = plan(g);
+  p.trace = g_sk_trace;
+  p.sig = c.chain_link((unsigned)(s.tiles * s.split));
 
   Q3_CHECK(s.smem <= 220 * 1024, Q3TTS_ERR_CAPACITY, "tc_skinny: shared memory request %zu too large", s.smem);
   cudaLaunchConfig_t cfg{};
diff --git a/mlx-swift-qwen3-tts_b200/csrc/rope_attention.cuh b/mlx-swift-qwen3-tts_b200/csrc/rope_attention.cuh
--- /dev/null
+++ b/mlx-swift-qwen3-tts_b200/csrc/rope_attention.cuh
@@ -0,0 +1,162 @@
+#pragma once
+#include <cuda_fp16.h>
+
+#include "device_utils.cuh"
+
+namespace q3 {
+
+__device__ __forceinline__ float4 kv_ld4(const float* p) { return *reinterpret_cast<const float4*>(p); }
+__device__ __forceinline__ float4 kv_ld4(const __half* p) {
+  const uint2 u = *reinterpret_cast<const uint2*>(p);
+  const float2 a = __half22float2(*reinterpret_cast<const __half2*>(&u.x)), b = __half22float2(*reinterpret_cast<const __half2*>(&u.y));
+  return make_float4(a.x, a.y, b.x, b.y);
+}
+__device__ __forceinline__ float kv_ld(const float* p) { return *p; }
+__device__ __forceinline__ float kv_ld(const __half* p) { return __half2float(*p); }
+__device__ __forceinline__ void kv_st(float* p, float v) { *p = v; }
+__device__ __forceinline__ void kv_st(__half* p, float v) { *p = __float2half_rn(v); }
+__device__ __forceinline__ void store_act(float* p, float v) { *p = v; }
+__device__ __forceinline__ void store_act(__half* p, float v) { *p = __float2half_rn(v); }
+
+template <int G>
+struct __align__(16) RopeAttnSmem {
+  float q[G * 128];
+  float part_o[4][G][128];
+  float part_m[4][G], part_l[4][G];
+};
+
+__device__ __forceinline__ void ra_bar(int bar_id) { asm volatile("bar.sync %0, 128;" ::"r"(bar_id) : "memory"); }
+
+template <int G, typename OutT, typename KvT>
+__device__ __forceinline__ void rope_attention_item(RopeAttnSmem<G>& sm, int bar_id, int tid, int row, int kvh, const float* __restrict__ qkv, int ld,
+                                                    int heads, int kv_heads, const float* __restrict__ q_norm, const float* __restrict__ k_norm,
+                                                    float eps, const float* __restrict__ inv_freq, const int* __restrict__ row_slot,
+                                                    const int* __restrict__ row_pos, const int* __restrict__ win_start, const KVLayout& kv,
+                                                    OutT* __restrict__ out, int ldo, float scale) {
+  const int lane = tid & 31, warp = tid >> 5;
+  const int slot = row_slot[row], pos = row_pos[row];
+  const int w0 = win_start ? win_start[slot] : 0;
+  const int S = pos - w0 + 1;
+  const int cap = kv.capacity;
+  const int r0 = w0 % cap;
+  const int ring = (r0 + S - 1 >= cap) ? r0 + S - 1 - cap : r0 + S - 1;
+  KvT* kb = static_cast<KvT*>(kv.k) + (size_t)slot * kv.slot_stride + (size_t)kvh * cap * 128;
+  KvT* vb = static_cast<KvT*>(kv.v) + (size_t)slot * kv.slot_stride + (size_t)kvh * cap * 128;
+  const float* rowp = qkv + (size_t)row * ld;
+  for (int hh = warp; hh <= G; hh += 4) {
+    const float* src = rowp + (size_t)(hh < G ? (kvh * G + hh) : (heads + kvh)) * 128;
+    const float a0 = src[lane], a1 = src[lane + 32], b0 = src[lane + 64], b1 = src[lane + 96];
+    const float ss = warp_sum(a0 * a0 + a1 * a1 + b0 * b0 + b1 * b1);
+    const float inv = rsqrtf(ss * (1.0f / 128.0f) + eps);
+    const float* nw = hh < G ? q_norm : k_norm;
+    const float x0 = a0 * inv * nw[lane], x1 = a1 * inv * nw[lane + 32], y0 = b0 * inv * nw[lane + 64], y1 = b1 * inv * nw[lane + 96];
+    float s0, c0, s1, c1;
+    sincosf((float)pos * inv_freq[lane], &s0, &c0);
+    sincosf((float)pos * inv_freq[lane + 32], &s1, &c1);
+    const float o0 = x0 * c0 - y0 * s0, o1 = x1 * c1 - y1 * s1, o2 = y0 * c0 + x0 * s0, o3 = y1 * c1 + x1 * s1;
+    if (hh < G) {
+      float* dst = sm.q + hh * 128;
+      dst[lane] = o0; dst[lane + 32] = o1; dst[lane + 64] = o2; dst[lane + 96] = o3;
+    } else {
+      KvT* dst = kb + (size_t)ring * 128;
+      kv_st(dst + lane, o0); kv_st(dst + lane + 32, o1); kv_st(dst + lane + 64, o2); kv_st(dst + lane + 96, o3);
+    }
+  }
+  kv_st(vb + (size_t)ring * 128 + tid, rowp[(size_t)(heads + kv_heads + kvh) * 128 + tid]);
+  ra_bar(bar_id);
+  const int seg = lane & 7, grp = warp * 4 + (lane >> 3);
+  float qf[G][16];
+#pragma unroll
+  for (int g = 0; g < G; ++g)
+#pragma unroll
+    for (int i = 0; i < 4; ++i) {
+      const float4 t = *reinterpret_cast<const float4*>(sm.q + g * 128 + i * 32 + seg * 4);
+      qf[g][4 * i] = t.x * scale; qf[g][4 * i + 1] = t.y * scale; qf[g][4 * i + 2] = t.z * scale; qf[g][4 * i + 3] = t.w * scale;
+    }
+  float mx[G], l[G], o[G][16];
+#pragma unroll
+  for (int g = 0; g < G; ++g) {
+    mx[g] = -INFINITY; l[g] = 0.f;
+#pragma unroll
+    for (int d = 0; d < 16; ++d) o[g][d] = 0.f;
+  }
+  for (int jb = 0; jb < S; jb += 32) {
+    const int j0 = jb + grp;
+    float4 kk[2][4], vv[2][4];
+#pragma unroll
+    for (int u = 0; u < 2; ++u) {
+      const int j = j0 + 16 * u;
+      const int rj = r0 + (j < S ? j : 0);
+      const size_t base = (size_t)(rj >= cap ? rj - cap : rj) * 128 + seg * 4;
+#pragma unroll
+      for (int i = 0; i < 4; ++i) {
+        kk[u][i] = kv_ld4(kb + base + i * 32);
+        vv[u][i] = kv_ld4(vb + base + i * 32);
+      }
+    }
+#pragma unroll
+    for (int u = 0; u < 2; ++u) {
+      const bool valid = j0 + 16 * u < S;
+#pragma unroll
+      for (int g = 0; g < G; ++g) {
+        float sdot = 0.f;
+#pragma unroll
+        for (int i = 0; i < 4; ++i)
+          sdot += kk[u][i].x * qf[g][4 * i] + kk[u][i].y * qf[g][4 * i + 1] + kk[u][i].z * qf[g][4 * i + 2] + kk[u][i].w * qf[g][4 * i + 3];
+        sdot += __shfl_xor_sync(0xffffffffu, sdot, 1);
+        sdot += __shfl_xor_sync(0xffffffffu, sdot, 2);
+        sdot += __shfl_xor_sync(0xffffffffu, sdot, 4);
+        if (!valid) sdot = -INFINITY;
+        const float mn = fmaxf(mx[g], sdot);
+        const bool none = mn == -INFINITY;
+        const float corr = none ? 1.f : expf(mx[g] - mn), pr = none ? 0.f : expf(sdot - mn);
+        mx[g] = mn;
+        l[g] = l[g] * corr + pr;
+#pragma unroll
+        for (int i = 0; i < 4; ++i) {
+          o[g][4 * i] = o[g][4 * i] * corr + pr * vv[u][i].x;
+          o[g][4 * i + 1] = o[g][4 * i + 1] * corr + pr * vv[u][i].y;
+          o[g][4 * i + 2] = o[g][4 * i + 2] * corr + pr * vv[u][i].z;
+          o[g][4 * i + 3] = o[g][4 * i + 3] * corr + pr * vv[u][i].w;
+        }
+      }
+    }
+  }
+#pragma unroll
+  for (int g = 0; g < G; ++g) {
+    float m_all = fmaxf(mx[g], __shfl_xor_sync(0xffffffffu, mx[g], 8));
+    m_all = fmaxf(m_all, __shfl_xor_sync(0xffffffffu, m_all, 16));
+    const float f = (mx[g] == -INFINITY) ? 0.f : expf(mx[g] - m_all);
+    float lw = l[g] * f;
+    lw += __shfl_xor_sync(0xffffffffu, lw, 8);
+    lw += __shfl_xor_sync(0xffffffffu, lw, 16);
+#pragma unroll
+    for (int d = 0; d < 16; ++d) {
+      float t = o[g][d] * f;
+      t += __shfl_xor_sync(0xffffffffu, t, 8);
+      t += __shfl_xor_sync(0xffffffffu, t, 16);
+      o[g][d] = t;
+    }
+    if (lane < 8) {
+#pragma unroll
+      for (int i = 0; i < 4; ++i)
+        *reinterpret_cast<float4*>(&sm.part_o[warp][g][i * 32 + seg * 4]) = make_float4(o[g][4 * i], o[g][4 * i + 1], o[g][4 * i + 2], o[g][4 * i + 3]);
+      if (lane == 0) { sm.part_m[warp][g] = m_all; sm.part_l[warp][g] = lw; }
+    }
+  }
+  ra_bar(bar_id);
+#pragma unroll
+  for (int g = 0; g < G; ++g) {
+    float m_all = fmaxf(fmaxf(sm.part_m[0][g], sm.part_m[1][g]), fmaxf(sm.part_m[2][g], sm.part_m[3][g]));
+    float num = 0.f, den = 0.f;
+#pragma unroll
+    for (int w = 0; w < 4; ++w) {
+      const float f = (sm.part_m[w][g] == -INFINITY) ? 0.f : expf(sm.part_m[w][g] - m_all);
+      num += sm.part_o[w][g][tid] * f;
+      den += sm.part_l[w][g] * f;
+    }
+    store_act(out + (size_t)row * ldo + (size_t)(kvh * G + g) * 128 + tid, num / den);
+  }
+}
+
+}
diff --git a/mlx-swift-qwen3-tts_b200/csrc/skinny_common.cuh b/mlx-swift-qwen3-tts_b200/csrc/skinny_common.cuh
--- a/mlx-swift-qwen3-tts_b200/csrc/skinny_common.cuh
+++ b/mlx-swift-qwen3-tts_b200/csrc/skinny_common.cuh
@@ -104,7 +104,8 @@
 
 template <int ACT, bool SWIGLU>
 __device__ __forceinline__ void sk_reduce_epilogue(const SkParams& p, float* stage_out, float* red, uint64_t* red_full, uint64_t* ack, const float* rowscale_s,
-                                                   uint32_t tmem_base, uint32_t rank, int n0) {
+                                                   uint32_t tmem_base, uint32_t rank, int n0, uint32_t rank_base = 0, uint32_t red_par = 0,
+                                                   uint32_t ack_par = 0) {
   const int warp = threadIdx.x >> 5, lane = threadIdx.x & 31;
   const int q = warp & 3;
   const int row = q * 32 + lane;
@@ -133,8 +134,8 @@
     mbar_expect_tx(red_full, slice_bytes * (uint32_t)(p.split - 1));
     for (int i = 1; i < p.split; ++i) {
       const uint32_t d = (rank + (uint32_t)i) & (uint32_t)(p.split - 1);
-      bulk_copy_to_rank(map_to_rank(smem_u32(red + (size_t)rank * kRowsW * p.mc), d), smem_u32(stage_out + (size_t)d * kRowsW * p.mc), slice_bytes,
-                        map_to_rank(smem_u32(red_full), d));
+      bulk_copy_to_rank(map_to_rank(smem_u32(red + (size_t)rank * kRowsW * p.mc), rank_base + d), smem_u32(stage_out + (size_t)d * kRowsW * p.mc), slice_bytes,
+                        map_to_rank(smem_u32(red_full), rank_base + d));
     }
   }
   if (threadIdx.x == 64) SK_STAMP(5);
@@ -147,11 +148,11 @@
     valid0 = valid0 < p.mc ? valid0 : p.mc;
     sk_load_res<16>(p, r16, lane_out ? valid0 : 0, m_base, so);
   }
-  if (p.split > 1) mbar_wait(red_full, 0);
+  if (p.split > 1) mbar_wait(red_full, red_par);
   if (threadIdx.x == 96) SK_STAMP_EPI(10);
   if (threadIdx.x == 64) {
     SK_STAMP(6);
-    for (int i = 1; i < p.split; ++i) mbar_arrive_remote_relaxed(map_to_rank(smem_u32(ack), (rank + (uint32_t)i) & (uint32_t)(p.split - 1)));
+    for (int i = 1; i < p.split; ++i) mbar_arrive_remote_relaxed(map_to_rank(smem_u32(ack), rank_base + ((rank + (uint32_t)i) & (uint32_t)(p.split - 1))));
   }
   const uint32_t own_s = smem_u32(stage_out), red_s = smem_u32(red);
   for (int cb = 0; cb < p.mc; cb += 16) {
@@ -184,7 +185,7 @@
   }
   if (threadIdx.x == 64 && p.split > 1) {
     SK_STAMP(7);
-    mbar_wait(ack, 0);
+    mbar_wait(ack, ack_par);
   }
 }
 
diff --git a/mlx-swift-qwen3-tts_b200/csrc/talker_engine.cu b/mlx-swift-qwen3-tts_b200/csrc/talker_engine.cu
--- a/mlx-swift-qwen3-tts_b200/csrc/talker_engine.cu
+++ b/mlx-swift-qwen3-tts_b200/csrc/talker_engine.cu
@@ -1,6 +1,7 @@
 #include <algorithm>
 #include <cmath>
 
+#include "cp_pass.h"
 #include "engine.h"
 #include "frame_kernel.h"
 #include "gemm_tc.h"
@@ -104,6 +105,19 @@
   chain_enabled_ = false;
   if (const char* e = getenv("Q3TTS_CHAIN")) chain_enabled_ = atoi(e) != 0;
   if (!pdl_enabled()) chain_enabled_ = false;
+  if (const char* e = getenv("Q3TTS_CP_PERSIST")) cp_persist_env_ = atoi(e) != 0;
+  if (handle_tc_ && cp_persist_env_ && opt_.use_cuda_graph) {
+    for (int b = 0; b < 2; ++b) cp_clusters_[b] = cp_pass_init(b == 0 ? 32 : 64, cp_why_);
+    const size_t n = (size_t)kCpPhaseSlots * kCpItems + 2;
+    d_cp_cnt_ = arena_.alloc_n<unsigned>(n);
+    Q3_CUDA(cudaMemsetAsync(d_cp_cnt_, 0, sizeof(unsigned) * n, stream_));
+    Q3_CUDA(cudaMallocHost(&h_cp_err_, sizeof(unsigned)));
+    *h_cp_err_ = 0;
+    if (getenv("Q3TTS_CP_TRACE")) {
+      d_cp_trace_ = arena_.alloc_n<unsigned long long>((size_t)15 * 8 * std::max(cp_clusters_[0], cp_clusters_[1]) * 32);
+      Q3_CUDA(cudaMemsetAsync(d_cp_trace_, 0, sizeof(unsigned long long) * 15 * 8 * std::max(cp_clusters_[0], cp_clusters_[1]) * 32, stream_));
+    }
+  }
   d_probe_logits_ = arena_.alloc_n<float>(4096);
   d_probe_set_ = arena_.alloc_n<unsigned>(128);
   d_probe_out_ = arena_.alloc_n<int>(1);
@@ -344,6 +358,7 @@
   drop_graphs();
   if (h_stage_) cudaFreeHost(h_stage_);
   if (h_state_) cudaFreeHost(h_state_);
+  if (h_cp_err_) cudaFreeHost(h_cp_err_);
   if (ev_a_) cudaEventDestroy(ev_a_);
   if (ev_b_) cudaEventDestroy(ev_b_);
   if (d_dump0_) cudaFree(d_dump0_);
@@ -717,6 +732,14 @@
   for (int g = 0; g < 15; ++g) {
     const int m = g == 0 ? 2 * n_slots : n_slots;
     float* x = d_cpin_;
+    if (g != 0 && use_cp_persist(n_slots)) {
+      if (w_.has_mtp) {
+        linear_tc(w_.small_to_mtp_tc, d_h16_, m, d_cpx_, Hcp, nullptr, 0, nullptr, TC_ACT_NONE, 0);
+        x = d_cpx_;
+        launch_scale_to_f16(c, x, (size_t)m * Hcp, 1.0f / kX16Div, (__half*)d_h16_);
+      }
+      issue_cp_pass(g, n_slots, x);
+    } else {
     if (w_.has_mtp) {
       if (step_tc_) {
         linear_tc(w_.small_to_mtp_tc, d_h16_, m, d_cpx_, Hcp, nullptr, 0, nullptr, TC_ACT_NONE, 0);
@@ -742,6 +765,7 @@
     } else {
       launch_linear(c, w_.lm_head[g], x, Hcp, n_slots, d_cplogits_, Vc, w_.cp.final_norm, w_.cp.eps, EPI_STORE);
     }
+    }
     SamplerParams pg = p;
     pg.vocab = Vc; pg.group = g + 1;
     launch_sample(c, d_cplogits_, Vc, n_slots, d_state_, pg, d_sets_, d_cur_codes_, d_forced_, F, dumpcp, 15 * Vc, g * Vc, dump_slot_,
@@ -760,6 +784,57 @@
     launch_linear(c, w_.codec_head, d_hlast_, H, n_slots, d_logits0_, V, nullptr, 0.f, EPI_STORE);
   }
   launch_step_advance(c, n_slots, d_state_, 192);
+}
+
+bool TalkerEngine::use_cp_persist(int n_slots) const {
+  const StackWeights& P = w_.cp;
+  if (!step_tc_ || n_slots < 1 || n_slots > 64 || cp_clusters_[n_slots <= 32 ? 0 : 1] < 1 || packed_gemm_ || !tc_skinny_enabled() || chain_on_) return false;
+  if (!opt_.use_cuda_graph || opt_.lanes > 1 || shared_.use_count() > 1) return false;
+  if (P.layers < 1 || P.layers > kCpMaxLayers || P.head_dim != 128 || P.kv_heads < 1 || P.heads != 2 * P.kv_heads || P.tc.empty()) return false;
+  return (int)w_.lm_head_tc.size() == 15 && (P.heads + 2 * P.kv_heads) <= kCpItems && cfg_.cp.vocab_size <= kCpItems * 128 && P.inter / 64 <= kCpItems;
+}
+
+void TalkerEngine::issue_cp_pass(int g, int n_slots, float* x) {
+  const StackWeights& S = w_.cp;
+  const int B = opt_.max_batch, m = n_slots;
+  const int qkv_ld = (S.heads + 2 * S.kv_heads) * 128, attn_ld = S.heads * 128;
+  const float inv16 = 1.0f / kX16Div;
+  CpPassParams p{};
+  int k = 0;
+  auto gemm = [&](const TcLinear& L, const void* a16, bool rms, float* out32, int ld32, void* out16, int ld16, int swiglu, const float* res) {
+    TcGemm t;
+    t.a = (const __half*)a16; t.w = (const __half*)L.w; t.Bt = 1; t.T = m; t.cin = L.in; t.N = L.out;
+    t.bias = L.bias; t.swiglu = swiglu; t.out32 = out32; t.ld32 = ld32; t.out16 = (__half*)out16; t.ld16 = ld16;
+    t.res = res; t.ld_res = res ? S.hidden : 0;
+    if (res) t.out16_scale = inv16;
+    if (rms) { t.rms_in = 1; t.rms_eps = S.eps; t.in_scale = inv16; }
+    p.sk[k] = tc_skinny_params(t, &p.wmap[k], &p.xmap[k]);
+    int tiles = 0, split = 0, stages = 0;
+    tc_skinny_grid(t, &tiles, &split, &stages);
+    Q3_CHECK(tiles <= kCpItems && split >= 1 && split <= 8 && p.sk[k].m_pad == p.sk[0].m_pad, Q3TTS_ERR_BAD_CONFIG, "cp_pass: GEMM %d outside the persistent plan", k);
+    ++k;
+  };
+  for (int l = 0; l < S.layers; ++l) {
+    const LayerTc& Tc = S.tc[l];
+    gemm(Tc.qkv, d_h16_, true, d_qkv_, qkv_ld, nullptr, 0, 0, nullptr);
+    gemm(Tc.o, d_attn16_, false, x, S.hidden, d_h16_, S.hidden, 0, x);
+    gemm(Tc.gate_up_il, d_h16_, true, nullptr, 0, d_act16_, S.inter, 1, nullptr);
+    gemm(Tc.down, d_act16_, false, x, S.hidden, d_h16_, S.hidden, 0, x);
+    p.q_norm[l] = S.layer[l].q_norm; p.k_norm[l] = S.layer[l].k_norm;
+    KVLayout& kv = p.kv[l];
+    kv.k = cp_k_ + l * cpkv_layer_stride_; kv.v = cp_v_ + l * cpkv_layer_stride_;
+    kv.slot_stride = cpkv_slot_stride_; kv.capacity = kCpCapacity; kv.f16 = 0;
+  }
+  gemm(w_.lm_head_tc[g], d_h16_, true, d_cplogits_, cfg_.cp.vocab_size, nullptr, 0, 0, nullptr);
+  p.qkv = d_qkv_; p.ld_qkv = qkv_ld; p.heads = S.heads; p.kv_heads = S.kv_heads;
+  p.eps = S.eps; p.scale = 1.0f / sqrtf(128.0f); p.inv_freq = d_cp_inv_freq_;
+  p.row_slot = d_iota_; p.row_pos = d_cp_pos_ + (size_t)g * B;
+  p.attn16 = (__half*)d_attn16_; p.ld_attn = attn_ld;
+  p.layers = S.layers; p.M = m; p.pass = g;
+  p.cnt = d_cp_cnt_; p.done = d_cp_cnt_ + kCpPhaseSlots * kCpItems; p.err = p.done + 1;
+  p.timeout_ns = 2000000000ull;
+  p.trace = d_cp_trace_;
+  launch_cp_pass(ctx(), p, cp_clusters_[m <= 32 ? 0 : 1]);
 }
 
 void TalkerEngine::run_frames(int n_slots, int n) {
@@ -809,11 +884,24 @@
     if (counter_) counter_->n += it->second.nodes;
     ++graph_replays;
   }
+  if (d_cp_trace_ && use_cp_persist(n_slots)) {
+    const int ctas = 8 * cp_clusters_[n_slots <= 32 ? 0 : 1];
+    std::vector<unsigned long long> t((size_t)15 * ctas * 32 + 2);
+    t[0] = (unsigned long long)ctas; t[1] = (unsigned long long)w_.cp.layers;
+    Q3_CUDA(cudaMemcpyAsync(t.data() + 2, d_cp_trace_, sizeof(unsigned long long) * (t.size() - 2), cudaMemcpyDeviceToHost, stream_));
+    Q3_CUDA(cudaStreamSynchronize(stream_));
+    if (FILE* f = fopen(getenv("Q3TTS_CP_TRACE"), "wb")) { fwrite(t.data(), sizeof(unsigned long long), t.size(), f); fclose(f); }
+  }
 }
 
 void TalkerEngine::fetch_states(int n_slots, std::vector<SlotState>& out) {
   Q3_CUDA(cudaMemcpyAsync(h_state_, d_state_, sizeof(SlotState) * n_slots, cudaMemcpyDeviceToHost, stream_));
+  if (h_cp_err_) Q3_CUDA(cudaMemcpyAsync(h_cp_err_, d_cp_cnt_ + kCpPhaseSlots * kCpItems + 1, sizeof(unsigned), cudaMemcpyDeviceToHost, stream_));
   Q3_CUDA(cudaStreamSynchronize(stream_));
+  if (h_cp_err_ && *h_cp_err_) {
+    const unsigned e = *h_cp_err_ - 1u;
+    fail(Q3TTS_ERR_CUDA, "cp_pass_kernel: a readiness wait expired (pass %u, phase %u, item %u)", e >> 16, (e >> 8) & 255u, e & 255u);
+  }
   out.assign(h_state_, h_state_ + n_slots);
 }
 
diff --git a/mlx-swift-qwen3-tts_b200/csrc/talker_kernels.cu b/mlx-swift-qwen3-tts_b200/csrc/talker_kernels.cu
--- a/mlx-swift-qwen3-tts_b200/csrc/talker_kernels.cu
+++ b/mlx-swift-qwen3-tts_b200/csrc/talker_kernels.cu
@@ -3,6 +3,7 @@
 
 #include "kernels.h"
 #include "device_utils.cuh"
+#include "rope_attention.cuh"
 #include "sampler.cuh"
 
 namespace q3 {
@@ -331,16 +332,6 @@
   c.tick();
 }
 
-__device__ __forceinline__ float4 kv_ld4(const float* p) { return *reinterpret_cast<const float4*>(p); }
-__device__ __forceinline__ float4 kv_ld4(const __half* p) {
-  const uint2 u = *reinterpret_cast<const uint2*>(p);
-  const float2 a = __half22float2(*reinterpret_cast<const __half2*>(&u.x)), b = __half22float2(*reinterpret_cast<const __half2*>(&u.y));
-  return make_float4(a.x, a.y, b.x, b.y);
-}
-__device__ __forceinline__ float kv_ld(const float* p) { return *p; }
-__device__ __forceinline__ float kv_ld(const __half* p) { return __half2float(*p); }
-__device__ __forceinline__ void kv_st(float* p, float v) { *p = v; }
-__device__ __forceinline__ void kv_st(__half* p, float v) { *p = __float2half_rn(v); }
 template <typename KvT>
 __global__ void __launch_bounds__(128) qk_norm_rope_append_kernel(float* __restrict__ qkv, int ld, int m, int heads, int kv_heads,
                                                                   const float* __restrict__ q_norm, const float* __restrict__ k_norm,
@@ -393,8 +384,6 @@
   c.tick();
 }
 
-__device__ __forceinline__ void store_act(float* p, float v) { *p = v; }
-__device__ __forceinline__ void store_act(__half* p, float v) { *p = __float2half_rn(v); }
 
 template <int G, typename OutT, typename KvT>
 __global__ void __launch_bounds__(128) attention_kernel(const float* __restrict__ qkv, int ld, int heads, int kv_heads,
@@ -463,9 +452,7 @@
                                                              const float* __restrict__ inv_freq, const int* __restrict__ row_slot,
                                                              const int* __restrict__ row_pos, const int* __restrict__ win_start, KVLayout kv,
                                                              OutT* __restrict__ out, int ldo, float scale, const ChainSig sig) {
-  __shared__ __align__(16) float q[G * 128];
-  __shared__ __align__(16) float part_o[4][G][128];
-  __shared__ float part_m[4][G], part_l[4][G];
+  __shared__ RopeAttnSmem<G> sm;
   pdl_launch_dependents();
   if (sig.in) {
     if (threadIdx.x == 0) chain_wait(sig.in, sig.in_target);
@@ -473,130 +460,8 @@
   } else {
     pdl_wait();
   }
-  const int row = blockIdx.x, kvh = blockIdx.y, tid = threadIdx.x, lane = tid & 31, warp = tid >> 5;
-  const int slot = row_slot[row], pos = row_pos[row];
-  const int w0 = win_start ? win_start[slot] : 0;
-  const int S = pos - w0 + 1;
-  const int cap = kv.capacity;
-  const int r0 = w0 % cap;
-  const int ring = (r0 + S - 1 >= cap) ? r0 + S - 1 - cap : r0 + S - 1;
-  KvT* kb = static_cast<KvT*>(kv.k) + (size_t)slot * kv.slot_stride + (size_t)kvh * cap * 128;
-  KvT* vb = static_cast<KvT*>(kv.v) + (size_t)slot * kv.slot_stride + (size_t)kvh * cap * 128;
-  const float* rowp = qkv + (size_t)row * ld;
-  for (int hh = warp; hh <= G; hh += 4) {
-    const float* src = rowp + (size_t)(hh < G ? (kvh * G + hh) : (heads + kvh)) * 128;
-    const float a0 = src[lane], a1 = src[lane + 32], b0 = src[lane + 64], b1 = src[lane + 96];
-    const float ss = warp_sum(a0 * a0 + a1 * a1 + b0 * b0 + b1 * b1);
-    const float inv = rsqrtf(ss * (1.0f / 128.0f) + eps);
-    const float* nw = hh < G ? q_norm : k_norm;
-    const float x0 = a0 * inv * nw[lane], x1 = a1 * inv * nw[lane + 32], y0 = b0 * inv * nw[lane + 64], y1 = b1 * inv * nw[lane + 96];
-    float s0, c0, s1, c1;
-    sincosf((float)pos * inv_freq[lane], &s0, &c0);
-    sincosf((float)pos * inv_freq[lane + 32], &s1, &c1);
-    const float o0 = x0 * c0 - y0 * s0, o1 = x1 * c1 - y1 * s1, o2 = y0 * c0 + x0 * s0, o3 = y1 * c1 + x1 * s1;
-    if (hh < G) {
-      float* dst = q + hh * 128;
-      dst[lane] = o0; dst[lane + 32] = o1; dst[lane + 64] = o2; dst[lane + 96] = o3;
-    } else {
-      KvT* dst = kb + (size_t)ring * 128;
-      kv_st(dst + lane, o0); kv_st(dst + lane + 32, o1); kv_st(dst + lane + 64, o2); kv_st(dst + lane + 96, o3);
-    }
-  }
-  kv_st(vb + (size_t)ring * 128 + tid, rowp[(size_t)(heads + kv_heads + kvh) * 128 + tid]);
-  __syncthreads();
-  const int seg = lane & 7, grp = warp * 4 + (lane >> 3);
-  float qf[G][16];
-#pragma unroll
-  for (int g = 0; g < G; ++g)
-#pragma unroll
-    for (int i = 0; i < 4; ++i) {
-      const float4 t = *reinterpret_cast<const float4*>(q + g * 128 + i * 32 + seg * 4);
-      qf[g][4 * i] = t.x * scale; qf[g][4 * i + 1] = t.y * scale; qf[g][4 * i + 2] = t.z * scale; qf[g][4 * i + 3] = t.w * scale;
-    }
-  float mx[G], l[G], o[G][16];
-#pragma unroll
-  for (int g = 0; g < G; ++g) {
-    mx[g] = -INFINITY; l[g] = 0.f;
-#pragma unroll
-    for (int d = 0; d < 16; ++d) o[g][d] = 0.f;
-  }
-  for (int jb = 0; jb < S; jb += 32) {
-    const int j0 = jb + grp;
-    float4 kk[2][4], vv[2][4];
-#pragma unroll
-    for (int u = 0; u < 2; ++u) {
-      const int j = j0 + 16 * u;
-      const int rj = r0 + (j < S ? j : 0);
-      const size_t base = (size_t)(rj >= cap ? rj - cap : rj) * 128 + seg * 4;
-#pragma unroll
-      for (int i = 0; i < 4; ++i) {
-        kk[u][i] = kv_ld4(kb + base + i * 32);
-        vv[u][i] = kv_ld4(vb + base + i * 32);
-      }
-    }
-#pragma unroll
-    for (int u = 0; u < 2; ++u) {
-      const bool valid = j0 + 16 * u < S;
-#pragma unroll
-      for (int g = 0; g < G; ++g) {
-        float sdot = 0.f;
-#pragma unroll
-        for (int i = 0; i < 4; ++i)
-          sdot += kk[u][i].x * qf[g][4 * i] + kk[u][i].y * qf[g][4 * i + 1] + kk[u][i].z * qf[g][4 * i + 2] + kk[u][i].w * qf[g][4 * i + 3];
-        sdot += __shfl_xor_sync(0xffffffffu, sdot, 1);
-        sdot += __shfl_xor_sync(0xffffffffu, sdot, 2);
-        sdot += __shfl_xor_sync(0xffffffffu, sdot, 4);
-        if (!valid) sdot = -INFINITY;
-        const float mn = fmaxf(mx[g], sdot);
-        const bool none = mn == -INFINITY;
-        const float corr = none ? 1.f : expf(mx[g] - mn), pr = none ? 0.f : expf(sdot - mn);
-        mx[g] = mn;
-        l[g] = l[g] * corr + pr;
-#pragma unroll
-        for (int i = 0; i < 4; ++i) {
-          o[g][4 * i] = o[g][4 * i] * corr + pr * vv[u][i].x;
-          o[g][4 * i + 1] = o[g][4 * i + 1] * corr + pr * vv[u][i].y;
-          o[g][4 * i + 2] = o[g][4 * i + 2] * corr + pr * vv[u][i].z;
-          o[g][4 * i + 3] = o[g][4 * i + 3] * corr + pr * vv[u][i].w;
-        }
-      }
-    }
-  }
-#pragma unroll
-  for (int g = 0; g < G; ++g) {
-    float m_all = fmaxf(mx[g], __shfl_xor_sync(0xffffffffu, mx[g], 8));
-    m_all = fmaxf(m_all, __shfl_xor_sync(0xffffffffu, m_all, 16));
-    const float f = (mx[g] == -INFINITY) ? 0.f : expf(mx[g] - m_all);
-    float lw = l[g] * f;
-    lw += __shfl_xor_sync(0xffffffffu, lw, 8);
-    lw += __shfl_xor_sync(0xffffffffu, lw, 16);
-#pragma unroll
-    for (int d = 0; d < 16; ++d) {
-      float t = o[g][d] * f;
-      t += __shfl_xor_sync(0xffffffffu, t, 8);
-      t += __shfl_xor_sync(0xffffffffu, t, 16);
-      o[g][d] = t;
-    }
-    if (lane < 8) {
-#pragma unroll
-      for (int i = 0; i < 4; ++i)
-        *reinterpret_cast<float4*>(&part_o[warp][g][i * 32 + seg * 4]) = make_float4(o[g][4 * i], o[g][4 * i + 1], o[g][4 * i + 2], o[g][4 * i + 3]);
-      if (lane == 0) { part_m[warp][g] = m_all; part_l[warp][g] = lw; }
-    }
-  }
-  __syncthreads();
-#pragma unroll
-  for (int g = 0; g < G; ++g) {
-    float m_all = fmaxf(fmaxf(part_m[0][g], part_m[1][g]), fmaxf(part_m[2][g], part_m[3][g]));
-    float num = 0.f, den = 0.f;
-#pragma unroll
-    for (int w = 0; w < 4; ++w) {
-      const float f = (part_m[w][g] == -INFINITY) ? 0.f : expf(part_m[w][g] - m_all);
-      num += part_o[w][g][tid] * f;
-      den += part_l[w][g] * f;
-    }
-    store_act(out + (size_t)row * ldo + (size_t)(kvh * G + g) * 128 + tid, num / den);
-  }
+  rope_attention_item<G, OutT, KvT>(sm, 0, threadIdx.x, blockIdx.x, blockIdx.y, qkv, ld, heads, kv_heads, q_norm, k_norm, eps, inv_freq, row_slot,
+                                    row_pos, win_start, kv, out, ldo, scale);
   if (sig.out) {
     __syncthreads();
     if (threadIdx.x == 0) chain_signal(sig.out);
```
